# imatge-upc/rsis

Hardware: AMD Instinct MI355X
Metric: training images/sec at 256x256, T=10, batch=32 per GPU (higher is better)
Workload: dtype f32

## Files before the change

include/rsis_hip.h:

```cpp
#ifndef RSIS_HIP_H
#define RSIS_HIP_H
#include <stddef.h>
#ifdef __cplusplus
extern "C" {
#endif

#define RSIS_ABI_VERSION 2

#define RSIS_DTYPE_F32 0
#define RSIS_DTYPE_BF16 1
#define RSIS_DTYPE_BF16_BLK 2
#define RSIS_DTYPE_F32_WINO 3

int rsis_version(void);
const char* rsis_error_string(int code);
int rsis_conv_uses_wino(int ks, int stride, int pad, int Cin, int Cout, int nseg, int lstm_hid);

int rsis_set_deterministic(int on);
int rsis_get_deterministic(void);

int rsis_conv_uses_bf16(int ks, int stride, int pad, int Cout);
long rsis_conv_packed_bytes_fwd(int dtype, int Cout, int ks, int stride, int pad, int nseg, const int* Cseg);
long rsis_conv_packed_bytes_dgrad(int dtype, int Cout, int ks, int stride, int pad, int c_count);
int rsis_conv_pack_fwd(const float* W, void* Wp, int Cout, int Ctot, int ks, int stride, int pad, int nseg, const int* Cseg,
                       const int* Coff, int lstm_hid, int dtype, void* stream);
int rsis_conv_pack_dgrad(const float* W, void* Wd, int Cout, int Ctot, int ks, int stride, int pad, int nseg, const int* Cseg,
                         const int* Coff, int lstm_hid, int dtype, void* stream);

int rsis_conv2d_fwd(const float* const* src, const int* Csrc, int nsrc, int B, int H, int W, const void* Wp, int Cout,
                    int ks, int stride, int pad, const float* bias, const float* addend, float* out, int Ho, int Wo,
                    int tile, int dtype, void* stream);
int rsis_conv2d_fwd_bn_eval(const float* const* src, const int* Csrc, int nsrc, int B, int H, int W, const void* Wp, int Cout,
                            int ks, int stride, int pad, const float* bias, const float* addend, const float* gamma, const float* beta,
                            const float* running_mean, const float* running_var, float eps, int relu, float* out, int Ho, int Wo,
                            int tile, int dtype, void* stream);

int rsis_conv2d_dgrad(const float* dy, int B, int Cout, int Hy, int Wy, const void* Wd, int Cin_packed, int ks, int stride,
                      int pad, float* const* dx, const int* Cdx, int ndst, int Hx, int Wx, const float* addend, int tile,
                      int dtype, void* stream);

int rsis_conv2d_wgrad(const float* dy, const float* x, float* dW, int B, int Cs, int H, int W, int Cout, int Ho, int Wo,
                      int ks, int stride, int pad, int Ctot, int c_off, int lstm_hid, int dtype, void* stream);

typedef struct rsis_wgrad_job {
  const float* dy;
  const float* x;
  float* dW;
  int B, Cs, H, W, Cout, Ho, Wo, ks, stride, pad, Ctot, c_off, lstm_hid, dtype;
} rsis_wgrad_job;
int rsis_conv2d_wgrad_batch(const rsis_wgrad_job* jobs, int njobs, void* stream);

int rsis_bias_grad(const float* dy, float* db, int B, int C, int HW, int lstm_hid, void* stream);

int rsis_convlstm_fwd(const float* const* src, const int* Csrc, int nsrc, int B, int H, int W, const void* Wp,
                      const float* bias_packed, const float* addend, const float* c_prev, float* h_out, float* c_out,
                      float* act_out, int hid, int ks, int pad, int tile, int dtype, void* stream);

typedef struct rsis_lstm_job {
  const float* src[3];
  int Csrc[3];
  int nsrc, B, H, W;
  const void* Wp;
  const float* bias_packed;
  const float* addend;
  const float* c_prev;
  float* h_out;
  float* c_out;
  float* act_out;
  int hid, ks, pad, tile, dtype;
  unsigned long long* side_key;
} rsis_lstm_job;
int rsis_convlstm_fwd_batch(const rsis_lstm_job* jobs, int njobs, void* stream);

int rsis_convlstm_bwd_gates(const float* dh, const float* dh2, const float* dc_next, const float* act, const float* c_prev,
                            const float* c, float* da, float* dc_prev, float* da_sum, int B, int hid, int HW, void* stream);

typedef struct rsis_lstm_bwd_job {
  const float* dh;
  const float* dh2;
  const float* dc_next;
  const float* act;
  const float* c_prev;
  const float* c;
  float* da;
  float* dc_prev;
  int B, hid, HW;
} rsis_lstm_bwd_job;
int rsis_convlstm_bwd_gates_batch(const rsis_lstm_bwd_job* jobs, int njobs, void* stream);
typedef struct rsis_dgrad_job {
  const float* dy;
  int B, Cout, Hy, Wy;
  const void* Wd;
  int Cin_packed, ks, stride, pad;
  float* dx[3];
  int Cdx[3];
  int ndst, Hx, Wx;
  const float* addend;
  int tile, dtype;
} rsis_dgrad_job;
int rsis_conv2d_dgrad_batch(const rsis_dgrad_job* jobs, int njobs, void* stream);

int rsis_upsample_bilinear_ac_fwd(const float* x, float* y, long BC, int Hi, int Wi, int Ho, int Wo, void* stream);
int rsis_upsample_bilinear_ac_bwd(const float* dy, float* dx, long BC, int Hi, int Wi, int Ho, int Wo, void* stream);
int rsis_upsample_maxpool_bwd(const float* dy, const float* dpool, const int* argmax, float* dx, long BC, int Hi, int Wi, int Ho,
                              int Wo, void* stream);

int rsis_global_maxpool_fwd(const float* x, float* y, int* argmax, long BC, int HW, void* stream);
int rsis_global_maxpool_bwd(const float* dy, const int* argmax, float* dx, long BC, int HW, void* stream);
int rsis_global_maxpool_bwd_add(const float* dy, const int* argmax, float* dx, long BC, int HW, void* stream);

int rsis_upsample_bilinear_ac_scaled_fwd(const float* x, const float* scale, float* y, long BC, int Hi, int Wi, int Ho, int Wo, void* stream);
int rsis_upsample_maxpool_scaled_bwd(const float* dy, const float* dpool, const int* argmax, const float* scale, float* dx, long BC, int Hi,
                                     int Wi, int Ho, int Wo, void* stream);
int rsis_global_maxpool_scaled_bwd_add(const float* dy, const int* argmax, const float* scale, float* dx, long BC, int HW, void* stream);
int rsis_scale_planes(const float* x, const float* scale, float* y, long BC, int HW, void* stream);

int rsis_dropout_scales(unsigned int* state, float* s2, float* mc, float* ms, long n, float p2, float pc, float ps, void* stream);
int rsis_dropout_heads_mask(float* side, const float* s2, const float* mc, const float* ms, float* side_c, float* side_s, long n, void* stream);
int rsis_dropout_heads_mask_bwd(const float* dside_c, const float* dside_s, const float* mc, const float* ms, float* dside, long n, void* stream);

int rsis_bn_fwd(const float* x, const float* res, float* y, double* stats, const float* gamma, const float* beta,
                float* running_mean, float* running_var, float* save_mean, float* save_rstd, int B, int C, int HW,
                float eps, float momentum, int relu, int train, void* stream);
int rsis_bn_bwd(const float* dy, const float* x, const float* y, const float* save_mean, const float* save_rstd,
                const float* gamma, double* stats, float* dx, float* dres, float* dgamma, float* dbeta, int B, int C,
                int HW, int relu, void* stream);

int rsis_bn_bwd_eval(const float* dy, const float* x, const float* y, const float* running_mean, const float* running_var,
                     const float* gamma, double* stats, float* dx, float* dres, float* dgamma, float* dbeta, int B, int C, int HW,
                     float eps, int relu, void* stream);

int rsis_bn_fwd_mask(const float* x, const float* res, float* y, unsigned char* mask, double* stats, const float* gamma, const float* beta,
                     float* running_mean, float* running_var, float* save_mean, float* save_rstd, int B, int C, int HW,
                     float eps, float momentum, int train, void* stream);
int rsis_bn_bwd_mask(const float* dy, const float* x, const unsigned char* mask, const float* save_mean, const float* save_rstd,
                     const float* gamma, double* stats, float* dx, float* dres, float* dgamma, float* dbeta, int B, int C,
                     int HW, int flags, void* stream);
int rsis_bn_bwd_eval_mask(const float* dy, const float* x, const unsigned char* mask, const float* running_mean, const float* running_var,
                          const float* gamma, double* stats, float* dx, float* dres, float* dgamma, float* dbeta, int B, int C, int HW,
                          float eps, int flags, void* stream);

int rsis_subsample2d(const float* x, float* y, long BC, int H, int W, int stride, void* stream);

int rsis_maxpool3x3s2_fwd(const float* x, float* y, unsigned char* argmax, long BC, int H, int W, int Ho, int Wo,
                          void* stream);
int rsis_maxpool3x3s2_bwd(const float* dy, const unsigned char* argmax, float* dx, long BC, int H, int W, int Ho, int Wo,
                          int accumulate, void* stream);

int rsis_adam_step(float* p, const float* g, float* m, float* v, long n, float lr, float beta1, float beta2, float eps,
                   float weight_decay, int step, float gscale, const int* step_dev, void* stream);

int rsis_sgd_step(float* p, const float* g, float* buf, long n, float lr, float momentum, float weight_decay, float gscale,
                  void* stream);
int rsis_rmsprop_step(float* p, const float* g, float* sq, long n, float lr, float alpha, float eps, float weight_decay, float gscale,
                      void* stream);

int rsis_assign_min_cost(const float* scores, long long* perm, int B, int G, int T, void* stream);

typedef struct rsis_pack_job {
  const float* W;
  void* out;
  int dgrad;
  int dtype;
  int Cout, Ctot, ks, stride, pad, nseg, Cseg[3], Coff[3], lstm_hid;
  int imode, ldw, krows;
  int block_begin;
} rsis_pack_job;
int rsis_conv_pack_job_fill(rsis_pack_job* job);
int rsis_conv_pack_batch(const rsis_pack_job* jobs_dev, int njobs, int total_blocks, void* stream);

int rsis_conv_out_wgrad(const float* dy, const float* x, float* dW, float* db, int B, int Cin, int H, int W, void* stream);

int rsis_conv_out_seq_fwd(const float* x, const void* Wp, const float* bias, float* y, int T, int B, int Cin, int H, int W, void* stream);
int rsis_conv_out_seq_dgrad(const float* dy, const void* Wd, float* dx, int T, int B, int Cin, int H, int W, void* stream);
int rsis_conv_out_seq_wgrad(const float* dy, const float* x, float* dW, float* db, int T, int B, int Cin, int H, int W, void* stream);

int rsis_sum_leading(const float* x, float* y, int T, long n, void* stream);

int rsis_affine_nearest(const float* x, float* y, const float* mat, int mat_rows, int N, int C, int H, int W, void* stream);

long rsis_targets_work_ints(int B);
int rsis_targets_from_maps(const int* ins, const int* seg, int B, int H, int W, int T, float* y_mask, long long* y_class, float* sw_mask,
                           float* sw_class, int* work, void* stream);

long rsis_instance_maps_work_ints(int B);
int rsis_instance_maps(const int* raw, const int* class_of_label, int n_labels, int B, int H, int W, int* ins, int* seg, int* work,
                       void* stream);

int rsis_palette_to_ids(const unsigned char* rgb, long npix, const unsigned char* table, int ntab, unsigned char* ids, void* stream);
int rsis_idmap_rle_encode(const unsigned char* idmap, int h, int w, const int* ids, int k, unsigned int* counts, int cap, int* nruns,
                          void* stream);

int rsis_softiou_sums(const float* logits, const float* y, float* S, int B, int T, int G, long N, void* stream);
int rsis_softiou_bwd(const float* logits, const float* y, const long long* perm, int perm_ld, const float* ca, const float* cb,
                     float* dlogits, int B, int T, int G, long N, void* stream);

int rsis_heads_fwd(const float* const* side, const int* Cside, int nside, int B, const float* Wc, const float* bc, int ncls,
                   const float* Ws, const float* bs, float* class_probs, float* stop, void* stream);
int rsis_heads_fwd_keys(const unsigned long long* const* keys, float* const* side_out, int* const* arg_out, const int* Cside, int nside,
                        int B, const float* Wc, const float* bc, int ncls, const float* Ws, const float* bs, float* class_probs, float* stop,
                        void* stream);
int rsis_heads_bwd(const float* const* side, const int* Cside, int nside, int B, const float* Wc, int ncls, const float* Ws,
                   const float* class_probs, const float* dprobs, const float* dstop, float* const* dside, float* dWc, float* dbc,
                   float* dWs, float* dbs, void* stream);
int rsis_heads_wide_fwd(const unsigned long long* const* keys, float* const* side_out, int* const* arg_out, const float* const* side,
                        const int* Cside, int nside, int rows, const float* Wc, const float* bc, int ncls, const float* Ws, const float* bs,
                        float* class_probs, float* stop, void* stream);
int rsis_heads_wide_bwd(const float* const* side, const int* Cside, int nside, int rows, const float* Wc, int ncls, const float* Ws,
                        const float* class_probs, const float* dprobs, const float* dstop, float* const* dside, float* dWc, float* dbc,
                        float* dWs, float* dbs, float* scratch, long scratch_floats, void* stream);

int rsis_loss_tail(const float* probs, const long long* y_class, const float* stop, const float* siou, const float* sw_mask,
                   const float* sw_class, const float* cls_w, int n, int C, float bw, float w_iou, float w_cls, float w_stop,
                   float* out, float* dprobs, float* dstop, float* dsiou, const float* gout, void* stream);

int rsis_mask_resize_threshold(const float* prob, int n, int Hm, int Wm, const unsigned char* ignore, float th, unsigned char* seg,
                               unsigned char* raw, unsigned int* area, int h, int w, void* stream);
int rsis_rle_encode(const unsigned char* masks, int n, long len, unsigned int* counts, int cap, int* nruns, void* stream);
int rsis_rle_to_string(const unsigned int* counts, int m, char* out, int cap);
int rsis_largest_component(const unsigned char* mask, unsigned char* out, int* labels, int* counts, int* best, int n, int h, int w,
                           void* stream);

int rsis_overlay_moments(const unsigned char* masks, int n, const int* order, int k, int h, int w, unsigned long long* moments,
                         void* stream);
int rsis_overlay_masks(const unsigned char* image, const unsigned char* masks, int n, const int* order, const unsigned char* colors,
                       int k, float alpha, unsigned char* out, int h, int w, void* stream);

int rsis_mask_pack_bits(const unsigned char* masks, int n, long len, unsigned long long* bits, long stride, unsigned int* area, void* stream);
int rsis_rle_to_bits(const unsigned int* counts, long counts_len, const long long* desc, int n, unsigned int* ends, unsigned long long* bits,
                     long bits_len, unsigned int* area, void* stream);
int rsis_poly_to_bits(const double* xy, long nverts, const long long* parts, long nparts, const long long* recs, int n,
                      unsigned long long* scratch, unsigned long long* bits, long bits_len, unsigned int* area, void* stream);
int rsis_paint_instance_maps(const unsigned long long* bits, long bits_len, const unsigned int* area, long nrec, const long long* recs,
                             const long long* imgs, int B, int max_recs, const int* src_y, const int* src_x, int Ho, int Wo, int* ins, int* seg,
                             void* stream);
long rsis_mask_intersect_blocks(long D, long G, long stride);
int rsis_mask_intersect_batch(const unsigned long long* bits, long bits_len, const long long* jobs, int njobs, int total_blocks,
                              unsigned int* inter, long inter_len, void* stream);
int rsis_coco_iou_batch(const long long* cells, int ncells, const unsigned int* inter, long inter_len, const int* dt_row,
                        const unsigned int* dt_marea, long ndt, const int* gt_col, const unsigned int* gt_marea, const int* gt_crowd, long ngt,
                        double* ious, long ious_len, void* stream);
int rsis_coco_match_batch(const long long* cells, int ncells, const double* ious, long ious_len, const int* gperm, const int* gflag, long ngt,
                          const double* dt_area, long ndt, const double* arng, int nrng, const double* thrs, int T, int* dtm, int* dti,
                          long dt_out_len, int* gtm, long gt_out_len, void* stream);
int rsis_rle_from_string(const char* s, unsigned int* counts, int cap);

long rsis_label_contingency_blocks(long npix);
int rsis_label_contingency_batch(const unsigned char* pool, long pool_len, const long long* jobs, int njobs, int total_blocks,
                                 unsigned int* counts, long counts_len, void* stream);
int rsis_label_scores_batch(const unsigned int* counts, long counts_len, const long long* jobs, int njobs, double* scores, void* stream);

long rsis_inst_overlap_blocks(long npix, long P);
int rsis_inst_presence_batch(const void* pool, long pool_len, const long long* jobs, int njobs, int total_blocks, unsigned char* flags,
                             long flags_len, void* stream);
int rsis_inst_overlap_batch(const void* pool, long pool_len, const long long* jobs, int njobs, int total_blocks, const unsigned short* lut,
                            long lut_len, const unsigned long long* bits, long bits_len, unsigned int* counts, long counts_len, void* stream);


int rsis_blk_from_nchw(const float* x, void* y_blk, int B, int C, int H, int W, void* stream);
int rsis_blk_to_nchw(const void* x_blk, float* y, int B, int C, int H, int W, void* stream);
// ... 99 lines not shown
```

rsis_amd/_lib.py:

```python
import ctypes
import os

import torch

_HERE = os.path.dirname(os.path.abspath(__file__))
LIB_PATH = os.environ.get("RSIS_HIP_LIB") or os.path.join(_HERE, "lib", "librsis_hip.so")

_vp, _i, _l, _f = ctypes.c_void_p, ctypes.c_int, ctypes.c_long, ctypes.c_float
_ip = ctypes.POINTER(ctypes.c_int)
_vpp = ctypes.POINTER(ctypes.c_void_p)

class PackJob(ctypes.Structure):
    _fields_ = [("W", ctypes.c_void_p), ("out", ctypes.c_void_p), ("dgrad", ctypes.c_int), ("dtype", ctypes.c_int), ("Cout", ctypes.c_int),
                ("Ctot", ctypes.c_int), ("ks", ctypes.c_int), ("stride", ctypes.c_int), ("pad", ctypes.c_int),
                ("nseg", ctypes.c_int), ("Cseg", ctypes.c_int * 3), ("Coff", ctypes.c_int * 3), ("lstm_hid", ctypes.c_int),
                ("imode", ctypes.c_int), ("ldw", ctypes.c_int), ("krows", ctypes.c_int), ("block_begin", ctypes.c_int)]


class WgradJob(ctypes.Structure):
    _fields_ = [("dy", ctypes.c_void_p), ("x", ctypes.c_void_p), ("dW", ctypes.c_void_p)] + \
               [(k, ctypes.c_int) for k in ("B", "Cs", "H", "W", "Cout", "Ho", "Wo", "ks", "stride", "pad", "Ctot", "c_off", "lstm_hid", "dtype")]


class LstmJob(ctypes.Structure):
    _fields_ = [("src", ctypes.c_void_p * 3), ("Csrc", ctypes.c_int * 3), ("nsrc", ctypes.c_int), ("B", ctypes.c_int), ("H", ctypes.c_int),
                ("W", ctypes.c_int), ("Wp", ctypes.c_void_p), ("bias_packed", ctypes.c_void_p), ("addend", ctypes.c_void_p),
                ("c_prev", ctypes.c_void_p), ("h_out", ctypes.c_void_p), ("c_out", ctypes.c_void_p), ("act_out", ctypes.c_void_p),
                ("hid", ctypes.c_int), ("ks", ctypes.c_int), ("pad", ctypes.c_int), ("tile", ctypes.c_int), ("dtype", ctypes.c_int),
                ("side_key", ctypes.c_void_p)]


class LstmBwdJob(ctypes.Structure):
    _fields_ = [(k, ctypes.c_void_p) for k in ("dh", "dh2", "dc_next", "act", "c_prev", "c", "da", "dc_prev")] + \
               [(k, ctypes.c_int) for k in ("B", "hid", "HW")]


class DgradJob(ctypes.Structure):
    _fields_ = [("dy", ctypes.c_void_p), ("B", ctypes.c_int), ("Cout", ctypes.c_int), ("Hy", ctypes.c_int), ("Wy", ctypes.c_int),
                ("Wd", ctypes.c_void_p), ("Cin_packed", ctypes.c_int), ("ks", ctypes.c_int), ("stride", ctypes.c_int), ("pad", ctypes.c_int),
                ("dx", ctypes.c_void_p * 3), ("Cdx", ctypes.c_int * 3), ("ndst", ctypes.c_int), ("Hx", ctypes.c_int), ("Wx", ctypes.c_int),
                ("addend", ctypes.c_void_p), ("tile", ctypes.c_int), ("dtype", ctypes.c_int)]


class BlkConvJob(ctypes.Structure):
    _fields_ = [("src", ctypes.c_void_p * 3), ("Csrc", ctypes.c_int * 3), ("nsrc", ctypes.c_int), ("B", ctypes.c_int), ("H", ctypes.c_int),
                ("W", ctypes.c_int), ("Wp", ctypes.c_void_p), ("Cout", ctypes.c_int), ("Cpack", ctypes.c_int), ("bias", ctypes.c_void_p),
                ("addend", ctypes.c_void_p), ("dst", ctypes.c_void_p * 2), ("Cdst", ctypes.c_int * 2), ("ndst", ctypes.c_int),
                ("hid", ctypes.c_int), ("c_prev", ctypes.c_void_p), ("c_out", ctypes.c_void_p), ("h_out", ctypes.c_void_p),
                ("act_out", ctypes.c_void_p), ("side_key", ctypes.c_void_p), ("tile", ctypes.c_int)]


class BlkResizeJob(ctypes.Structure):
    _fields_ = [("src", ctypes.c_void_p), ("dst", ctypes.c_void_p), ("dpool", ctypes.c_void_p), ("arg", ctypes.c_void_p)] + \
               [(k, ctypes.c_int) for k in ("B", "C", "Hi", "Wi", "Ho", "Wo")]


class BlkResizeScaledJob(ctypes.Structure):
    _fields_ = BlkResizeJob._fields_ + [("scale", ctypes.c_void_p)]


class BlkLstmBwdJob(ctypes.Structure):
    _fields_ = [(k, ctypes.c_void_p) for k in ("dh", "dh2", "dc_next", "act", "c_prev", "c", "da", "dc_prev")] + \
               [(k, ctypes.c_int) for k in ("B", "hid", "HW")]


SIGNATURES = {
    "rsis_version": (_i, []),
    "rsis_error_string": (ctypes.c_char_p, [_i]),
    "rsis_set_deterministic": (_i, [_i]),
    "rsis_get_deterministic": (_i, []),
    "rsis_conv_uses_bf16": (_i, [_i, _i, _i, _i]),
    "rsis_conv_uses_wino": (_i, [_i, _i, _i, _i, _i, _i, _i]),
    "rsis_conv_packed_bytes_fwd": (_l, [_i, _i, _i, _i, _i, _i, _ip]),
    "rsis_conv_packed_bytes_dgrad": (_l, [_i, _i, _i, _i, _i, _i]),
    "rsis_conv_pack_fwd": (_i, [_vp, _vp, _i, _i, _i, _i, _i, _i, _ip, _ip, _i, _i, _vp]),
    "rsis_conv_pack_dgrad": (_i, [_vp, _vp, _i, _i, _i, _i, _i, _i, _ip, _ip, _i, _i, _vp]),
    "rsis_conv_pack_job_fill": (_i, [ctypes.POINTER(PackJob)]),
    "rsis_conv_pack_batch": (_i, [_vp, _i, _i, _vp]),
    "rsis_conv2d_fwd": (_i, [_vpp, _ip, _i, _i, _i, _i, _vp, _i, _i, _i, _i, _vp, _vp, _vp, _i, _i, _i, _i, _vp]),
    "rsis_conv2d_fwd_bn_eval": (_i, [_vpp, _ip, _i, _i, _i, _i, _vp, _i, _i, _i, _i, _vp, _vp, _vp, _vp, _vp, _vp, _f, _i, _vp, _i, _i, _i, _i, _vp]),
    "rsis_conv2d_dgrad": (_i, [_vp, _i, _i, _i, _i, _vp, _i, _i, _i, _i, _vpp, _ip, _i, _i, _i, _vp, _i, _i, _vp]),
    "rsis_conv2d_wgrad": (_i, [_vp, _vp, _vp, _i, _i, _i, _i, _i, _i, _i, _i, _i, _i, _i, _i, _i, _i, _vp]),
    "rsis_conv2d_wgrad_batch": (_i, [ctypes.POINTER(WgradJob), _i, _vp]),
    "rsis_affine_nearest": (_i, [_vp, _vp, _vp, _i, _i, _i, _i, _i, _vp]),
    "rsis_targets_work_ints": (_l, [_i]),
    "rsis_targets_from_maps": (_i, [_vp, _vp, _i, _i, _i, _i, _vp, _vp, _vp, _vp, _vp, _vp]),
    "rsis_instance_maps_work_ints": (_l, [_i]),
    "rsis_instance_maps": (_i, [_vp, _vp, _i, _i, _i, _i, _vp, _vp, _vp, _vp]),
    "rsis_palette_to_ids": (_i, [_vp, _l, _vp, _i, _vp, _vp]),
    "rsis_idmap_rle_encode": (_i, [_vp, _i, _i, _vp, _i, _vp, _i, _vp, _vp]),
    "rsis_conv_out_wgrad": (_i, [_vp, _vp, _vp, _vp, _i, _i, _i, _i, _vp]),
    "rsis_conv_out_seq_fwd": (_i, [_vp, _vp, _vp, _vp, _i, _i, _i, _i, _i, _vp]),
    "rsis_conv_out_seq_dgrad": (_i, [_vp, _vp, _vp, _i, _i, _i, _i, _i, _vp]),
    "rsis_conv_out_seq_wgrad": (_i, [_vp, _vp, _vp, _vp, _i, _i, _i, _i, _i, _vp]),
    "rsis_sum_leading": (_i, [_vp, _vp, _i, _l, _vp]),
    "rsis_bias_grad": (_i, [_vp, _vp, _i, _i, _i, _i, _vp]),
    "rsis_convlstm_fwd": (_i, [_vpp, _ip, _i, _i, _i, _i, _vp, _vp, _vp, _vp, _vp, _vp, _vp, _i, _i, _i, _i, _i, _vp]),
    "rsis_convlstm_fwd_batch": (_i, [ctypes.POINTER(LstmJob), _i, _vp]),
    "rsis_convlstm_bwd_gates": (_i, [_vp, _vp, _vp, _vp, _vp, _vp, _vp, _vp, _vp, _i, _i, _i, _vp]),
    "rsis_upsample_bilinear_ac_fwd": (_i, [_vp, _vp, _l, _i, _i, _i, _i, _vp]),
    "rsis_upsample_bilinear_ac_bwd": (_i, [_vp, _vp, _l, _i, _i, _i, _i, _vp]),
    "rsis_upsample_maxpool_bwd": (_i, [_vp, _vp, _vp, _vp, _l, _i, _i, _i, _i, _vp]),
    "rsis_global_maxpool_fwd": (_i, [_vp, _vp, _vp, _l, _i, _vp]),
    "rsis_global_maxpool_bwd": (_i, [_vp, _vp, _vp, _l, _i, _vp]),
    "rsis_global_maxpool_bwd_add": (_i, [_vp, _vp, _vp, _l, _i, _vp]),
    "rsis_bn_fwd": (_i, [_vp, _vp, _vp, _vp, _vp, _vp, _vp, _vp, _vp, _vp, _i, _i, _i, _f, _f, _i, _i, _vp]),
    "rsis_bn_bwd": (_i, [_vp, _vp, _vp, _vp, _vp, _vp, _vp, _vp, _vp, _vp, _vp, _i, _i, _i, _i, _vp]),
    "rsis_bn_bwd_eval": (_i, [_vp, _vp, _vp, _vp, _vp, _vp, _vp, _vp, _vp, _vp, _vp, _i, _i, _i, _f, _i, _vp]),
    "rsis_bn_fwd_mask": (_i, [_vp, _vp, _vp, _vp, _vp, _vp, _vp, _vp, _vp, _vp, _vp, _i, _i, _i, _f, _f, _i, _vp]),
    "rsis_bn_bwd_mask": (_i, [_vp, _vp, _vp, _vp, _vp, _vp, _vp, _vp, _vp, _vp, _vp, _i, _i, _i, _i, _vp]),
    "rsis_bn_bwd_eval_mask": (_i, [_vp, _vp, _vp, _vp, _vp, _vp, _vp, _vp, _vp, _vp, _vp, _i, _i, _i, _f, _i, _vp]),
    "rsis_subsample2d": (_i, [_vp, _vp, _l, _i, _i, _i, _vp]),
    "rsis_maxpool3x3s2_fwd": (_i, [_vp, _vp, _vp, _l, _i, _i, _i, _i, _vp]),
    "rsis_maxpool3x3s2_bwd": (_i, [_vp, _vp, _vp, _l, _i, _i, _i, _i, _i, _vp]),
    "rsis_assign_min_cost": (_i, [_vp, _vp, _i, _i, _i, _vp]),
    "rsis_heads_fwd": (_i, [_vpp, _ip, _i, _i, _vp, _vp, _i, _vp, _vp, _vp, _vp, _vp]),
    "rsis_heads_fwd_keys": (_i, [_vpp, _vpp, _vpp, _ip, _i, _i, _vp, _vp, _i, _vp, _vp, _vp, _vp, _vp]),
    "rsis_blk_from_nchw": (_i, [_vp, _vp, _i, _i, _i, _i, _vp]),
    "rsis_blk_to_nchw": (_i, [_vp, _vp, _i, _i, _i, _i, _vp]),
    "rsis_blk_bn_scratch_doubles": (ctypes.c_long, [_i]),
    "rsis_blk_bn_fwd": (_i, [_vp, _vp, _vp, _vp, _vp, _vp, _vp, _vp, _vp, _vp, _i, _i, _i, _i, _f, _f, _i, _i, _vp]),
    "rsis_blk_bn_bwd": (_i, [_vp, _vp, _vp, _vp, _vp, _vp, _vp, _vp, _vp, _vp, _vp, _vp, _i, _i, _i, _i, _i, _i, _vp]),
    "rsis_blk_subsample2d": (_i, [_vp, _vp, _i, _i, _i, _i, _i, _vp]),
    "rsis_blk_upscatter2d": (_i, [_vp, _vp, _i, _i, _i, _i, _i, _vp]),
    "rsis_blk_conv2d": (_i, [_vp, _i, _i, _i, _i, _vp, _i, _i, _vp, _vp, _i, _vp]),
    "rsis_blk_conv2d_bn_eval": (_i, [_vp, _i, _i, _i, _i, _vp, _i, _i, _vp, _vp, _vp, _vp, _vp, ctypes.c_float, _i, _i, _vp, _i, _vp]),
    "rsis_convlstm_bwd_gates_batch": (_i, [ctypes.POINTER(LstmBwdJob), _i, _vp]),
    "rsis_conv2d_dgrad_batch": (_i, [ctypes.POINTER(DgradJob), _i, _vp]),
    "rsis_blk_conv3x3_batch": (_i, [ctypes.POINTER(BlkConvJob), _i, _vp]),
    "rsis_blk_upsample_fwd_batch": (_i, [ctypes.POINTER(BlkResizeJob), _i, _vp]),
    "rsis_blk_upsample_bwd_batch": (_i, [ctypes.POINTER(BlkResizeJob), _i, _vp]),
    "rsis_blk_lstm_bwd_batch": (_i, [ctypes.POINTER(BlkLstmBwdJob), _i, _vp]),
    "rsis_blk_sum_leading": (_i, [_vp, _vp, _i, _l, _vp]),
    "rsis_blk_bias_grad": (_i, [_vp, _vp, _i, _i, _i, _i, _vp]),
    "rsis_blk_conv_out_seq_fwd": (_i, [_vp, _vp, _vp, _vp, _i, _i, _i, _i, _vp]),
    "rsis_blk_conv_out_seq_dgrad": (_i, [_vp, _vp, _vp, _i, _i, _i, _i, _vp]),
    "rsis_blk_conv_out_seq_wgrad": (_i, [_vp, _vp, _vp, _vp, _i, _i, _i, _i, _vp]),
    "rsis_upconv_out_supported": (_i, [_i, _i, _i, _i, _i]),
    "rsis_upconv_out_bwd_blocks": (_i, [_i, _i, _i, _i]),
    "rsis_upconv_out_fwd": (_i, [_vp, _i, _vp, _vp, _vp, _i, _i, _i, _i, _i, _i, _i, _vp]),
    "rsis_upconv_out_bwd": (_i, [_vp, _vp, _i, _vp, _vp, _vp, _vp, _vp, _vp, _vp, _i, _i, _i, _i, _i, _i, _i, _vp]),
    "rsis_comm_available": (_i, []),
    "rsis_comm_unique_id": (_i, [_vp]),
    "rsis_comm_init": (_i, [_vpp, _i, _i, _vp]),
    "rsis_comm_size": (_i, [_vp]),
    "rsis_comm_allreduce_sum_f32": (_i, [_vp, _vp, _l, _vp]),
    "rsis_comm_destroy": (_i, [_vp]),
    "rsis_comm_last_error": (ctypes.c_char_p, []),
    "rsis_heads_bwd": (_i, [_vpp, _ip, _i, _i, _vp, _i, _vp, _vp, _vp, _vp, _vpp, _vp, _vp, _vp, _vp, _vp]),
    "rsis_heads_wide_fwd": (_i, [_vpp, _vpp, _vpp, _vpp, _ip, _i, _i, _vp, _vp, _i, _vp, _vp, _vp, _vp, _vp]),
    "rsis_heads_wide_bwd": (_i, [_vpp, _ip, _i, _i, _vp, _i, _vp, _vp, _vp, _vp, _vpp, _vp, _vp, _vp, _vp, _vp, _l, _vp]),
    "rsis_loss_tail": (_i, [_vp, _vp, _vp, _vp, _vp, _vp, _vp, _i, _i, _f, _f, _f, _f, _vp, _vp, _vp, _vp, _vp, _vp]),
    "rsis_softiou_sums": (_i, [_vp, _vp, _vp, _i, _i, _i, _l, _vp]),
    "rsis_softiou_bwd": (_i, [_vp, _vp, _vp, _i, _vp, _vp, _vp, _i, _i, _i, _l, _vp]),
    "rsis_mask_resize_threshold": (_i, [_vp, _i, _i, _i, _vp, _f, _vp, _vp, _vp, _i, _i, _vp]),
    "rsis_rle_encode": (_i, [_vp, _i, _l, _vp, _i, _vp, _vp]),
    "rsis_largest_component": (_i, [_vp, _vp, _vp, _vp, _vp, _i, _i, _i, _vp]),
    "rsis_overlay_moments": (_i, [_vp, _i, _vp, _i, _i, _i, _vp, _vp]),
    "rsis_overlay_masks": (_i, [_vp, _vp, _i, _vp, _vp, _i, _f, _vp, _i, _i, _vp]),
    "rsis_rle_to_string": (_i, [_vp, _i, ctypes.c_char_p, _i]),
    "rsis_mask_pack_bits": (_i, [_vp, _i, _l, _vp, _l, _vp, _vp]),
    "rsis_rle_to_bits": (_i, [_vp, _l, _vp, _i, _vp, _vp, _l, _vp, _vp]),
    "rsis_mask_intersect_blocks": (_l, [_l, _l, _l]),
    "rsis_mask_intersect_batch": (_i, [_vp, _l, _vp, _i, _i, _vp, _l, _vp]),
    "rsis_coco_iou_batch": (_i, [_vp, _i, _vp, _l, _vp, _vp, _l, _vp, _vp, _vp, _l, _vp, _l, _vp]),
    "rsis_poly_to_bits": (_i, [_vp, _l, _vp, _l, _vp, _i, _vp, _vp, _l, _vp, _vp]),
    "rsis_paint_instance_maps": (_i, [_vp, _l, _vp, _l, _vp, _vp, _i, _i, _vp, _vp, _i, _i, _vp, _vp, _vp]),
    "rsis_coco_match_batch": (_i, [_vp, _i, _vp, _l, _vp, _vp, _l, _vp, _l, _vp, _i, _vp, _i, _vp, _vp, _l, _vp, _l, _vp]),
    "rsis_rle_from_string": (_i, [ctypes.c_char_p, _vp, _i]),
    "rsis_label_contingency_blocks": (_l, [_l]),
    "rsis_label_contingency_batch": (_i, [_vp, _l, _vp, _i, _i, _vp, _l, _vp]),
    "rsis_label_scores_batch": (_i, [_vp, _l, _vp, _i, _vp, _vp]),
    "rsis_inst_overlap_blocks": (_l, [_l, _l]),
    "rsis_inst_presence_batch": (_i, [_vp, _l, _vp, _i, _i, _vp, _l, _vp]),
    "rsis_inst_overlap_batch": (_i, [_vp, _l, _vp, _i, _i, _vp, _l, _vp, _l, _vp, _l, _vp]),
    "rsis_adam_step": (_i, [_vp, _vp, _vp, _vp, _l, _f, _f, _f, _f, _f, _i, _f, _vp, _vp]),
    "rsis_sgd_step": (_i, [_vp, _vp, _vp, _l, _f, _f, _f, _f, _vp]),
    "rsis_rmsprop_step": (_i, [_vp, _vp, _vp, _l, _f, _f, _f, _f, _f, _vp]),
    "rsis_upsample_bilinear_ac_scaled_fwd": (_i, [_vp, _vp, _vp, _l, _i, _i, _i, _i, _vp]),
# ... 67 lines not shown
```

rsis_amd/csrc/api.hip:

```cpp
#include "common.h"
#include "../../include/rsis_hip.h"
#include "launchers.h"
#include <stdlib.h>

static inline int krows_of(int C, int ks) { return rsis_roundup(C * ks * ks, RSIS_KPAD); }
static inline int log2i(int s) { int l = 0; while ((1 << l) < s) ++l; return l; }
static inline bool use_direct(int ks, int stride, int pad) { return ks == 3 && stride == 1 && pad == 1; }
static inline bool use_direct_s2(int ks, int stride, int pad) { return ks == 3 && stride == 2 && pad == 1; }
static inline bool use_direct_f2(int ks, int stride, int pad) {
  static const bool on = !(getenv("RSIS_CONV_F2") && getenv("RSIS_CONV_F2")[0] == '0');
  return on && use_direct_s2(ks, stride, pad);
}
static inline bool use_direct_fwd(int ks, int stride, int pad) { return use_direct(ks, stride, pad) || use_direct_f2(ks, stride, pad); }
static inline int seg_chunks(int nseg, const int* Cseg, int ck) {
  int q = 0;
  for (int s = 0; s < nseg; ++s) q += (Cseg[s] + ck - 1) / ck;
  return q;
}
static inline int direct_rows(int nseg, const int* Cseg) { return seg_chunks(nseg, Cseg, RSIS_CK) * RSIS_CK * 9; }
static inline bool bf16_geom(int ks, int stride, int pad, int Cout) {
  return Cout > 1 && ((ks == 3 && stride == 1 && pad == 1) || (ks == 1 && pad == 0));
}
static inline bool use_bf16(int dtype, int ks, int stride, int pad, int Cout) {
  return dtype == RSIS_DTYPE_BF16 && bf16_geom(ks, stride, pad, Cout);
// ... 52 lines not shown
    default: return "unknown error";
  }
}

int rsis_conv_uses_bf16(int ks, int stride, int pad, int Cout) { return bf16_geom(ks, stride, pad, Cout) ? 1 : 0; }
int rsis_conv_uses_wino(int ks, int stride, int pad, int Cin, int Cout, int nseg, int lstm_hid) {
  return wino_geom(ks, stride, pad, Cin, Cout, nseg, lstm_hid) ? 1 : 0;
}

struct PackPlan { int status; PackMode mode; int krows; int ldw; long bytes; };
static PackPlan pack_plan(bool dgrad, int dtype, int Cout, int Ctot, int ks, int stride, int pad, int nseg, const int* Cseg, const int* Coff,
                          int lstm_hid) {
  PackPlan p = {RSIS_OK, PACK_IGEMM_FWD, 0, 0, 0};
  int csum = 0;
  for (int s = 0; s < nseg; ++s) csum += Cseg[s];
  p.ldw = rsis_roundup(dgrad ? csum : Cout, RSIS_LDW_ALIGN);
  if (lstm_hid > 0 && dtype == RSIS_DTYPE_BF16 && ks != 3) { p.status = RSIS_ERR_UNSUPPORTED; return p; }
  if (dtype == RSIS_DTYPE_F32_WINO && (dgrad ? wino_geom_dgrad(ks, stride, pad, csum, Cout) : wino_geom(ks, stride, pad, csum, Cout, nseg, lstm_hid))) {
    if (!dgrad && (csum != Ctot || (Coff && Coff[0] != 0))) { p.status = RSIS_ERR_UNSUPPORTED; return p; }
    p.mode = dgrad ? PACK_WINO_DGRAD : PACK_WINO_FWD;
    p.krows = dgrad ? (csum / 32) * (Cout / 8) : (Cout / 32) * (csum / 8);
    p.bytes = (long)p.krows * 32 * 8 * 16 * 4;
    return p;
  }
  long cell = 4;
  if (use_bf16(dtype, ks, stride, pad, Cout)) {
    p.mode = dgrad ? PACK_BF16_DGRAD : PACK_BF16_FWD;
    p.krows = dgrad ? bf16_rows(ks, 1, &Cout) : bf16_rows(ks, nseg, Cseg);
    cell = 16;
  } else if (dgrad ? use_direct(ks, stride, pad) : use_direct_fwd(ks, stride, pad)) {
    p.mode = dgrad ? PACK_DIRECT_DGRAD : PACK_DIRECT_FWD;
    p.krows = dgrad ? direct_rows(1, &Cout) : direct_rows(nseg, Cseg);
  } else if (dgrad && use_direct_s2(ks, stride, pad) && nseg == 1) {
    p.mode = PACK_DIRECT_DGRAD_S2;
    p.krows = direct_rows(1, &Cout);
  } else {
    p.mode = dgrad ? PACK_IGEMM_DGRAD : PACK_IGEMM_FWD;
    p.krows = krows_of(dgrad ? Cout : csum, ks);
  }
  p.bytes = (long)p.krows * p.ldw * cell;
  return p;
}

long rsis_conv_packed_bytes_fwd(int dtype, int Cout, int ks, int stride, int pad, int nseg, const int* Cseg) {
  if (nseg < 1 || nseg > RSIS_MAX_SRC || !Cseg) return -1;
  int csum = 0;
  for (int s = 0; s < nseg; ++s) csum += Cseg[s];
  return pack_plan(false, dtype, Cout, csum, ks, stride, pad, nseg, Cseg, nullptr, 0).bytes;
}

long rsis_conv_packed_bytes_dgrad(int dtype, int Cout, int ks, int stride, int pad, int c_count) {
  const int one[1] = {c_count}, two[2] = {c_count, 0};
  const long a = pack_plan(true, dtype, Cout, c_count, ks, stride, pad, 1, one, nullptr, 0).bytes;
  const long b = pack_plan(true, dtype, Cout, c_count, ks, stride, pad, 2, two, nullptr, 0).bytes;
  return a > b ? a : b;
}

static int pack_args_check(int Cout, int Ctot, int ks, int nseg, const int* Cseg, const int* Coff, int lstm_hid) {
  if (nseg < 1 || nseg > RSIS_MAX_SRC || !Cseg) return RSIS_ERR_ARG;
  int base = 0;
  for (int s = 0; s < nseg; ++s) {
    const int off = Coff ? Coff[s] : base;
    if (Cseg[s] < 1 || off < 0 || off + Cseg[s] > Ctot) return RSIS_ERR_ARG;
    base += Cseg[s];
  }
  if (Cout < 1 || ks < 1 || (long)Cout * Ctot * ks * ks >= (1L << 31)) return RSIS_ERR_ARG;
  return (lstm_hid > 0 && Cout != 4 * lstm_hid) ? RSIS_ERR_ARG : RSIS_OK;
}

static int pack_one(bool dgrad, const float* W, void* out, int Cout, int Ctot, int ks, int stride, int pad, int nseg, const int* Cseg,
                    const int* Coff, int lstm_hid, int dtype, void* stream) {
  if (!W || !out || pack_args_check(Cout, Ctot, ks, nseg, Cseg, Coff, lstm_hid)) return RSIS_ERR_ARG;
  const PackPlan p = pack_plan(dgrad, dtype, Cout, Ctot, ks, stride, pad, nseg, Cseg, Coff, lstm_hid);
  if (p.status) return p.status;
  return rsis_l_pack(p.mode, W, out, Cout, Ctot, ks, nseg, Cseg, Coff, p.ldw, p.krows, lstm_hid, (hipStream_t)stream);
}
int rsis_conv_pack_fwd(const float* W, void* Wp, int Cout, int Ctot, int ks, int stride, int pad, int nseg, const int* Cseg,
                       const int* Coff, int lstm_hid, int dtype, void* stream) {
  return pack_one(false, W, Wp, Cout, Ctot, ks, stride, pad, nseg, Cseg, Coff, lstm_hid, dtype, stream);
}
int rsis_conv_pack_dgrad(const float* W, void* Wd, int Cout, int Ctot, int ks, int stride, int pad, int nseg, const int* Cseg,
                         const int* Coff, int lstm_hid, int dtype, void* stream) {
  return pack_one(true, W, Wd, Cout, Ctot, ks, stride, pad, nseg, Cseg, Coff, lstm_hid, dtype, stream);
}

int rsis_conv_pack_job_fill(rsis_pack_job* j) {
  if (!j || pack_args_check(j->Cout, j->Ctot, j->ks, j->nseg, j->Cseg, j->Coff, j->lstm_hid)) return -1;
  const PackPlan p = pack_plan(j->dgrad != 0, j->dtype, j->Cout, j->Ctot, j->ks, j->stride, j->pad, j->nseg, j->Cseg, j->Coff, j->lstm_hid);
  if (p.status) return -1;
  j->imode = p.mode; j->krows = p.krows; j->ldw = p.ldw;
  return rsis_l_pack_blocks(p.mode, p.krows, p.ldw, j->ks);
}

int rsis_conv_pack_batch(const rsis_pack_job* jobs_dev, int njobs, int total_blocks, void* stream) {
  if (!jobs_dev || njobs < 1 || total_blocks < 1) return RSIS_ERR_ARG;
  return rsis_l_pack_batch(jobs_dev, njobs, total_blocks, (hipStream_t)stream);
}


int rsis_conv_out_wgrad(const float* dy, const float* x, float* dW, float* db, int B, int Cin, int H, int W, void* stream) {
  if (!dy || !x || !dW || B < 1) return RSIS_ERR_ARG;
  if (!rsis_c1_supported(Cin) || W % 4 != 0) return RSIS_ERR_UNSUPPORTED;
  return rsis_l_c1_wgrad(dy, x, dW, db, B, Cin, H, W, 1, (hipStream_t)stream);
}

static inline bool c1_seq_ok(int T, int B, int Cin, int H, int W) {
  return T >= 1 && B >= 1 && rsis_c1_supported(Cin) && W % 4 == 0 && (long)T * B * Cin * H * W < (1L << 40);
}
int rsis_conv_out_seq_fwd(const float* x, const void* Wp, const float* bias, float* y, int T, int B, int Cin, int H, int W, void* stream) {
  if (!x || !Wp || !y) return RSIS_ERR_ARG;
  if (!c1_seq_ok(T, B, Cin, H, W)) return RSIS_ERR_UNSUPPORTED;
  return rsis_l_c1_fwd(x, (const float*)Wp, rsis_roundup(1, RSIS_LDW_ALIGN), bias, y, T * B, Cin, H, W, T, (hipStream_t)stream);
}
int rsis_conv_out_seq_dgrad(const float* dy, const void* Wd, float* dx, int T, int B, int Cin, int H, int W, void* stream) {
  if (!dy || !Wd || !dx) return RSIS_ERR_ARG;
  if (!c1_seq_ok(T, B, Cin, H, W)) return RSIS_ERR_UNSUPPORTED;
  return rsis_l_c1_dgrad(dy, (const float*)Wd, rsis_roundup(Cin, RSIS_LDW_ALIGN), dx, T * B, Cin, H, W, T, (hipStream_t)stream);
}
int rsis_conv_out_seq_wgrad(const float* dy, const float* x, float* dW, float* db, int T, int B, int Cin, int H, int W, void* stream) {
  if (!dy || !x || !dW) return RSIS_ERR_ARG;
  if (!c1_seq_ok(T, B, Cin, H, W)) return RSIS_ERR_UNSUPPORTED;
  return rsis_l_c1_wgrad(dy, x, dW, db, T * B, Cin, H, W, T, (hipStream_t)stream);
}
int rsis_sum_leading(const float* x, float* y, int T, long n, void* stream) {
  if (!x || !y || T < 1 || n < 1) return RSIS_ERR_ARG;
  return rsis_l_sum_leading(x, y, T, n, (hipStream_t)stream);
}

int rsis_affine_nearest(const float* x, float* y, const float* mat, int mat_rows, int N, int C, int H, int W, void* stream) {
  if (!x || !y || !mat || x == y || N < 1 || C < 1 || H < 1 || W < 1 || (mat_rows != 2 && mat_rows != 3)) return RSIS_ERR_ARG;
  if ((long)H * W >= (1L << 31) || N > 65535) return RSIS_ERR_UNSUPPORTED;
  return rsis_l_affine_nearest(x, y, mat, N, C, H, W, mat_rows * 3, (hipStream_t)stream);
}

long rsis_targets_work_ints(int B) { return B < 1 ? 0 : rsis_l_targets_work_ints(B); }

int rsis_targets_from_maps(const int* ins, const int* seg, int B, int H, int W, int T, float* y_mask, long long* y_class, float* sw_mask,
                           float* sw_class, int* work, void* stream) {
  if (!ins || !seg || !y_mask || !y_class || !sw_mask || !sw_class || !work || B < 1 || H < 1 || W < 1 || T < 1) return RSIS_ERR_ARG;
  if ((long)H * W >= (1L << 31) || B > 65535) return RSIS_ERR_UNSUPPORTED;
  return rsis_l_targets_from_maps(ins, seg, B, H, W, T, y_mask, y_class, sw_mask, sw_class, work, (hipStream_t)stream);
}

long rsis_instance_maps_work_ints(int B) { return B < 1 ? 0 : rsis_l_instance_maps_work_ints(B); }

int rsis_instance_maps(const int* raw, const int* class_of_label, int n_labels, int B, int H, int W, int* ins, int* seg, int* work,
                       void* stream) {
  if (!raw || !class_of_label || !ins || !seg || !work || raw == ins || raw == seg || ins == seg || n_labels < 1 || n_labels > 66 ||
      B < 1 || H < 1 || W < 1)
    return RSIS_ERR_ARG;
  if ((long)H * W >= (1L << 31) || B > 65535) return RSIS_ERR_UNSUPPORTED;
  return rsis_l_instance_maps(raw, class_of_label, n_labels, B, H, W, ins, seg, work, (hipStream_t)stream);
}

int rsis_palette_to_ids(const unsigned char* rgb, long npix, const unsigned char* table, int ntab, unsigned char* ids, void* stream) {
  if (!rgb || !table || !ids || npix < 1 || ntab < 1 || ntab > 256) return RSIS_ERR_ARG;
  return rsis_l_palette_to_ids(rgb, npix, table, ntab, ids, (hipStream_t)stream);
}

int rsis_idmap_rle_encode(const unsigned char* idmap, int h, int w, const int* ids, int k, unsigned int* counts, int cap, int* nruns,
                          void* stream) {
  if (!idmap || !ids || !counts || !nruns || h < 1 || w < 1 || k < 1 || cap < 1 || (long)h * w >= (1L << 32)) return RSIS_ERR_ARG;
  return rsis_l_idmap_rle_encode(idmap, h, w, ids, k, counts, cap, nruns, (hipStream_t)stream);
}

static int fill_sources(ConvArgs& a, const float* const* src, const int* Csrc, int nsrc, int ks, bool allow_empty = false) {
// ... 131 lines not shown
    return rsis_launch_conv3x3_direct(a, 2, direct_variant(tile), (hipStream_t)stream);
  }
  if (ks == 1 && pad == 0 && stride > 1) {
    if (!inplace && zero_dsts(a, (hipStream_t)stream)) return RSIS_ERR_LAUNCH;
    a.Ho = Hy; a.Wo = Wy; a.stride = 1; a.sshift = 0; a.ostride = stride;
    return rsis_launch_conv_igemm(a, ks, false, 0, tile, (hipStream_t)stream);
  }
  return rsis_launch_conv_igemm(a, ks, true, 0, tile, (hipStream_t)stream);
}

static int wgrad_route(WgradArgs& a, int ks, int lstm_hid, int dtype) {
  if (dtype == RSIS_DTYPE_BF16_BLK) {
    a.blk = 1;
    return rsis_wgrad_bf16_supported(a, ks) ? 1 : -1;
  }
  if (dtype != RSIS_DTYPE_BF16) {
    const int staged = rsis_wgrad_staged_limbs(a, ks);
    if (staged < 0) return -1;
    if (staged > 0) { a.limbs = 1; return 1; }
  }
  if (use_direct(ks, a.stride, a.pad) && a.Cout == 1 && lstm_hid == 0 && rsis_c1_supported(a.Cs) && a.H == a.Ho && a.W == a.Wo && a.W % 4 == 0)
    return 0;
  if (dtype == RSIS_DTYPE_BF16 && rsis_wgrad_bf16_supported(a, ks)) return 1;
  static const bool tiled_ok = !(getenv("RSIS_WGRAD_TILED") && getenv("RSIS_WGRAD_TILED")[0] == '0');
  if (tiled_ok && rsis_wgrad_tiled_supported(a, ks)) return 2;
  return 3;
}
static int wgrad_fill(WgradArgs& a, const float* dy, const float* x, float* dW, int B, int Cs, int H, int W, int Cout, int Ho, int Wo,
                      int ks, int stride, int pad, int Ctot, int c_off, int lstm_hid) {
  if (!dy || !x || !dW || c_off < 0 || c_off + Cs > Ctot) return RSIS_ERR_ARG;
  a = WgradArgs{};
  a.dy = dy; a.x = x; a.dw = dW; a.B = B; a.Cs = Cs; a.H = H; a.W = W; a.Ho = Ho; a.Wo = Wo; a.Cout = Cout;
  a.stride = stride; a.pad = pad; a.ldo = Ctot * ks * ks; a.n_off = c_off * ks * ks; a.interleave_hid = lstm_hid;
  return RSIS_OK;
}
static int wgrad_launch_one(WgradArgs& a, int route, int ks, hipStream_t st) {
  switch (route) {
    case 0: return rsis_l_c1_wgrad(a.dy, a.x, a.dw + a.n_off, nullptr, a.B, a.Cs, a.H, a.W, 1, st);
    case 1: return rsis_launch_conv_wgrad_bf16(a, ks, st);
    case 2: return rsis_launch_conv_wgrad_tiled(a, ks, st);
    default: return rsis_launch_conv_wgrad(a, ks, st);
  }
}

int rsis_conv2d_wgrad(const float* dy, const float* x, float* dW, int B, int Cs, int H, int W, int Cout, int Ho, int Wo,
                      int ks, int stride, int pad, int Ctot, int c_off, int lstm_hid, int dtype, void* stream) {
  WgradArgs a;
  const int rc = wgrad_fill(a, dy, x, dW, B, Cs, H, W, Cout, Ho, Wo, ks, stride, pad, Ctot, c_off, lstm_hid);
  if (rc) return rc;
  const int route = wgrad_route(a, ks, lstm_hid, dtype);
  if (route < 0) return RSIS_ERR_UNSUPPORTED;
  return wgrad_launch_one(a, route, ks, (hipStream_t)stream);
}

int rsis_conv2d_wgrad_batch(const rsis_wgrad_job* jobs, int njobs, void* stream) {
  if (!jobs || njobs < 1) return RSIS_ERR_ARG;
  WgradArgs* tiled[4] = {(WgradArgs*)malloc(sizeof(WgradArgs) * njobs), (WgradArgs*)malloc(sizeof(WgradArgs) * njobs),
                         (WgradArgs*)malloc(sizeof(WgradArgs) * njobs), (WgradArgs*)malloc(sizeof(WgradArgs) * njobs)};
  int nt[4] = {0, 0, 0, 0};
  int rc = (tiled[0] && tiled[1] && tiled[2] && tiled[3]) ? RSIS_OK : RSIS_ERR_LAUNCH;
  for (int j = 0; j < njobs && rc == RSIS_OK; ++j) {
    const rsis_wgrad_job& q = jobs[j];
    WgradArgs a;
    rc = wgrad_fill(a, q.dy, q.x, q.dW, q.B, q.Cs, q.H, q.W, q.Cout, q.Ho, q.Wo, q.ks, q.stride, q.pad, q.Ctot, q.c_off, q.lstm_hid);
    if (rc) break;
    const int route = wgrad_route(a, q.ks, q.lstm_hid, q.dtype);
    if (route < 0) { rc = RSIS_ERR_UNSUPPORTED; break; }
    if ((route == 1 || route == 2) && (q.ks == 1 || q.ks == 3) && !rsis_deterministic()) {
      const int li = (route == 1 ? 2 : 0) + (q.ks == 3);
      tiled[li][nt[li]++] = a;
    } else rc = wgrad_launch_one(a, route, q.ks, (hipStream_t)stream);
  }
  if (rc == RSIS_OK) rc = rsis_launch_conv_wgrad_tiled_group(tiled[0], nt[0], 1, (hipStream_t)stream);
  if (rc == RSIS_OK) rc = rsis_launch_conv_wgrad_tiled_group(tiled[1], nt[1], 3, (hipStream_t)stream);
  if (rc == RSIS_OK) rc = rsis_launch_conv_wgrad_bf16_group(tiled[2], nt[2], 1, (hipStream_t)stream);
  if (rc == RSIS_OK) rc = rsis_launch_conv_wgrad_bf16_group(tiled[3], nt[3], 3, (hipStream_t)stream);
  for (int i = 0; i < 4; ++i) free(tiled[i]);
  return rc;
}

int rsis_bias_grad(const float* dy, float* db, int B, int C, int HW, int lstm_hid, void* stream) {
  if (!dy || !db) return RSIS_ERR_ARG;
  return rsis_l_channel_sum(dy, db, B, C, HW, lstm_hid, (hipStream_t)stream);
}

static int lstm_fill(ConvArgs& a, int& route, const float* const* src, const int* Csrc, int nsrc, int B, int H, int W, const void* Wp,
                     const float* bias_packed, const float* addend, const float* c_prev, float* h_out, float* c_out, float* act_out, int hid,
                     int ks, int pad, int dtype, unsigned long long* side_key = nullptr) {
  a = ConvArgs{};
  int rc = fill_sources(a, src, Csrc, nsrc, ks, addend != nullptr);
  if (rc) return rc;
  if (!Wp || !h_out || !c_out || hid < 1 || B < 1) return RSIS_ERR_ARG;
  if (2 * pad != ks - 1) return RSIS_ERR_UNSUPPORTED;
  if (dtype == RSIS_DTYPE_BF16 && ks != 3) return RSIS_ERR_UNSUPPORTED;
  a.B = B; a.H = H; a.W = W; a.Ho = H; a.Wo = W; a.stride = 1; a.pad = pad; a.sshift = 0;
  a.wp = (const float*)Wp; a.ldw = rsis_roundup(4 * hid, RSIS_LDW_ALIGN); a.Cout = 4 * hid; a.bias = bias_packed; a.addend = addend;
  a.ndst = 1; a.dst[0] = nullptr; a.Cd[0] = 4 * hid;
  a.hid = hid; a.c_prev = c_prev; a.h_out = h_out; a.c_out = c_out; a.act_out = act_out;
  a.ostride = 1; a.oH = H; a.oW = W; a.ksplit = 1;
  route = use_bf16(dtype, ks, 1, pad, 4 * hid) ? 0 : (use_direct(ks, 1, pad) ? 1 : 2);
  a.side_key = side_key;
  a.precise = act_out ? 0 : 1;
  if (side_key && (route == 2 || (long)H * W >= 0x7FFFFFFFL)) return RSIS_ERR_UNSUPPORTED;
  return RSIS_OK;
}
static int lstm_launch_one(ConvArgs& a, int route, int ks, int tile, hipStream_t st) {
  if (route == 0) return rsis_launch_conv_bf16(a, 3, 1, direct_variant(tile), st);
  if (route == 1) return rsis_launch_conv3x3_direct(a, 1, direct_variant(tile), st);
  return rsis_launch_conv_igemm(a, ks, false, 1, tile, st);
}

int rsis_convlstm_fwd(const float* const* src, const int* Csrc, int nsrc, int B, int H, int W, const void* Wp,
                      const float* bias_packed, const float* addend, const float* c_prev, float* h_out, float* c_out,
                      float* act_out, int hid, int ks, int pad, int tile, int dtype, void* stream) {
  ConvArgs a;
  int route = 0;
  const int rc = lstm_fill(a, route, src, Csrc, nsrc, B, H, W, Wp, bias_packed, addend, c_prev, h_out, c_out, act_out, hid, ks, pad, dtype);
  if (rc) return rc;
  return lstm_launch_one(a, route, ks, tile, (hipStream_t)stream);
}

int rsis_convlstm_fwd_batch(const rsis_lstm_job* jobs, int njobs, void* stream) {
  if (!jobs || njobs < 1) return RSIS_ERR_ARG;
  ConvArgs* grp = (ConvArgs*)malloc(sizeof(ConvArgs) * njobs);
  int* force = (int*)malloc(sizeof(int) * njobs);
  if (!grp || !force) { free(grp); free(force); return RSIS_ERR_LAUNCH; }
  int ng = 0, rc = RSIS_OK;
  for (int j = 0; j < njobs && rc == RSIS_OK; ++j) {
    const rsis_lstm_job& q = jobs[j];
    if (q.nsrc < 0 || q.nsrc > RSIS_MAX_SRC) { rc = RSIS_ERR_ARG; break; }
    ConvArgs a;
    int route = 0;
    rc = lstm_fill(a, route, q.src, q.Csrc, q.nsrc, q.B, q.H, q.W, q.Wp, q.bias_packed, q.addend, q.c_prev, q.h_out, q.c_out, q.act_out,
                   q.hid, q.ks, q.pad, q.dtype, q.side_key);
    if (rc) break;
    const bool groupable = route == 1 && (size_t)q.B * 4 * q.hid * q.H * q.W * 4 < (1ull << 31) && !rsis_deterministic();
    if (groupable) { force[ng] = direct_variant(q.tile % 100); grp[ng++] = a; }
    else rc = lstm_launch_one(a, route, q.ks, q.tile, (hipStream_t)stream);
  }
  if (rc == RSIS_OK && ng == 1) rc = rsis_launch_conv3x3_direct(grp[0], 1, force[0], (hipStream_t)stream);
  else if (rc == RSIS_OK && ng > 1) rc = rsis_launch_convlstm_direct_group(grp, ng, force, (hipStream_t)stream);
  free(grp); free(force);
  return rc;
}

int rsis_convlstm_bwd_gates(const float* dh, const float* dh2, const float* dc_next, const float* act, const float* c_prev,
                            const float* c, float* da, float* dc_prev, float* da_sum, int B, int hid, int HW, void* stream) {
  if (!act || !c || !da) return RSIS_ERR_ARG;
  return rsis_l_lstm_bwd(dh, dh2, dc_next, act, c_prev, c, da, dc_prev, da_sum, B, hid, HW, (hipStream_t)stream);
}

int rsis_upsample_bilinear_ac_fwd(const float* x, float* y, long BC, int Hi, int Wi, int Ho, int Wo, void* stream) {
  if (!x || !y) return RSIS_ERR_ARG;
  return rsis_l_upsample_fwd(x, y, BC, Hi, Wi, Ho, Wo, nullptr, (hipStream_t)stream);
}
int rsis_upsample_bilinear_ac_scaled_fwd(const float* x, const float* scale, float* y, long BC, int Hi, int Wi, int Ho, int Wo, void* stream) {
  if (!x || !y || BC < 1 || Hi < 1 || Wi < 1 || Ho < 1 || Wo < 1) return RSIS_ERR_ARG;
  if (scale && Hi == Ho && Wi == Wo) return rsis_l_scale_planes(x, scale, y, BC, Hi * Wi, (hipStream_t)stream);
  return rsis_l_upsample_fwd(x, y, BC, Hi, Wi, Ho, Wo, scale, (hipStream_t)stream);
}
int rsis_upsample_maxpool_scaled_bwd(const float* dy, const float* dpool, const int* argmax, const float* scale, float* dx, long BC, int Hi, int Wi,
                                     int Ho, int Wo, void* stream) {
  if (!dy || !dx || !dpool || !argmax || BC < 1 || Hi < 1 || Wi < 1 || Ho < 1 || Wo < 1) return RSIS_ERR_ARG;
  return rsis_l_upsample_bwd(dy, dx, BC, Hi, Wi, Ho, Wo, dpool, argmax, scale, (hipStream_t)stream);
}
int rsis_global_maxpool_scaled_bwd_add(const float* dy, const int* argmax, const float* scale, float* dx, long BC, int HW, void* stream) {
// ... 589 lines not shown
```

rsis_amd/csrc/launchers.h:

```cpp
#pragma once
#include "common.h"
#include "../../include/rsis_hip.h"

int rsis_launch_conv_igemm(ConvArgs& a, int ks, bool dgrad, int epi, int force_tile, hipStream_t st);
int rsis_launch_conv3x3_direct(ConvArgs& a, int epi, int force_variant, hipStream_t st);
int rsis_launch_convlstm_direct_group(ConvArgs* jobs, int n, const int* force_variant, hipStream_t st);
int rsis_launch_conv3x3_direct_group_plain(ConvArgs* jobs, int n, const int* force_variant, hipStream_t st);
int rsis_launch_conv_wino(const float* x, const void* U, const float* bias, const float* addend, float* y, int B, int C, int Cout, int H, int W, hipStream_t st,
                          int precise);
int rsis_launch_conv_wino_group(int n, const float* const* x, const void* const* U, float* const* y, float* const* y1, const int* B, const int* C, const int* Cout,
                                const int* C0, const int* H, const int* W, hipStream_t st);
int rsis_launch_conv_bf16(ConvArgs& a, int ks, int epi, int force_variant, hipStream_t st);
int rsis_launch_conv_blk(ConvArgs& a, int ks, int variant, hipStream_t st);
int rsis_l_blk_from_nchw(const float* x, void* y, int B, int C, int HW, hipStream_t st);
int rsis_l_blk_to_nchw(const void* x, float* y, int B, int C, int HW, hipStream_t st);
int rsis_launch_conv_blk_dec(BlkConvJob* jobs, int n, int epi, const int* force_variant, hipStream_t st);
int rsis_launch_conv_wgrad(WgradArgs& a, int ks, hipStream_t st);
bool rsis_wgrad_bf16_supported(const WgradArgs& w, int ks);
int rsis_wgrad_staged_limbs(const WgradArgs& w, int ks);
int rsis_launch_conv_wgrad_bf16_group(const WgradArgs* w, int n, int ks, hipStream_t st);
int rsis_launch_conv_wgrad_bf16(const WgradArgs& w, int ks, hipStream_t st);
int rsis_launch_conv_wgrad_tiled_group(const WgradArgs* w, int n, int ks, hipStream_t st);
int rsis_launch_conv_wgrad_tiled(const WgradArgs& w, int ks, hipStream_t st);
bool rsis_wgrad_tiled_supported(const WgradArgs& w, int ks);
bool rsis_c1_supported(int Cin);
int rsis_l_c1_fwd(const float* x, const float* wp, int ldw, const float* bias, float* y, int B, int Cin, int H, int W, int seqT, hipStream_t st);
int rsis_l_c1_dgrad(const float* dy, const float* wd, int ldw, float* dx, int B, int Cin, int H, int W, int seqT, hipStream_t st);
int rsis_l_c1_wgrad(const float* dy, const float* x, float* dw, float* db, int B, int Cin, int H, int W, int seqT, hipStream_t st);
bool rsis_upconv_supported(int C, int Hs, int Ws, int Ho, int Wo);
int rsis_upconv_bwd_blocks(int T, int B, int Hs, int Ws);
int rsis_l_upconv_fwd(const void* h, int h_blk, const float* w, const float* bias, float* out, int T, int B, int Hs, int Ws, int Ho, int Wo, hipStream_t st);
int rsis_l_upconv_bwd(const float* dout, const void* h, int h_blk, const float* w, void* dh, float* dW, float* db, const float* dside, const int* arg,
                      float* partial, int T, int B, int Hs, int Ws, int Ho, int Wo, hipStream_t st);
int rsis_l_pack_batch(const rsis_pack_job* jobs, int njobs, int total_blocks, hipStream_t st);
int rsis_l_pack_blocks(PackMode mode, int krows, int ldw, int ks);
int rsis_l_pack(PackMode mode, const float* W, void* out, int Cout, int Ctot, int ks, int nseg, const int* Cseg, const int* Coff, int ldw, int krows, int hid,
                hipStream_t st);
int rsis_l_lstm_bwd(const float* dh, const float* dh2, const float* dc_next, const float* act, const float* c_prev, const float* c, float* da, float* dc_prev,
                    float* da_sum, int B, int hid, int HW, hipStream_t st);
int rsis_l_lstm_bwd_group(const void* const* ptrs, const int* dims, int n, hipStream_t st);
int rsis_l_upsample_fwd(const float* x, float* y, long BC, int Hi, int Wi, int Ho, int Wo, const float* scale, hipStream_t st);
int rsis_l_upsample_bwd(const float* dy, float* dx, long BC, int Hi, int Wi, int Ho, int Wo, const float* pool_g, const int* pool_arg, const float* scale,
                        hipStream_t st);
int rsis_l_scale_planes(const float* x, const float* scale, float* y, long BC, int HW, hipStream_t st);
int rsis_l_gmax_fwd(const float* x, float* y, int* arg, long BC, int HW, hipStream_t st);
int rsis_l_gmax_bwd(const float* dy, const int* arg, float* dx, long BC, int HW, hipStream_t st);
int rsis_l_bn_fwd(const float* x, const float* res, float* y, unsigned char* mask, double* stats, const float* gamma, const float* beta, float* run_mean,
                  float* run_var, float* save_mean, float* save_rstd, int B, int C, int HW, float eps, float momentum, int relu, int train_flags, hipStream_t st);
int rsis_l_bn_bwd(const float* dy, const float* x, const float* y, const unsigned char* mask, const float* mean, const float* rstd, const float* gamma,
                  double* stats, float* dx, float* dres, float* dgamma, float* dbeta, int B, int C, int HW, int relu_flags, float eval_eps, hipStream_t st);
int rsis_l_gmax_bwd_add(const float* dy, const int* arg, float* dx, long BC, int HW, const float* scale, hipStream_t st);
int rsis_l_subsample(const float* x, float* y, long BC, int H, int W, int Ho, int Wo, int s, hipStream_t st);
int rsis_l_maxpool_fwd(const float* x, float* y, unsigned char* arg, long BC, int H, int W, int Ho, int Wo, hipStream_t st);
int rsis_l_maxpool_bwd(const float* dy, const unsigned char* arg, float* dx, long BC, int H, int W, int Ho, int Wo, int accumulate, hipStream_t st);
int rsis_l_sum_leading(const float* x, float* y, int T, long n, hipStream_t st);
int rsis_l_channel_sum(const float* dy, float* db, int B, int C, int HW, int hid, hipStream_t st);
int rsis_l_adam(float* p, const float* g, float* m, float* v, long n, float lr, float b1, float b2, float eps, float wd, int step, float gscale, const int* step_dev,
                hipStream_t st);
int rsis_l_assign(const float* scores, long long* perm, int B, int G, int T, hipStream_t st);
int rsis_l_flat_rule(int rule, float* p, const float* g, float* s, long n, float lr, float c0, float c1, float wd, float gscale, hipStream_t st);
long rsis_l_blk_bn_scratch(int C);
int rsis_l_blk_bn_fwd(const void* x, const void* res, void* y, double* scratch, const float* gamma, const float* beta, float* run_mean, float* run_var,
                      float* save_mean, float* save_rstd, int B, int C, int HW, float eps, float momentum, int relu, int train, hipStream_t st);
int rsis_l_blk_bn_bwd(const void* dy, const void* x, const void* y, double* scratch, const float* gamma, const float* beta, const float* save_mean,
                      const float* save_rstd, void* dx, void* dres, float* dgamma, float* dbeta, int accumulate, int B, int C, int HW, int relu, hipStream_t st);
int rsis_l_blk_subsample(const void* x, void* y, long BCb, int H, int W, int Ho, int Wo, int stride, hipStream_t st);
int rsis_l_blk_upscatter(const void* dy, void* dx, long BCb, int H, int W, int Ho, int Wo, int stride, hipStream_t st);
int rsis_l_blk_upsample_fwd(const BlkResizeJob* jobs, int n, hipStream_t st);
int rsis_l_blk_upsample_bwd(const BlkResizeJob* jobs, int n, hipStream_t st);
int rsis_l_blk_upsample_fwd_scaled(const BlkResizeScaledJob* jobs, int n, hipStream_t st);
int rsis_l_blk_upsample_bwd_scaled(const BlkResizeScaledJob* jobs, int n, hipStream_t st);
int rsis_l_blk_lstm_bwd(const BlkLstmBwdJob* jobs, int n, hipStream_t st);
int rsis_l_blk_sum_leading(const void* x, void* y, int T, long n, hipStream_t st);
int rsis_l_blk_channel_sum(const void* dy, float* db, int B, int C, int HW, int hid, hipStream_t st);
int rsis_l_blk_c1_fwd(const void* x, const float* w, const float* bias, float* y, int T, int B, int H, int W, hipStream_t st);
int rsis_l_blk_c1_dgrad(const float* dy, const float* w, void* dx, int T, int B, int H, int W, hipStream_t st);
int rsis_l_blk_c1_wgrad(const float* dy, const void* x, float* dw, float* db, int T, int B, int H, int W, hipStream_t st);
int rsis_l_dropout_scales(unsigned* state, float* s2, float* mc, float* ms, long n, float p2, float pc, float ps, hipStream_t st);
int rsis_l_dropout_heads_mask(float* side, const float* s2, const float* mc, const float* ms, float* side_c, float* side_s, long n, hipStream_t st);
int rsis_l_dropout_heads_mask_bwd(const float* dc, const float* ds, const float* mc, const float* ms, float* dside, long n, hipStream_t st);
int rsis_l_softiou_sums(const float* logits, const float* y, float* S, int B, int T, int G, long N, hipStream_t st);
int rsis_l_softiou_bwd(const float* logits, const float* y, const long long* perm, int perm_ld, const float* ca, const float* cb, float* dlogits, int B, int T,
                       int G, long N, hipStream_t st);
int rsis_l_heads_fwd(const float* const* side, const int* C, int n, int B, const float* Wc, const float* bc, int ncls, const float* Ws, const float* bs,
                     float* probs, float* stop, hipStream_t st, const unsigned long long* const* keys = nullptr, float* const* side_out = nullptr,
                     int* const* arg_out = nullptr);
int rsis_l_heads_bwd(const float* const* side, const int* C, int n, int B, const float* Wc, int ncls, const float* Ws, const float* probs, const float* dprobs,
                     const float* dstop, float* const* dside, float* dWc, float* dbc, float* dWs, float* dbs, hipStream_t st);
int rsis_l_heads_wide_fwd(const float* const* side, const int* C, int n, int rows, const float* Wc, const float* bc, int ncls, const float* Ws,
                          const float* bs, float* probs, float* stop, hipStream_t st, const unsigned long long* const* keys = nullptr,
                          float* const* side_out = nullptr, int* const* arg_out = nullptr);
int rsis_l_heads_wide_bwd(const float* const* side, const int* C, int n, int rows, const float* Wc, int ncls, const float* Ws, const float* probs,
                          const float* dprobs, const float* dstop, float* const* dside, float* dWc, float* dbc, float* dWs, float* dbs, float* scratch,
                          long scratch_floats, hipStream_t st);
int rsis_l_loss_tail(const float* probs, const long long* y_class, const float* stop, const float* siou, const float* sw_mask, const float* sw_class,
                     const float* cls_w, int n, int C, float bw, float w_iou, float w_cls, float w_stop, float* out, float* dprobs, float* dstop, float* dsiou,
                     const float* gout, hipStream_t st);
int rsis_l_affine_nearest(const float* x, float* y, const float* mat, int N, int C, int H, int W, int mat_stride, hipStream_t st);
long rsis_l_targets_work_ints(int B);
int rsis_l_targets_from_maps(const int* ins, const int* seg, int B, int H, int W, int T, float* y_mask, long long* y_class, float* sw_mask, float* sw_class,
                             int* work, hipStream_t st);
long rsis_l_instance_maps_work_ints(int B);
int rsis_l_instance_maps(const int* raw, const int* class_of_label, int n_labels, int B, int H, int W, int* ins, int* seg, int* work, hipStream_t st);
int rsis_l_palette_to_ids(const unsigned char* rgb, long npix, const unsigned char* table, int ntab, unsigned char* ids, hipStream_t st);
int rsis_l_idmap_rle_encode(const unsigned char* idmap, int h, int w, const int* ids, int k, unsigned int* counts, int cap, int* nruns, hipStream_t st);
int rsis_l_mask_resize_threshold(const float* prob, int n, int Hm, int Wm, const unsigned char* ignore, float th, unsigned char* seg, unsigned char* raw,
                                 unsigned int* area, int h, int w, hipStream_t st);
int rsis_l_rle_encode(const unsigned char* masks, int n, long len, unsigned int* counts, int cap, int* nruns, hipStream_t st);
int rsis_l_rle_to_string(const unsigned int* counts, int m, char* out, int cap);
int rsis_l_largest_component(const unsigned char* mask, unsigned char* out, int* labels, int* counts, int* best, int n, int h, int w, hipStream_t st);
int rsis_l_overlay_moments(const unsigned char* masks, int n, const int* order, int k, int h, int w, unsigned long long* moments, hipStream_t st);
int rsis_l_overlay_masks(const unsigned char* image, const unsigned char* masks, int n, const int* order, const unsigned char* colors, int k, float alpha,
                         unsigned char* out, int h, int w, hipStream_t st);
int rsis_l_mask_pack_bits(const unsigned char* masks, int n, long len, unsigned long long* bits, long stride, unsigned int* area, hipStream_t st);
int rsis_l_rle_to_bits(const unsigned int* counts, long counts_len, const long long* desc, int n, unsigned int* ends, unsigned long long* bits, long bits_len,
                       unsigned int* area, hipStream_t st);
int rsis_l_poly_to_bits(const double* xy, long nverts, const long long* parts, long nparts, const long long* recs, int n, unsigned long long* scratch,
                        unsigned long long* bits, long bits_len, unsigned int* area, hipStream_t st);
int rsis_l_paint_instance_maps(const unsigned long long* bits, long bits_len, const unsigned int* area, long nrec, const long long* recs,
                               const long long* imgs, int B, int max_recs, const int* src_y, const int* src_x, int Ho, int Wo, int* ins, int* seg,
                               hipStream_t st);
long rsis_l_mask_intersect_blocks(long D, long G, long stride);
int rsis_l_mask_intersect_batch(const unsigned long long* bits, long bits_len, const long long* jobs, int njobs, int total_blocks, unsigned int* inter,
                                long inter_len, hipStream_t st);
int rsis_l_coco_iou_batch(const long long* cells, int ncells, const unsigned int* inter, long inter_len, const int* dt_row, const unsigned int* dt_marea, long ndt,
                          const int* gt_col, const unsigned int* gt_marea, const int* gt_crowd, long ngt, double* ious, long ious_len, hipStream_t st);
int rsis_l_coco_match_batch(const long long* cells, int ncells, const double* ious, long ious_len, const int* gperm, const int* gflag, long ngt,
                            const double* dt_area, long ndt, const double* arng, int nrng, const double* thrs, int T, int* dtm, int* dti, long dt_out_len, int* gtm,
                            long gt_out_len, hipStream_t st);
int rsis_l_rle_from_string(const char* s, unsigned int* counts, int cap);
long rsis_l_label_contingency_blocks(long npix);
int rsis_l_label_contingency_batch(const unsigned char* pool, long pool_len, const long long* jobs, int njobs, int total_blocks, unsigned int* counts,
                                   long counts_len, hipStream_t st);
int rsis_l_label_scores_batch(const unsigned int* counts, long counts_len, const long long* jobs, int njobs, double* scores, hipStream_t st);
long rsis_l_inst_overlap_blocks(long npix, long P);
int rsis_l_inst_presence_batch(const unsigned char* pool, long pool_len, const long long* jobs, int njobs, int total_blocks, unsigned char* flags, long flags_len,
                               hipStream_t st);
int rsis_l_inst_overlap_batch(const unsigned char* pool, long pool_len, const long long* jobs, int njobs, int total_blocks, const unsigned short* lut, long lut_len,
                              const unsigned long long* bits, long bits_len, unsigned int* counts, long counts_len, hipStream_t st);
// ... 1 lines not shown
```

rsis_amd/csrc/pointwise.hip:

```cpp
#include "common.h"
#include "launchers.h"
#include <cstdlib>
#include <type_traits>

__global__ void lstm_bwd_kernel(const float* __restrict__ dh, const float* __restrict__ dh2, const float* __restrict__ dc_next,
                                const float* __restrict__ act, const float* __restrict__ c_prev,
                                const float* __restrict__ c, float* __restrict__ da, float* __restrict__ dc_prev,
                                float* __restrict__ da_sum, int hid, int HW, long total) {
  for (long e = blockIdx.x * (long)blockDim.x + threadIdx.x; e < total; e += (long)gridDim.x * blockDim.x) {
    const long bj = e / HW;
    const int sp = (int)(e - bj * HW);
    const long g0 = bj * 4 * HW + sp;
    const float gi = act[g0], gf = act[g0 + HW], go = act[g0 + 2L * HW], gg = act[g0 + 3L * HW];
    const float tc = tanhf(c[e]);
    const float dhv = (dh ? dh[e] : 0.f) + (dh2 ? dh2[e] : 0.f);
    float dcv = dhv * go * (1.f - tc * tc);
    if (dc_next) dcv += dc_next[e];
    const float cp = c_prev ? c_prev[e] : 0.f;
    const float dai = dcv * gg * gi * (1.f - gi);
    const float daf = dcv * cp * gf * (1.f - gf);
    const float dao = dhv * tc * go * (1.f - go);
    const float dag = dcv * gi * (1.f - gg * gg);
    da[g0] = dai; da[g0 + HW] = daf; da[g0 + 2L * HW] = dao; da[g0 + 3L * HW] = dag;
    if (da_sum) { da_sum[g0] += dai; da_sum[g0 + HW] += daf; da_sum[g0 + 2L * HW] += dao; da_sum[g0 + 3L * HW] += dag; }
// ... 482 lines not shown
  double s1 = 0.0, s2 = 0.0;
  if ((HW & 3) == 0) {
    BN_FOREACH(4, {
      f32x4 g = *reinterpret_cast<const f32x4*>(dy + idx);
      const f32x4 xv = *reinterpret_cast<const f32x4*>(x + idx);
      if constexpr (MASK) {
        bn_mask_grad(g, mask[idx >> 2]);
      } else if (relu) {
        const f32x4 yv = *reinterpret_cast<const f32x4*>(y + idx);
        for (int k = 0; k < 4; ++k) if (!(yv[k] > 0.f)) g[k] = 0.f;
      }
      float p1 = 0.f, p2 = 0.f;
      for (int k = 0; k < 4; ++k) { p1 += g[k]; p2 += g[k] * ((xv[k] - m) * r); }
      s1 += p1; s2 += p2;
    })
  } else {
    BN_FOREACH(1, {
      float g = dy[idx];
      if (relu && !(y[idx] > 0.f)) g = 0.f;
      s1 += g; s2 += (double)g * ((x[idx] - m) * r);
    })
  }
  block_reduce2_atomic(s1, s2, stats + 2 * c);
}

template <bool MASK>
__global__ __launch_bounds__(256) void bn_bwd_apply_kernel(const float* __restrict__ dy, const float* __restrict__ x,
                                                           const float* __restrict__ y, const unsigned char* __restrict__ mask,
                                                           const float* __restrict__ mean,
                                                           const float* __restrict__ rstd, const float* __restrict__ gamma,
                                                           const double* __restrict__ stats, float* __restrict__ dx,
                                                           float* __restrict__ dres, float* __restrict__ dgamma,
                                                           float* __restrict__ dbeta, int C, int HW, long N, int relu,
                                                           int accum, float eval_eps) {
  const int c = blockIdx.x;
  const bool ev = eval_eps >= 0.f;
  const float m = mean[c], r = ev ? 1.f / sqrtf(rstd[c] + eval_eps) : rstd[c];
  const float mg = ev ? 0.f : (float)(stats[2 * c] / (double)N), mgx = ev ? 0.f : (float)(stats[2 * c + 1] / (double)N);
  const float kk = gamma[c] * r;
  if (blockIdx.y == 0 && threadIdx.x == 0) {
    const float dg = (float)stats[2 * c + 1], db = (float)stats[2 * c];
    dgamma[c] = accum ? dgamma[c] + dg : dg;
    dbeta[c] = accum ? dbeta[c] + db : db;
  }
  if ((HW & 3) == 0) {
    BN_FOREACH(4, {
      f32x4 g = *reinterpret_cast<const f32x4*>(dy + idx);
      const f32x4 xv = *reinterpret_cast<const f32x4*>(x + idx);
      if constexpr (MASK) {
        bn_mask_grad(g, mask[idx >> 2]);
      } else if (relu) {
        const f32x4 yv = *reinterpret_cast<const f32x4*>(y + idx);
        for (int k = 0; k < 4; ++k) if (!(yv[k] > 0.f)) g[k] = 0.f;
      }
      f32x4 o;
      for (int k = 0; k < 4; ++k) o[k] = kk * (g[k] - mg - ((xv[k] - m) * r) * mgx);
      *reinterpret_cast<f32x4*>(dx + idx) = o;
      if (dres) *reinterpret_cast<f32x4*>(dres + idx) = g;
    })
  } else {
    BN_FOREACH(1, {
      float g = dy[idx];
      if (relu && !(y[idx] > 0.f)) g = 0.f;
      const float xh = (x[idx] - m) * r;
      dx[idx] = kk * (g - mg - xh * mgx);
      if (dres) dres[idx] = g;
    })
  }
}
#undef BN_FOREACH

template <int NT>
__device__ __forceinline__ void block_allreduce2(double& a, double& b) {
  for (int o = 32; o > 0; o >>= 1) { a += __shfl_down(a, o, 64); b += __shfl_down(b, o, 64); }
  __shared__ double sa[NT / 64], sb[NT / 64];
  const int w = threadIdx.x >> 6;
  if ((threadIdx.x & 63) == 0) { sa[w] = a; sb[w] = b; }
  __syncthreads();
  a = 0.0; b = 0.0;
#pragma unroll
  for (int i = 0; i < NT / 64; ++i) { a += sa[i]; b += sb[i]; }
}

template <int NT, int VPT>
__global__ __launch_bounds__(NT) void bn_fwd_fused_kernel(const float* __restrict__ x, const float* __restrict__ res,
                                                          float* __restrict__ y, unsigned char* __restrict__ mask,
                                                          const float* __restrict__ gamma,
                                                          const float* __restrict__ beta, float* __restrict__ run_mean,
                                                          float* __restrict__ run_var, float* __restrict__ save_mean,
                                                          float* __restrict__ save_rstd, int C, int HW, long N, float eps,
                                                          float momentum, int relu) {
  const int c = blockIdx.x;
  const int ng = (int)(N / 4), hwg = HW / 4;
  f32x4 v[VPT];
  double s = 0.0, ss = 0.0;
#pragma unroll
  for (int i = 0; i < VPT; ++i) {
    const int g = threadIdx.x + i * NT;
    if (g < ng) {
      const int b = g / hwg, sp = (g - b * hwg) * 4;
      v[i] = *reinterpret_cast<const f32x4*>(x + ((size_t)b * C + c) * HW + sp);
      s += (v[i][0] + v[i][1]) + (v[i][2] + v[i][3]);
      ss += (v[i][0] * v[i][0] + v[i][1] * v[i][1]) + (v[i][2] * v[i][2] + v[i][3] * v[i][3]);
    }
  }
  block_allreduce2<NT>(s, ss);
  const double m = s / (double)N;
  double var = ss / (double)N - m * m;
  if (var < 0) var = 0;
  const float mean = (float)m, rstd = (float)(1.0 / sqrt(var + (double)eps));
  if (threadIdx.x == 0) {
    save_mean[c] = mean; save_rstd[c] = rstd;
    const double unb = N > 1 ? var * (double)N / (double)(N - 1) : var;
    run_mean[c] = (1.f - momentum) * run_mean[c] + momentum * mean;
    run_var[c] = (1.f - momentum) * run_var[c] + momentum * (float)unb;
  }
  const float sc = rstd * gamma[c], sh = beta[c] - mean * sc;
#pragma unroll
  for (int i = 0; i < VPT; ++i) {
    const int g = threadIdx.x + i * NT;
    if (g < ng) {
      const int b = g / hwg, sp = (g - b * hwg) * 4;
      const size_t idx = ((size_t)b * C + c) * HW + sp;
      f32x4 r = {0.f, 0.f, 0.f, 0.f};
      if (res) r = *reinterpret_cast<const f32x4*>(res + idx);
      f32x4 o;
#pragma unroll
      for (int k = 0; k < 4; ++k) { const float t = v[i][k] * sc + sh + r[k]; o[k] = relu ? fmaxf(t, 0.f) : t; }
      *reinterpret_cast<f32x4*>(y + idx) = o;
      if (mask) mask[idx >> 2] = bn_relu_bits(o);
    }
  }
}

template <int NT, int VPT, bool MASK>
__global__ __launch_bounds__(NT) void bn_bwd_fused_kernel(const float* __restrict__ dy, const float* __restrict__ x,
                                                          const float* __restrict__ y, const unsigned char* __restrict__ mask,
                                                          const float* __restrict__ mean,
                                                          const float* __restrict__ rstd, const float* __restrict__ gamma,
                                                          float* __restrict__ dx, float* __restrict__ dres,
                                                          float* __restrict__ dgamma, float* __restrict__ dbeta, int C, int HW,
                                                          long N, int relu, int accum) {
  const int c = blockIdx.x;
  const int ng = (int)(N / 4), hwg = HW / 4;
  const float m = mean[c], r = rstd[c];
  f32x4 g[VPT], xh[VPT];
  double s1 = 0.0, s2 = 0.0;
  if constexpr (MASK) {
    unsigned mb[VPT];
#pragma unroll
    for (int i = 0; i < VPT; ++i) {
      const int gi = min((int)threadIdx.x + i * NT, ng - 1);
      const int b = gi / hwg, sp = (gi - b * hwg) * 4;
      const size_t idx = ((size_t)b * C + c) * HW + sp;
      g[i] = *reinterpret_cast<const f32x4*>(dy + idx);
      xh[i] = *reinterpret_cast<const f32x4*>(x + idx);
      mb[i] = mask[idx >> 2];
    }
#pragma unroll
    for (int i = 0; i < VPT; ++i) {
      if ((int)threadIdx.x + i * NT < ng) {
        bn_mask_grad(g[i], mb[i]);
        float p1 = 0.f, p2 = 0.f;
#pragma unroll
        for (int k = 0; k < 4; ++k) { xh[i][k] = (xh[i][k] - m) * r; p1 += g[i][k]; p2 += g[i][k] * xh[i][k]; }
        s1 += p1; s2 += p2;
      }
    }
  } else {
#pragma unroll
    for (int i = 0; i < VPT; ++i) {
      const int gi = threadIdx.x + i * NT;
      if (gi < ng) {
        const int b = gi / hwg, sp = (gi - b * hwg) * 4;
        const size_t idx = ((size_t)b * C + c) * HW + sp;
        g[i] = *reinterpret_cast<const f32x4*>(dy + idx);
        const f32x4 xv = *reinterpret_cast<const f32x4*>(x + idx);
        if (relu) {
          const f32x4 yv = *reinterpret_cast<const f32x4*>(y + idx);
#pragma unroll
          for (int k = 0; k < 4; ++k) if (!(yv[k] > 0.f)) g[i][k] = 0.f;
        }
        float p1 = 0.f, p2 = 0.f;
#pragma unroll
        for (int k = 0; k < 4; ++k) { xh[i][k] = (xv[k] - m) * r; p1 += g[i][k]; p2 += g[i][k] * xh[i][k]; }
        s1 += p1; s2 += p2;
      }
    }
  }
  block_allreduce2<NT>(s1, s2);
  const float mg = (float)(s1 / (double)N), mgx = (float)(s2 / (double)N);
  const float kk = gamma[c] * r;
  if (threadIdx.x == 0) {
    const float dg = (float)s2, db = (float)s1;
    dgamma[c] = accum ? dgamma[c] + dg : dg;
    dbeta[c] = accum ? dbeta[c] + db : db;
  }
#pragma unroll
  for (int i = 0; i < VPT; ++i) {
    const int gi = threadIdx.x + i * NT;
    if (gi < ng) {
      const int b = gi / hwg, sp = (gi - b * hwg) * 4;
      const size_t idx = ((size_t)b * C + c) * HW + sp;
      f32x4 o;
#pragma unroll
      for (int k = 0; k < 4; ++k) o[k] = kk * (g[i][k] - mg - xh[i][k] * mgx);
      *reinterpret_cast<f32x4*>(dx + idx) = o;
      if (dres) *reinterpret_cast<f32x4*>(dres + idx) = g[i];
    }
  }
}

__global__ void subsample_kernel(const float* __restrict__ x, float* __restrict__ y, int H, int W, int Ho, int Wo, int s, long total4) {
  const int wq = (Wo + 3) / 4;
  for (long e = blockIdx.x * (long)blockDim.x + threadIdx.x; e < total4; e += (long)gridDim.x * blockDim.x) {
    const int q = (int)(e % wq);
    const long t = e / wq;
    const int ho = (int)(t % Ho);
    const long bc = t / Ho;
    const float* xr = x + (bc * H + (long)ho * s) * W;
    float* yr = y + (bc * Ho + ho) * (long)Wo + 4 * q;
    if (s == 2 && (W & 3) == 0 && 4 * q + 3 < Wo && 8 * q + 7 < W) {
      const f32x4 a = *reinterpret_cast<const f32x4*>(xr + 8 * q), b = *reinterpret_cast<const f32x4*>(xr + 8 * q + 4);
      const f32x4 o = {a[0], a[2], b[0], b[2]};
      if ((Wo & 3) == 0) *reinterpret_cast<f32x4*>(yr) = o;
      else { yr[0] = o[0]; yr[1] = o[1]; yr[2] = o[2]; yr[3] = o[3]; }
    } else {
      for (int k = 0; k < 4 && 4 * q + k < Wo; ++k) yr[k] = xr[(long)(4 * q + k) * s];
    }
  }
}

__global__ void maxpool3x3s2_fwd_kernel(const float* __restrict__ x, float* __restrict__ y, unsigned char* __restrict__ arg,
                                        int H, int W, int Ho, int Wo, long total) {
  for (long e = blockIdx.x * (long)blockDim.x + threadIdx.x; e < total; e += (long)gridDim.x * blockDim.x) {
    const int wo = (int)(e % Wo);
    const long t = e / Wo;
    const int ho = (int)(t % Ho);
    const long bc = t / Ho;
    const float* xb = x + bc * H * W;
    float v[9];
    bool ok[9];
#pragma unroll
    for (int r = 0; r < 3; ++r)
#pragma unroll
      for (int s = 0; s < 3; ++s) {
        const int h = ho * 2 - 1 + r, w = wo * 2 - 1 + s;
        ok[r * 3 + s] = (unsigned)h < (unsigned)H && (unsigned)w < (unsigned)W;
        v[r * 3 + s] = xb[min(max(h, 0), H - 1) * W + min(max(w, 0), W - 1)];
      }
    float best = -INFINITY; int bi = 0;
#pragma unroll
    for (int k = 0; k < 9; ++k)
      if (ok[k] && (v[k] > best || v[k] != v[k])) { best = v[k]; bi = k; }
    y[e] = best; arg[e] = (unsigned char)bi;
  }
}

__global__ void maxpool3x3s2_bwd_kernel(const float* __restrict__ dy, const unsigned char* __restrict__ arg,
                                        float* __restrict__ dx, int H, int W, int Ho, int Wo, long total, int accumulate) {
  for (long e = blockIdx.x * (long)blockDim.x + threadIdx.x; e < total; e += (long)gridDim.x * blockDim.x) {
    const int w = (int)(e % W);
    const long t = e / W;
    const int h = (int)(t % H);
    const long bc = t / H;
    float g = 0.f;
    const int ho_lo = h >> 1, wo_lo = w >> 1;
#pragma unroll
    for (int a = 0; a < 2; ++a) {
#pragma unroll
      for (int b = 0; b < 2; ++b) {
        const int ho = ho_lo + a, wo = wo_lo + b;
        const int r = h - (ho * 2 - 1), s = w - (wo * 2 - 1);
        const bool ok = ho < Ho && r >= 0 && r <= 2 && wo < Wo && s >= 0 && s <= 2;
        const long o = (bc * Ho + min(ho, Ho - 1)) * Wo + min(wo, Wo - 1);
        const int ar = arg[o];
        const float d = dy[o];
        g += (ok && ar == r * 3 + s) ? d : 0.f;
      }
    }
    if (accumulate) g += dx[e];
    dx[e] = g;
  }
}

__global__ __launch_bounds__(256) void maxpool3x3s2_bwd_v8_kernel(const float* __restrict__ dy, const unsigned char* __restrict__ arg,
                                                                  float* __restrict__ dx, int H, int W, int Ho, int Wo, long items,
                                                                  int accumulate) {
  const int Wq = W >> 2, Hp = H >> 1;
  for (long e = blockIdx.x * (long)blockDim.x + threadIdx.x; e < items; e += (long)gridDim.x * blockDim.x) {
    const int wq = (int)(e % Wq);
    const long t = e / Wq;
    const int hp = (int)(t % Hp);
    const long bc = t / Hp;
    const int h0 = hp * 2, w0 = wq * 4;
    float d[6];
    int th[6], tw[6];
#pragma unroll
    for (int a = 0; a < 2; ++a)
#pragma unroll
      for (int b = 0; b < 3; ++b) {
        const int ho = hp + a, wo = wq * 2 + b;
        const bool ok = ho < Ho && wo < Wo;
        const long o = (bc * Ho + min(ho, Ho - 1)) * Wo + min(wo, Wo - 1);
        const int ar = arg[o];
        d[a * 3 + b] = dy[o];
        th[a * 3 + b] = ok ? ho * 2 - 1 + ar / 3 - h0 : -1;
        tw[a * 3 + b] = wo * 2 - 1 + ar % 3 - w0;
      }
    f32x4 o0 = {0.f, 0.f, 0.f, 0.f}, o1 = {0.f, 0.f, 0.f, 0.f};
#pragma unroll
    for (int k = 0; k < 6; ++k)
#pragma unroll
      for (int j = 0; j < 4; ++j) {
        o0[j] += (th[k] == 0 && tw[k] == j) ? d[k] : 0.f;
        o1[j] += (th[k] == 1 && tw[k] == j) ? d[k] : 0.f;
      }
    float* p = dx + (bc * H + h0) * W + w0;
    if (accumulate) {
      o0 += *reinterpret_cast<const f32x4*>(p);
      o1 += *reinterpret_cast<const f32x4*>(p + W);
    }
    *reinterpret_cast<f32x4*>(p) = o0;
    *reinterpret_cast<f32x4*>(p + W) = o1;
  }
}

__global__ __launch_bounds__(256) void channel_sum_kernel(const float* __restrict__ dy, float* __restrict__ db, int C, int HW,
                                                          long N, int hid) {
  const int c = blockIdx.x;
  double s = 0.0;
  if ((HW & 3) == 0) {
    const long ng = N / 4;
    const int hwg = HW / 4;
    for (long g = blockIdx.y * 256L + threadIdx.x; g < ng; g += gridDim.y * 256L) {
      const long b = g / hwg; const int sp = (int)(g - b * hwg) * 4;
      const f32x4 v = *reinterpret_cast<const f32x4*>(dy + (b * C + c) * HW + sp);
      s += ((double)v[0] + (double)v[1]) + ((double)v[2] + (double)v[3]);
    }
  } else {
    for (long e = blockIdx.y * 256L + threadIdx.x; e < N; e += gridDim.y * 256L) {
      const long b = e / HW; const int sp = (int)(e - b * HW);
      s += dy[(b * C + c) * HW + sp];
    }
  }
  for (int o = 32; o > 0; o >>= 1) s += __shfl_down(s, o, 64);
  __shared__ double sa[4];
  if ((threadIdx.x & 63) == 0) sa[threadIdx.x >> 6] = s;
  __syncthreads();
  if (threadIdx.x == 0) {
    const int row = hid > 0 ? (c & 3) * hid + (c >> 2) : c;
    atomicAdd(db + row, (float)(sa[0] + sa[1] + sa[2] + sa[3]));
  }
}

__global__ void adam_kernel(float* __restrict__ p, const float* __restrict__ g, float* __restrict__ m, float* __restrict__ v,
                            long n, float lr, float b1, float b2, float eps, float wd, int step, float gscale,
                            const int* __restrict__ step_dev) {
  const float st = (float)(step_dev ? *step_dev : step);
  const float bc1 = 1.f - powf(b1, st);
  const float bc2_sqrt = sqrtf(1.f - powf(b2, st));
  for (long e = blockIdx.x * (long)blockDim.x + threadIdx.x; e < n; e += (long)gridDim.x * blockDim.x) {
    float gv = g[e] * gscale + wd * p[e];
    const float mv = b1 * m[e] + (1.f - b1) * gv;
    const float vv = b2 * v[e] + (1.f - b2) * gv * gv;
    m[e] = mv; v[e] = vv;
    const float denom = sqrtf(vv) / bc2_sqrt + eps;
    p[e] -= (lr / bc1) * (mv / denom);
  }
}

#define RSIS_ASSIGN_MAX 64
__global__ __launch_bounds__(64) void assign_kernel(const float* __restrict__ scores, long long* __restrict__ perm, int B, int G,
                                                    int T) {
  const int b = blockIdx.x;
  const int lane = threadIdx.x;
  const float* a = scores + (size_t)b * G * T;
  const int n = T, m = G;
  const bool col = lane < m;
  double u = 0.0, v = 0.0;
  int p = 0;
  for (int i = 1; i <= n; ++i) {
    const int p0 = i;
    int j0 = 0;
    double minv = 1e300;
    bool used = false, in_tree = false;
    int way = 0;
    for (int it = 0; it <= m; ++it) {
      if (j0 > 0 && lane == j0 - 1) used = true;
      const int i0 = j0 == 0 ? p0 : __shfl(p, j0 - 1, 64);
      if (lane == i0 - 1) in_tree = true;
      const double ui0 = __shfl(u, i0 - 1, 64);
      double cand = 1e300;
      if (col && !used) {
        const float sc = a[(size_t)lane * T + (i0 - 1)];
        const double cur = (sc == sc && fabsf(sc) < 1e30f ? (double)sc : 1e30) - ui0 - v;
        if (cur < minv) { minv = cur; way = j0; }
        cand = minv;
      }
      double best = cand;
      int bj = lane;
      for (int o = 32; o > 0; o >>= 1) {
        const double ob = __shfl_xor(best, o, 64);
        const int oj = __shfl_xor(bj, o, 64);
        if (ob < best || (ob == best && oj < bj)) { best = ob; bj = oj; }
      }
      const double delta = best;
      if (in_tree) u += delta;
      if (col) { if (used) v -= delta; else minv -= delta; }
      j0 = bj + 1;
      if (__shfl(p, j0 - 1, 64) == 0) break;
    }
    while (j0 != 0) {
      const int j1 = __shfl(way, j0 - 1, 64);
      const int pj1 = j1 == 0 ? p0 : __shfl(p, j1 - 1, 64);
      if (lane == j0 - 1) p = pj1;
      j0 = j1;
    }
  }
  __shared__ long long outp[RSIS_ASSIGN_MAX];
  if (lane < G) outp[lane] = 0;
  __syncthreads();
  if (col && p != 0) outp[p - 1] = lane;
  __syncthreads();
  if (lane < G) perm[(size_t)b * G + lane] = outp[lane];
}

#define RSIS_ASSIGN_MAX2 128
__device__ __forceinline__ int assign2_lane(int x, int l) { return __builtin_amdgcn_readlane(x, l); }
__device__ __forceinline__ double assign2_lane(double x, int l) {
  return __hiloint2double(__builtin_amdgcn_readlane(__double2hiint(x), l), __builtin_amdgcn_readlane(__double2loint(x), l));
}
template <int CTRL, int ROW_MASK>
__device__ __forceinline__ double assign2_min_dpp(double x) {
  const int lo = __double2loint(x), hi = __double2hiint(x);
  return fmin(x, __hiloint2double(__builtin_amdgcn_update_dpp(hi, hi, CTRL, ROW_MASK, 0xf, false),
// ... 173 lines not shown
      const int tiles_x = (Wo + 63) / 64, tiles_y = (Ho + 31) / 32;
      if (!scale)
        hipLaunchKernelGGL((upsample_fwd_lds_kernel<32, 64, 20, 12>), dim3((unsigned)(BC * tiles_x * tiles_y)), dim3(256), 0, st, x, y, Hi,
                           Wi, Ho, Wo, fh, fw, tiles_x, tiles_y, scale);
      else
        hipLaunchKernelGGL((upsample_fwd_lds_kernel<32, 64, 20, 12, true>), dim3((unsigned)(BC * tiles_x * tiles_y)), dim3(256), 0, st, x, y,
                           Hi, Wi, Ho, Wo, fh, fw, tiles_x, tiles_y, scale);
      return rsis_check_launch();
    }
  }
  if (Wo % 4 == 0 && BC * Ho < (1L << 31)) {
    const int Wq = Wo / 4;
    const long rows = BC * Ho;
    int shift = -1;
    if (Wq <= 256 && (Wq & (Wq - 1)) == 0) { shift = 0; while ((1 << shift) < Wq) ++shift; }
    if (shift < 0 && Wq <= 256) shift = -2;
    const dim3 grid = shift >= 0 ? dim3((unsigned)((rows + (256 >> shift) - 1) / (256 >> shift)))
                                 : (shift == -2 ? dim3((unsigned)((rows * Wq + 255) / 256)) : dim3((unsigned)rows, (Wq + 255) / 256));
    sc_pick(scale, [&](auto sc) {
      hipLaunchKernelGGL((upsample_fwd_v4_kernel<decltype(sc)::value>), grid, dim3(256), 0, st, x, y, Hi, Wi, Ho, Wo, ac_scale(Hi, Ho),
                         ac_scale(Wi, Wo), rows, Wq, shift, scale);
    });
  } else {
    sc_pick(scale, [&](auto sc) {
      hipLaunchKernelGGL((upsample_fwd_kernel<decltype(sc)::value>), dim3(ew_grid(total)), dim3(256), 0, st, x, y, Hi, Wi, Ho, Wo,
                         ac_scale(Hi, Ho), ac_scale(Wi, Wo), total, scale);
    });
  }
  return rsis_check_launch();
}
int rsis_l_upsample_bwd(const float* dy, float* dx, long BC, int Hi, int Wi, int Ho, int Wo, const float* pool_g, const int* pool_arg,
                        const float* scale, hipStream_t st) {
  const float sh = ac_scale(Hi, Ho), sw = ac_scale(Wi, Wo);
  const float smin = sh < sw ? sh : sw;
  const bool tiled = smin > 0.f && (2.f / smin + 1.f <= UK);
  const int ut = (Hi > 16 || Wi > 16) ? 32 : 16;
  const bool fits = tiled && ((ut - 1) / smin + UK + 3 <= (ut == 32 ? 80 : 44));
  if (fits) {
    const int tiles_x = (Wi + ut - 1) / ut, tiles_y = (Hi + ut - 1) / ut;
    long ppb = BC * tiles_x * tiles_y / 2048;
    if (ppb < 1) ppb = 1;
    if (ppb > 16) ppb = 16;
    const long blocks = (BC + ppb - 1) / ppb * tiles_x * tiles_y;
    const int vec = Wo % 4 == 0;
    if (ut == 32 && !scale)
      hipLaunchKernelGGL((upsample_bwd_kernel<32, 80>), dim3((unsigned)blocks), dim3(256), 0, st, dy, dx, Hi, Wi, Ho, Wo, sh, sw, tiles_x,
                         tiles_y, BC, (int)ppb, vec, pool_g, pool_arg, scale);
    else if (ut == 32)
      hipLaunchKernelGGL((upsample_bwd_kernel<32, 80, true>), dim3((unsigned)blocks), dim3(256), 0, st, dy, dx, Hi, Wi, Ho, Wo, sh, sw, tiles_x,
                         tiles_y, BC, (int)ppb, vec, pool_g, pool_arg, scale);
    else if (!scale)
      hipLaunchKernelGGL((upsample_bwd_kernel<16, 44>), dim3((unsigned)blocks), dim3(256), 0, st, dy, dx, Hi, Wi, Ho, Wo, sh, sw, tiles_x,
                         tiles_y, BC, (int)ppb, vec, pool_g, pool_arg, scale);
    else
      hipLaunchKernelGGL((upsample_bwd_kernel<16, 44, true>), dim3((unsigned)blocks), dim3(256), 0, st, dy, dx, Hi, Wi, Ho, Wo, sh, sw, tiles_x,
                         tiles_y, BC, (int)ppb, vec, pool_g, pool_arg, scale);
  } else {
    const long total = BC * Hi * Wi;
    sc_pick(scale, [&](auto sc) {
      hipLaunchKernelGGL((upsample_bwd_generic_kernel<decltype(sc)::value>), dim3(ew_grid(total)), dim3(256), 0, st, dy, dx, Hi, Wi, Ho, Wo, sh, sw,
                         total, pool_g, pool_arg, scale);
    });
  }
  return rsis_check_launch();
}
int rsis_l_gmax_fwd(const float* x, float* y, int* arg, long BC, int HW, hipStream_t st) {
  hipLaunchKernelGGL(global_maxpool_fwd_kernel, dim3((unsigned)BC), dim3(256), 0, st, x, y, arg, HW);
  return rsis_check_launch();
}
int rsis_l_gmax_bwd(const float* dy, const int* arg, float* dx, long BC, int HW, hipStream_t st) {
  const long total = BC * HW;
  hipLaunchKernelGGL(global_maxpool_bwd_kernel, dim3(ew_grid(total)), dim3(256), 0, st, dy, arg, dx, HW, total);
  return rsis_check_launch();
}
int rsis_l_bn_fwd(const float* x, const float* res, float* y, unsigned char* mask, double* stats, const float* gamma, const float* beta,
                  float* run_mean, float* run_var, float* save_mean, float* save_rstd, int B, int C, int HW, float eps,
                  float momentum, int relu, int train_flags, hipStream_t st) {
  const long N = (long)B * HW;
  const int S = chan_splits(C, N);
  const int train = train_flags & 1;
  if (mask && (!relu || (HW & 3))) return RSIS_ERR_UNSUPPORTED;
  if (train && bn_fused_ok(C, HW, N)) {
    if (N / 4 <= 256 * 8 && C <= 512)
      hipLaunchKernelGGL((bn_fwd_fused_kernel<512, 4>), dim3(C), dim3(512), 0, st, x, res, y, mask, gamma, beta, run_mean, run_var,
                         save_mean, save_rstd, C, HW, N, eps, momentum, relu);
    else if (N / 4 <= 256 * 8)
      hipLaunchKernelGGL((bn_fwd_fused_kernel<256, 8>), dim3(C), dim3(256), 0, st, x, res, y, mask, gamma, beta, run_mean, run_var,
                         save_mean, save_rstd, C, HW, N, eps, momentum, relu);
    else
      hipLaunchKernelGGL((bn_fwd_fused_kernel<1024, 8>), dim3(C), dim3(1024), 0, st, x, res, y, mask, gamma, beta, run_mean, run_var,
                         save_mean, save_rstd, C, HW, N, eps, momentum, relu);
    return rsis_check_launch();
  }
  if (train) {
    if (!(train_flags & 2) && rsis_zero_async(stats, sizeof(double) * 2 * C, st) != RSIS_OK) return RSIS_ERR_LAUNCH;
    hipLaunchKernelGGL(bn_stats_kernel, dim3(C, S), dim3(256), 0, st, x, stats, C, HW, N);
  }
  hipLaunchKernelGGL(bn_apply_kernel, dim3(C, S), dim3(256), 0, st, x, res, y, mask, stats, gamma, beta, run_mean, run_var, save_mean,
                     save_rstd, C, HW, N, eps, momentum, relu, train ? 0 : 1);
  return rsis_check_launch();
}
template <int NT, int VPT>
static void bn_bwd_fused_launch(const float* dy, const float* x, const float* y, const unsigned char* mask, const float* mean,
                                const float* rstd, const float* gamma, float* dx, float* dres, float* dgamma, float* dbeta, int C,
                                int HW, long N, int relu, int accum, hipStream_t st) {
  if (mask)
    hipLaunchKernelGGL((bn_bwd_fused_kernel<NT, VPT, true>), dim3(C), dim3(NT), 0, st, dy, x, y, mask, mean, rstd, gamma, dx, dres,
                       dgamma, dbeta, C, HW, N, relu, accum);
  else
    hipLaunchKernelGGL((bn_bwd_fused_kernel<NT, VPT, false>), dim3(C), dim3(NT), 0, st, dy, x, y, mask, mean, rstd, gamma, dx, dres,
                       dgamma, dbeta, C, HW, N, relu, accum);
}
int rsis_l_bn_bwd(const float* dy, const float* x, const float* y, const unsigned char* mask, const float* mean, const float* rstd,
                  const float* gamma, double* stats, float* dx, float* dres, float* dgamma, float* dbeta, int B, int C, int HW,
                  int relu_flags, float eval_eps, hipStream_t st) {
  const long N = (long)B * HW;
  const int S = chan_splits(C, N);
  const int relu = relu_flags & 1, accum = (relu_flags >> 2) & 1;
  if (mask && (!relu || (HW & 3))) return RSIS_ERR_UNSUPPORTED;
  if (eval_eps < 0.f && bn_fused_ok(C, HW, N)) {
    if (N / 4 <= 256 * 8 && C <= 512)
      bn_bwd_fused_launch<512, 4>(dy, x, y, mask, mean, rstd, gamma, dx, dres, dgamma, dbeta, C, HW, N, relu, accum, st);
    else if (N / 4 <= 256 * 8)
      bn_bwd_fused_launch<256, 8>(dy, x, y, mask, mean, rstd, gamma, dx, dres, dgamma, dbeta, C, HW, N, relu, accum, st);
    else
      bn_bwd_fused_launch<1024, 8>(dy, x, y, mask, mean, rstd, gamma, dx, dres, dgamma, dbeta, C, HW, N, relu, accum, st);
    return rsis_check_launch();
  }
  if (!(relu_flags & 2) && rsis_zero_async(stats, sizeof(double) * 2 * C, st) != RSIS_OK) return RSIS_ERR_LAUNCH;
  if (mask) {
    hipLaunchKernelGGL(bn_bwd_reduce_kernel<true>, dim3(C, S), dim3(256), 0, st, dy, x, y, mask, mean, rstd, stats, C, HW, N, relu,
                       eval_eps);
    hipLaunchKernelGGL(bn_bwd_apply_kernel<true>, dim3(C, S), dim3(256), 0, st, dy, x, y, mask, mean, rstd, gamma, stats, dx, dres,
                       dgamma, dbeta, C, HW, N, relu, accum, eval_eps);
  } else {
    hipLaunchKernelGGL(bn_bwd_reduce_kernel<false>, dim3(C, S), dim3(256), 0, st, dy, x, y, mask, mean, rstd, stats, C, HW, N, relu,
                       eval_eps);
    hipLaunchKernelGGL(bn_bwd_apply_kernel<false>, dim3(C, S), dim3(256), 0, st, dy, x, y, mask, mean, rstd, gamma, stats, dx, dres,
                       dgamma, dbeta, C, HW, N, relu, accum, eval_eps);
  }
  return rsis_check_launch();
}
int rsis_l_scale_planes(const float* x, const float* scale, float* y, long BC, int HW, hipStream_t st) {
  const long total = BC * HW;
  hipLaunchKernelGGL(scale_planes_kernel, dim3(ew_grid(total)), dim3(256), 0, st, x, scale, y, HW, total);
  return rsis_check_launch();
}
int rsis_l_gmax_bwd_add(const float* dy, const int* arg, float* dx, long BC, int HW, const float* scale, hipStream_t st) {
  sc_pick(scale, [&](auto sc) {
    hipLaunchKernelGGL((global_maxpool_bwd_add_kernel<decltype(sc)::value>), dim3((unsigned)((BC + 255) / 256)), dim3(256), 0, st, dy, arg, dx, HW, BC,
                       scale);
  });
  return rsis_check_launch();
}
int rsis_l_subsample(const float* x, float* y, long BC, int H, int W, int Ho, int Wo, int s, hipStream_t st) {
  const long total4 = BC * Ho * ((Wo + 3) / 4);
  hipLaunchKernelGGL(subsample_kernel, dim3(ew_grid(total4)), dim3(256), 0, st, x, y, H, W, Ho, Wo, s, total4);
  return rsis_check_launch();
}
int rsis_l_maxpool_fwd(const float* x, float* y, unsigned char* arg, long BC, int H, int W, int Ho, int Wo, hipStream_t st) {
  const long total = BC * Ho * Wo;
  hipLaunchKernelGGL(maxpool3x3s2_fwd_kernel, dim3(ew_grid(total)), dim3(256), 0, st, x, y, arg, H, W, Ho, Wo, total);
  return rsis_check_launch();
}
int rsis_l_maxpool_bwd(const float* dy, const unsigned char* arg, float* dx, long BC, int H, int W, int Ho, int Wo, int accumulate,
                       hipStream_t st) {
  const long total = BC * H * W;
  if ((H & 1) == 0 && (W & 3) == 0) {
    hipLaunchKernelGGL(maxpool3x3s2_bwd_v8_kernel, dim3(ew_grid(total / 8)), dim3(256), 0, st, dy, arg, dx, H, W, Ho, Wo, total / 8,
                       accumulate);
    return rsis_check_launch();
  }
  hipLaunchKernelGGL(maxpool3x3s2_bwd_kernel, dim3(ew_grid(total)), dim3(256), 0, st, dy, arg, dx, H, W, Ho, Wo, total, accumulate);
  return rsis_check_launch();
}
__global__ __launch_bounds__(256) void sum_leading_kernel(const float* __restrict__ x, float* __restrict__ y, int T, long n, long n4) {
  const long e = (long)blockIdx.x * 256 + threadIdx.x;
  if (e < n4) {
    const f32x4* p = reinterpret_cast<const f32x4*>(x) + e;
    f32x4 acc = p[0];
    for (int t = 1; t < T; ++t) { const f32x4 v = p[(size_t)t * (n / 4)]; acc[0] += v[0]; acc[1] += v[1]; acc[2] += v[2]; acc[3] += v[3]; }
    reinterpret_cast<f32x4*>(y)[e] = acc;
  } else {
    const long i = 4 * n4 + (e - n4);
    if (i < n) { float acc = x[i]; for (int t = 1; t < T; ++t) acc += x[(size_t)t * n + i]; y[i] = acc; }
  }
}
int rsis_l_sum_leading(const float* x, float* y, int T, long n, hipStream_t st) {
  const bool v4 = (n % 4 == 0) && ((((size_t)x | (size_t)y) & 15) == 0);
  const long n4 = v4 ? n / 4 : 0, threads = n4 + (n - 4 * n4);
  hipLaunchKernelGGL(sum_leading_kernel, dim3((unsigned)((threads + 255) / 256)), dim3(256), 0, st, x, y, T, n, n4);
  return rsis_check_launch();
}

int rsis_l_channel_sum(const float* dy, float* db, int B, int C, int HW, int hid, hipStream_t st) {
  const long N = (long)B * HW;
  int S = chan_splits(C, N);
  if (S > 512) S = 512;
  hipLaunchKernelGGL(channel_sum_kernel, dim3(C, S), dim3(256), 0, st, dy, db, C, HW, N, hid);
  return rsis_check_launch();
}
int rsis_l_adam(float* p, const float* g, float* m, float* v, long n, float lr, float b1, float b2, float eps, float wd,
                int step, float gscale, const int* step_dev, hipStream_t st) {
  hipLaunchKernelGGL(adam_kernel, dim3(ew_grid(n)), dim3(256), 0, st, p, g, m, v, n, lr, b1, b2, eps, wd, step, gscale, step_dev);
  return rsis_check_launch();
}

int rsis_l_assign(const float* scores, long long* perm, int B, int G, int T, hipStream_t st) {
  if (G > RSIS_ASSIGN_MAX2) return RSIS_ERR_ARG;
  if (G <= RSIS_ASSIGN_MAX) hipLaunchKernelGGL(assign_kernel, dim3(B), dim3(64), 0, st, scores, perm, B, G, T);
  else hipLaunchKernelGGL(assign2_kernel, dim3(B), dim3(64), sizeof(float) * (size_t)G * (T < 2 ? 2 : T), st, scores, perm, B, G, T);
  return rsis_check_launch();
}
```

rsis_amd/decoder_seq.py:

```python
import os

import torch

from . import _lib, decoder_fused, dropout, ops
from ._lib import check, int_array, lib, ptr, ptr_array, stream

ENABLED = [os.environ.get("RSIS_DECODER_SEQ", "1") != "0"]
RECORD, LAST = [False], {}


def _is_blk(t):
    return t.dtype == torch.bfloat16 and t.dim() == 5 and t.shape[-1] == 8


def _chan(t):
    return t.shape[1] * 8 if _is_blk(t) else t.shape[1]


def supported(decoder, skip_feats, T):
    n = len(decoder.clstm_list)
    if not (ENABLED[0] and decoder_fused.WAVEFRONT[0] and decoder_fused.FUSED_POOL[0] and decoder.fused and decoder.skip_mode == "concat" and
            len(skip_feats) == n and T >= 1 and "forward" not in decoder.__dict__):
        return False
    if not all(0 <= p < 1 for p in dropout.rates(decoder)):
# ... 189 lines not shown
                  "rsis_conv_out_seq_fwd")
        else:
            tmp = torch.empty((B, 1, H5, W5), dtype=torch.float32, device=self.dev)
            for t in range(T):
                check(L.rsis_conv2d_fwd(ptr_array([UP5[t]]), int_array([last.hid]), 1, B, H5, W5, ptr(co_wp), 1, 3, 1, 1, ptr(co_b.detach()), None,
                                        ptr(tmp), H5, W5, ops.FORCE_TILE[0], co_pack.dtype, stream()), "rsis_conv2d_fwd(conv_out)")
                out_masks[:, t].copy_(tmp.view(B, -1))

    def tail_bwd(self, d_masks, last, UP5, dUP5, conv_out, co_w, dW, db):
        L, T, B = self.L, self.T, self.B
        H5, W5 = 2 * last.H, 2 * last.W
        co_pack = conv_out._pack
        co_wd = co_pack.dgrad(co_w)
        dW = dW() if dW else None
        db = db() if db else None
        if self.seq_ok:
            check(L.rsis_conv_out_seq_dgrad(ptr(d_masks), ptr(co_wd), ptr(dUP5), T, B, last.hid, H5, W5, stream()), "rsis_conv_out_seq_dgrad")
            if dW is not None:
                check(L.rsis_conv_out_seq_wgrad(ptr(d_masks), ptr(UP5), ptr(dW), ptr(db), T, B, last.hid, H5, W5, stream()), "rsis_conv_out_seq_wgrad")
            elif db is not None:
                db += d_masks.sum()
            return
        for t in range(T):
            dy = d_masks[:, t].contiguous().view(B, 1, H5, W5)
            check(L.rsis_conv2d_dgrad(ptr(dy), B, 1, H5, W5, ptr(co_wd), co_pack.cin, 3, 1, 1, ptr_array([dUP5[t]]), int_array([last.hid]), 1,
                                      H5, W5, None, ops.FORCE_TILE[0], co_pack.dtype, stream()), "rsis_conv2d_dgrad(conv_out)")
            if dW is not None:
                check(L.rsis_conv2d_wgrad(ptr(dy), ptr(UP5[t]), ptr(dW), B, last.hid, H5, W5, 1, H5, W5, 3, 1, 1, last.hid, 0, 0, co_pack.dtype,
                                          stream()), "rsis_conv2d_wgrad(conv_out)")
            if db is not None:
                check(L.rsis_bias_grad(ptr(dy), ptr(db), B, 1, H5 * W5, 0, stream()), "rsis_bias_grad(conv_out)")

    def up5_bwd(self, dUP5, dside, last, DH_last, sc=None):
        if sc is not None:
            check(self.L.rsis_upsample_maxpool_scaled_bwd(ptr(dUP5), ptr(dside), ptr(last.ARG), ptr(sc), ptr(DH_last), self.T * self.B * last.hid,
                                                          last.H, last.W, 2 * last.H, 2 * last.W, stream()), "rsis_upsample_maxpool_scaled_bwd(all steps)")
            return
        check(self.L.rsis_upsample_maxpool_bwd(ptr(dUP5), ptr(dside), ptr(last.ARG), ptr(DH_last), self.T * self.B * last.hid, last.H, last.W,
                                               2 * last.H, 2 * last.W, stream()), "rsis_upsample_maxpool_bwd(all steps)")

    def up_bwd(self, levels, cells, DUP, DH, dsides, s2=None):
        B = self.B
        for i, t in cells:
            if i + 1 < len(levels):
                lv, nx = levels[i], levels[i + 1]
                if s2 is not None and (nx.H, nx.W) == (lv.H, lv.W):
                    check(self.L.rsis_scale_planes(ptr(DUP[i + 1]), ptr(s2[i][t]), ptr(DH[i]), B * lv.hid, lv.H * lv.W, stream()), "rsis_scale_planes")
                    check(self.L.rsis_global_maxpool_scaled_bwd_add(ptr(dsides[i][t]), ptr(lv.ARG[t]), ptr(s2[i][t]), ptr(DH[i]), B * lv.hid,
                                                                    lv.H * lv.W, stream()), "rsis_global_maxpool_scaled_bwd_add")
                elif s2 is not None:
                    check(self.L.rsis_upsample_maxpool_scaled_bwd(ptr(DUP[i + 1]), ptr(dsides[i][t]), ptr(lv.ARG[t]), ptr(s2[i][t]), ptr(DH[i]),
                                                                  B * lv.hid, lv.H, lv.W, nx.H, nx.W, stream()), "rsis_upsample_maxpool_scaled_bwd")
                elif (nx.H, nx.W) == (lv.H, lv.W):
                    DH[i].copy_(DUP[i + 1])
                    check(self.L.rsis_global_maxpool_bwd_add(ptr(dsides[i][t]), ptr(lv.ARG[t]), ptr(DH[i]), B * lv.hid, lv.H * lv.W, stream()),
                          "rsis_global_maxpool_bwd_add")
                else:
                    check(self.L.rsis_upsample_maxpool_bwd(ptr(DUP[i + 1]), ptr(dsides[i][t]), ptr(lv.ARG[t]), ptr(DH[i]), B * lv.hid, lv.H, lv.W,
                                                           nx.H, nx.W, stream()), "rsis_upsample_maxpool_bwd")

    def lstm_bwd(self, jobs):
        lb = (_lib.LstmBwdJob * len(jobs))()
        for j, job in zip(lb, jobs):
            j.dh, j.dh2, j.dc_next, j.act, j.c_prev, j.c, j.da, j.dc_prev = [ptr(x) for x in job]
            dh = job[0]
            j.B, j.hid, j.HW = dh.shape[0], dh.shape[1], dh.shape[2] * dh.shape[3]
        check(self.L.rsis_convlstm_bwd_gates_batch(lb, len(jobs), stream()), "rsis_convlstm_bwd_gates_batch")

    def dgrad(self, jobs):
        if not jobs:
            return
        dg = (_lib.DgradJob * len(jobs))()
        for j, (dy, wd, cin, dtype, dxs) in zip(dg, jobs):
            B, Cout, H, W = dy.shape
            (j.dy, j.B, j.Cout, j.Hy, j.Wy, j.Wd, j.Cin_packed, j.ks, j.stride, j.pad, j.ndst, j.Hx, j.Wx, j.addend, j.tile, j.dtype) = (
                ptr(dy), B, Cout, H, W, ptr(wd), cin, 3, 1, 1, len(dxs), H, W, None, ops.FORCE_TILE[0], dtype)
            for k, x in enumerate(dxs):
                j.dx[k], j.Cdx[k] = x.data_ptr(), x.shape[1]
        check(self.L.rsis_conv2d_dgrad_batch(dg, len(jobs), stream()), "rsis_conv2d_dgrad_batch")

    def sum_t(self, DA, dG):
        check(self.L.rsis_sum_leading(ptr(DA), ptr(dG), self.T, dG.numel(), stream()), "rsis_sum_leading")

    def skip_dgrad(self, jobs):
        for dy, wd, cin, dtype, (dx,) in jobs:
            B, Cout, H, W = dy.shape
            check(self.L.rsis_conv2d_dgrad(ptr(dy), B, Cout, H, W, ptr(wd), cin, 3, 1, 1, ptr_array([dx]), int_array([dx.shape[1]]), 1, H, W, None,
                                           ops.FORCE_TILE[0], dtype, stream()), "rsis_conv2d_dgrad(hoist)")

    def bias_grad(self, dG, db, lv):
        check(self.L.rsis_bias_grad(ptr(dG), ptr(db), self.B, 4 * lv.hid, lv.H * lv.W, lv.hid, stream()), "rsis_bias_grad(hoist)")

    def wgrad_formats(self, lv):
        if lv.dyn.dtype == ops.DTYPE_BF16 and decoder_fused._BLK_WGRAD[0] and lv.W % 4 != 0 and lv.hid % 8 == 0 and lv.c_up % 8 == 0:
            return lv.hoist.dtype, ops.DTYPE_BF16_BLK, lambda x: ops.blk_from_nchw(x.flatten(0, 1))
        return lv.hoist.dtype, lv.dyn.dtype, lambda x: x.flatten(0, 1)


class _Blk(_Layout):
    blk = 1
    by_level = False

    def empty(self, lead, C, H, W):
        return torch.empty(lead + (C // 8, H, W, 8), dtype=torch.bfloat16, device=self.dev)

    def to_nchw(self, x):
        return ops.blk_to_nchw(x)

    def from_nchw(self, x):
        return ops.blk_from_nchw(x)

    def hoist(self, levels, feats, gates_w, gates_b, need_grad):
        jobs = []
        for lv, f, w, b in zip(levels, feats, gates_w, gates_b):
            lv.skip = f if _is_blk(f) else ops.blk_from_nchw(f)
            jobs.append(ops.blk_conv_job([lv.skip], lv.hoist.fwd(w, b), 4 * lv.hid, bias=lv.hoist.bias_p, dsts=[lv.G]))
        ops.blk_conv3x3_batch(jobs)

    def gates(self, levels, cells, wps):
        jobs = []
        for i, t in cells:
            lv = levels[i]
            jobs.append(ops.blk_conv_job(_gate_srcs(lv, t), wps[i], 4 * lv.hid, addend=lv.G, hid=lv.hid, c_prev=lv.Cs[t - 1] if t > 0 else None,
                                         c_out=lv.Cs[t], h_out=lv.Hs[t], act_out=lv.ACT[t] if lv.ACT is not None else None, side_key=lv.KEY[t],
                                         shape=(self.B, lv.H, lv.W)))
        ops.blk_conv3x3_batch(jobs)

    def up(self, levels, cells, s2=None):
        ups = [ops.blk_resize_job(levels[i].Hs[t], levels[i + 1].UP[t], scale=s2[i][t] if s2 is not None else None)
               for i, t in cells if i + 1 < len(levels)]
        if ups:
            ops.blk_upsample_fwd_batch(ups)

    def tail(self, last, UP5, conv_out, co_w, co_b, out_masks, heads, sc=None):
        heads()
        ops.blk_upsample_fwd_batch([ops.blk_resize_job(last.Hs.flatten(0, 1), UP5.flatten(0, 1), scale=sc)])
        check(self.L.rsis_blk_conv_out_seq_fwd(ptr(UP5), ptr(co_w.detach()), ptr(co_b.detach()), ptr(out_masks), self.T, self.B, 2 * last.H,
                                               2 * last.W, stream()), "rsis_blk_conv_out_seq_fwd")

    def tail_bwd(self, d_masks, last, UP5, dUP5, conv_out, co_w, dW, db):
        L, T, B = self.L, self.T, self.B
        H5, W5 = 2 * last.H, 2 * last.W
        check(L.rsis_blk_conv_out_seq_dgrad(ptr(d_masks), ptr(co_w.detach()), ptr(dUP5), T, B, H5, W5, stream()), "rsis_blk_conv_out_seq_dgrad")
        if dW or db:
            dW = dW() if dW else torch.zeros_like(co_w)
            db = db() if db else None
            check(L.rsis_blk_conv_out_seq_wgrad(ptr(d_masks), ptr(UP5), ptr(dW), ptr(db), T, B, H5, W5, stream()), "rsis_blk_conv_out_seq_wgrad")

    def up5_bwd(self, dUP5, dside, last, DH_last, sc=None):
        ops.blk_upsample_bwd_batch([ops.blk_resize_job(dUP5.flatten(0, 1), DH_last.flatten(0, 1), dside, last.ARG, backward=True, scale=sc)])

    def up_bwd(self, levels, cells, DUP, DH, dsides, s2=None):
        ups = [ops.blk_resize_job(DUP[i + 1], DH[i], dsides[i][t], levels[i].ARG[t], backward=True, scale=s2[i][t] if s2 is not None else None)
               for i, t in cells if i + 1 < len(levels)]
        if ups:
            ops.blk_upsample_bwd_batch(ups)

    def lstm_bwd(self, jobs):
        ops.blk_lstm_bwd_batch([ops.blk_lstm_bwd_job(*job) for job in jobs])

    def dgrad(self, jobs):
        if jobs:
            ops.blk_conv3x3_batch([ops.blk_conv_job([dy], wd, sum(x.shape[1] for x in dxs) * 8, cpack=cin, dsts=dxs) for dy, wd, cin, _dt, dxs in jobs])

    def sum_t(self, DA, dG):
        check(self.L.rsis_blk_sum_leading(ptr(DA), ptr(dG), self.T, dG.numel() // 8, stream()), "rsis_blk_sum_leading")

    skip_dgrad = dgrad

    def bias_grad(self, dG, db, lv):
        check(self.L.rsis_blk_bias_grad(ptr(dG), ptr(db), self.B, 4 * lv.hid, lv.H * lv.W, lv.hid, stream()), "rsis_blk_bias_grad")

    def wgrad_formats(self, lv):
        return ops.DTYPE_BF16_BLK, ops.DTYPE_BF16_BLK, lambda x: x.flatten(0, 1)


class _DecoderSeqFn(torch.autograd.Function):

    @staticmethod
    def forward(ctx, layout, decoder, T, keep, want_hidden, *tensors):
        L = lib()
        n = len(decoder.clstm_list)
        feats = [t.contiguous() for t in tensors[:n]]
        params = tensors[n:]
        gates_w, gates_b = params[0:2 * n:2], params[1:2 * n:2]
        co_w, co_b, Wc, bc, Ws, bs = params[2 * n:2 * n + 6]
        _lib.require_cuda_f32(*params)
        need_grad = bool(keep) and any(ctx.needs_input_grad)
        dev = feats[0].device
        B = feats[0].shape[0]
        lay = layout(L, T, B, dev)
        hs = [c.hidden_size for c in decoder.clstm_list]
        tot = sum(hs)
        f32 = dict(dtype=torch.float32, device=dev)
        KEY = torch.zeros(T * B * tot, dtype=torch.int64, device=dev)
        SIDE = torch.empty(T * B * tot, **f32)
        ARG = torch.empty(T * B * tot, dtype=torch.int32, device=dev)
        levels = []
        for i, cell in enumerate(decoder.clstm_list):
            lv = _Level()
            lv.cell, lv.hid, lv.c_up, lv.c_skip = cell, hs[i], (0 if i == 0 else hs[i - 1]), _chan(feats[i])
            lv.H, lv.W = feats[i].shape[2], feats[i].shape[3]
            lv.hoist, lv.dyn = decoder_fused._packs(cell, lv.c_up, lv.c_skip)
            lv.G = lay.empty((B,), 4 * lv.hid, lv.H, lv.W)
            lv.Hs = lay.empty((T, B), lv.hid, lv.H, lv.W)
            lv.Cs = torch.empty((T, B, lv.hid, lv.H, lv.W), **f32)
            lv.ACT = lay.empty((T, B), 4 * lv.hid, lv.H, lv.W) if need_grad else None
            lv.UP = lay.empty((T, B), lv.c_up, lv.H, lv.W) if lv.c_up > 0 else None
            levels.append(lv)
        for lv, key, side, arg in zip(levels, _per_level(KEY, hs, T, B), _per_level(SIDE, hs, T, B), _per_level(ARG, hs, T, B)):
            lv.KEY, lv.SIDE, lv.ARG = key, side, arg
        drop = None
        p2, pc, ps = dropout.rates(decoder)
        if p2 > 0 or pc > 0 or ps > 0:
            drop = _Drop()
            drop.S2, drop.MC, drop.MS = dropout.draw(dropout.decoder_state(decoder, dev), T * B * tot, p2, pc, ps)
            drop.s2 = _per_level(drop.S2, hs, T, B) if p2 > 0 else None
            drop.SIDEC, drop.SIDES = torch.empty(T * B * tot, **f32), torch.empty(T * B * tot, **f32)
        s2 = drop.s2 if drop is not None else None
        lay.hoist(levels, feats, gates_w, gates_b, need_grad)
        last = levels[-1]
        H5, W5 = 2 * last.H, 2 * last.W
        upc = UPCONV[0] and s2 is None and L.rsis_upconv_out_supported(last.hid, last.H, last.W, H5, W5) == 1
        UP5 = None if upc else lay.empty((T, B), last.hid, H5, W5)
        probs_tb = torch.empty((T, B, Wc.shape[0]), **f32)
        stop_tb = torch.empty((T, B, 1), **f32)
        wps = [lv.dyn.fwd(w) for lv, w in zip(levels, gates_w)]
        for d in range(T + n - 1):
            cells = _diagonal(d, n, T)
            lay.gates(levels, cells, wps)
            if s2 is not None:
                lay.up(levels, cells, s2)
            else:
                lay.up(levels, cells)

        def heads():
            ops.heads_fwd_launch(L, [v.SIDE for v in levels], hs, T * B, Wc, bc, Ws, bs, probs_tb, stop_tb,
                                 ([v.KEY for v in levels], [v.ARG for v in levels]))
            if drop is not None:
                _heads_fwd_masked(L, SIDE, drop, hs, T, B, Wc, bc, Ws, bs, probs_tb, stop_tb)
        out_masks = torch.empty((B, T, H5 * W5), **f32)
        if upc:
            heads()
            check(L.rsis_upconv_out_fwd(ptr(last.Hs), lay.blk, ptr(co_w.detach()), ptr(co_b.detach()), ptr(out_masks), T, B, last.hid, last.H, last.W,
                                        H5, W5, stream()), "rsis_upconv_out_fwd")
        else:
# ... 35 lines not shown
        need_par = [need[5 + n + k] for k in range(len(params))]
        dev = feats[0].device
        B = feats[0].shape[0]
        hs = [lv.hid for lv in levels]
        f32 = dict(dtype=torch.float32, device=dev)
        last = levels[-1]
        H5, W5 = 2 * last.H, 2 * last.W
        UP5 = ctx.UP5
        drop = ctx.drop
        s2 = drop.s2 if drop is not None else None
        grads_par = [None] * len(params)

        def target(k):
            p = params[k]
            t = ops._direct_target(p)
            if t is not None:
                return t, True
            g = torch.zeros_like(p)
            grads_par[k] = g
            return g, False

        upc = ctx.upc
        dUP5 = None if upc else torch.empty_like(UP5)
        kw, kb = 2 * n, 2 * n + 1
        have_masks = d_masks is not None
        if upc:
            d_masks = torch.zeros((B, T, H5 * W5), **f32) if d_masks is None else d_masks.contiguous()
        elif d_masks is None:
            dUP5.zero_()
        else:
            lay.tail_bwd(d_masks.contiguous(), last, UP5, dUP5, decoder.conv_out, co_w, (lambda: target(kw)[0]) if need_par[kw] else None,
                         (lambda: target(kb)[0]) if need_par[kb] else None)
        DSIDE = torch.empty(T * B * sum(hs), **f32)
        dsides = _per_level(DSIDE, hs, T, B)
        if d_probs is None and d_stops is None:
            DSIDE.zero_()
        else:
            dp_tb = d_probs.transpose(0, 1).contiguous() if d_probs is not None else None
            ds_tb = d_stops.transpose(0, 1).contiguous() if d_stops is not None else None
            hb = [target(2 * n + 2 + k)[0] if need_par[2 * n + 2 + k] else None for k in range(4)]
            if drop is None:
                _heads_bwd_all_steps(L, levels, hs, n, T, B, Wc, Ws, ctx.probs_tb, dp_tb, ds_tb, dsides, hb)
            else:
                _heads_bwd_masked(L, drop, hs, T, B, Wc, Ws, ctx.probs_tb, dp_tb, ds_tb, DSIDE, hb)
        DA = [torch.empty_like(lv.ACT) for lv in levels]
        DH = [lay.empty((B,), lv.hid, lv.H, lv.W) for lv in levels]
        DHP = [lay.empty((B,), lv.hid, lv.H, lv.W) for lv in levels]
        DC = [[torch.empty((B, lv.hid, lv.H, lv.W), **f32) for _ in range(2)] for lv in levels]
        DUP = [lay.empty((B,), lv.c_up, lv.H, lv.W) if lv.c_up > 0 else None for lv in levels]
        dpk = [decoder_fused.dyn_dgrad_pack(lv.cell, lv.c_up, lv.c_skip, lv.H, lv.W) for lv in levels]
        wds = [pk.dgrad(w) for pk, w in zip(dpk, gates_w)]
        d_hidden = d_hidden or (None,) * (2 * n)
        dhf = [lay.from_nchw(g.contiguous()) if g is not None else None for g in d_hidden[0::2]]
        dcf = [g.contiguous() if g is not None else None for g in d_hidden[1::2]]
        DH_last = lay.empty((T, B), last.hid, last.H, last.W)
        if upc:
            dW = target(kw)[0] if need_par[kw] and have_masks else None
            db = target(kb)[0] if need_par[kb] and have_masks else None
            partial = torch.empty(L.rsis_upconv_out_bwd_blocks(T, B, last.H, last.W) * 80, **f32)
            check(L.rsis_upconv_out_bwd(ptr(d_masks), ptr(last.Hs), lay.blk, ptr(co_w.detach()), ptr(DH_last), ptr(dW), ptr(db), ptr(dsides[n - 1]),
                                        ptr(last.ARG), ptr(partial), T, B, last.hid, last.H, last.W, H5, W5, stream()), "rsis_upconv_out_bwd")
        else:
            if s2 is not None:
                lay.up5_bwd(dUP5, dsides[n - 1], last, DH_last, s2[n - 1])
            else:
                lay.up5_bwd(dUP5, dsides[n - 1], last, DH_last)
        for d in range(T + n - 2, -1, -1):
            cells = _diagonal(d, n, T)
            if s2 is not None:
                lay.up_bwd(levels, cells, DUP, DH, dsides, s2)
            else:
                lay.up_bwd(levels, cells, DUP, DH, dsides)
            lstm, dg = [], []
            for i, t in cells:
                lv = levels[i]
                dh2, dcn = (dhf[i], dcf[i]) if t == T - 1 else (DHP[i], DC[i][(t + 1) & 1])
                lstm.append((DH[i] if i + 1 < n else DH_last[t], dh2, dcn, lv.ACT[t], lv.Cs[t - 1] if t > 0 else None, lv.Cs[t], DA[i][t],
                             DC[i][t & 1] if t > 0 else None))
                dxs = ([DUP[i]] if lv.c_up > 0 else []) + ([DHP[i]] if t > 0 else [])
                if dxs:
                    dg.append((DA[i][t], wds[i], lv.dyn.cin, dpk[i].dtype, dxs))
            lay.lstm_bwd(lstm)
            lay.dgrad(dg)
        dG, dskip, dfeats = [None] * n, [None] * n, [None] * n
        for grp in ([[i] for i in range(n)] if lay.by_level else [range(n)]):
            for i in grp:
                if T == 1:
                    dG[i] = DA[i][0]
                else:
                    dG[i] = torch.empty_like(levels[i].G)
                    lay.sum_t(DA[i], dG[i])
                if need_feat[i]:
                    dskip[i] = torch.empty_like(levels[i].skip)
            lay.skip_dgrad([(dG[i], levels[i].hoist.dgrad(gates_w[i]), levels[i].hoist.cin, levels[i].hoist.dtype, [dskip[i]]) for i in grp
                            if need_feat[i]])
            for i in grp:
                lv = levels[i]
                kw, kb = 2 * i, 2 * i + 1
                hid, H, W = lv.hid, lv.H, lv.W
                if need_feat[i]:
                    dfeats[i] = dskip[i] if _is_blk(feats[i]) else lay.to_nchw(dskip[i])
                if need_par[kb]:
                    lay.bias_grad(dG[i], target(kb)[0], lv)
                if need_par[kw]:
                    dW, direct = target(kw)
                    Ctot = gates_w[i].shape[1]
                    dt_skip, dt, rows = lay.wgrad_formats(lv)
                    ops.wgrad_launch(L, dG[i], lv.skip, dW, B, lv.c_skip, H, W, 4 * hid, H, W, 3, 1, 1, Ctot, lv.c_up, hid, dt_skip,
                                     "rsis_conv2d_wgrad(hoist)", direct)
                    da = rows(DA[i])
                    if lv.c_up > 0:
                        ops.wgrad_launch(L, da, rows(lv.UP), dW, T * B, lv.c_up, H, W, 4 * hid, H, W, 3, 1, 1, Ctot, 0, hid, dt,
                                         "rsis_conv2d_wgrad(batched up)", direct)
                    if T > 1:
                        ops.wgrad_launch(L, da[B:], rows(lv.Hs[:T - 1]), dW, (T - 1) * B, hid, H, W, 4 * hid, H, W, 3, 1, 1, Ctot, lv.c_up + lv.c_skip,
                                         hid, dt, "rsis_conv2d_wgrad(batched h)", direct)
        for lv in levels:
            lv.G = lv.Hs = lv.Cs = lv.ACT = lv.UP = lv.skip = None
        ctx.lay = ctx.levels = ctx.UP5 = ctx.feats = ctx.params = ctx.decoder = ctx.drop = None
        return (None, None, None, None, None) + tuple(dfeats) + tuple(grads_par)


def decoder_sequence_stacked(decoder, skip_feats, T, want_hidden=True):
    n = len(decoder.clstm_list)
    params = []
    for c in decoder.clstm_list:
        params += [c.Gates.weight, c.Gates.bias]
    params += [decoder.conv_out.weight, decoder.conv_out.bias, decoder.fc_class.weight, decoder.fc_class.bias, decoder.fc_stop.weight,
               decoder.fc_stop.bias]
    keep = torch.is_grad_enabled() and (any(f.requires_grad for f in skip_feats) or any(p.requires_grad for p in params))
    layout = _Blk if blk_supported(decoder, skip_feats) else _Nchw
    res = _DecoderSeqFn.apply(layout, decoder, int(T), keep, bool(want_hidden), *skip_feats, *params)
    out_masks, out_probs, out_stops = res[:3]
    hidden = [[res[3 + 2 * i], res[4 + 2 * i]] for i in range(n)] if len(res) > 3 else None
    size = (2 * skip_feats[-1].shape[2], 2 * skip_feats[-1].shape[3])
    return out_masks, out_probs, out_stops, hidden, size
```

rsis_amd/ops.py:

```python
import ctypes
import os
import weakref

import torch

from . import _lib
from ._lib import check, int_array, lib, ptr, ptr_array, require_cuda_f32, stream

_WEIGHT_EPOCH = [0]


FORCE_TILE = [0]


DIRECT_GRAD = [False]


def _direct_target(param):
    g = param.grad if DIRECT_GRAD[0] and param is not None else None
    return g if (g is not None and g.is_contiguous() and g.dtype == torch.float32 and g.is_cuda) else None


DTYPE_F32, DTYPE_BF16 = 0, 1
DTYPE_F32_WINO = 3
# ... 21 lines not shown
        return d
    return DTYPE_F32_WINO if (rule == "all" or (cin == cout and cin in rule)) else d

DTYPES = {"fp32": DTYPE_F32, "f32": DTYPE_F32, "float32": DTYPE_F32, "bf16": DTYPE_BF16, "bfloat16": DTYPE_BF16}


def set_dtype(module, dtype):
    d = DTYPES[dtype] if isinstance(dtype, str) else int(dtype)
    for m in module.modules():
        if hasattr(m, "_set_rsis_dtype"):
            m._set_rsis_dtype(d)
    return module


def set_deterministic(on=True):
    return bool(lib().rsis_set_deterministic(1 if on else 0))


def is_deterministic():
    return bool(lib().rsis_get_deterministic())


SUBSAMPLE_1X1 = [os.environ.get("RSIS_SUBSAMPLE_1X1", "1") != "0"]
_PACKS = weakref.WeakSet()
_BATCH = {"sig": None, "jobs": None, "n": 0, "blocks": 0}


def repack_all():
    L = lib()
    todo = []
    for p in list(_PACKS):
        w = p._refs[0]() if p._refs is not None else None
        if w is None or not w.is_cuda:
            continue
        b = p._refs[1]() if p._refs[1] is not None else None
        if p.wp is not None and p._key_f is not None:
            todo.append((p, w, b, p.wp, 0))
        if p.wd is not None and p._key_d is not None:
            todo.append((p, w, b, p.wd, 1))
    if not todo:
        return
    sig = tuple((id(p), w.data_ptr(), out.data_ptr(), d) for p, w, _b, out, d in todo)
    if _BATCH["sig"] != sig:
        jobs = (_lib.PackJob * len(todo))()
        blocks = 0
        for i, (p, w, _b, out, d) in enumerate(todo):
            jobs[i] = p._job(w, out, d)
            nb = L.rsis_conv_pack_job_fill(ctypes.byref(jobs[i]))
            if nb < 0:
                raise _lib.RsisHipError("rsis_conv_pack_job_fill rejected a pack job")
            jobs[i].block_begin = blocks
            blocks += nb
        raw = torch.frombuffer(bytearray(bytes(jobs)), dtype=torch.uint8).to(todo[0][1].device)
        _BATCH.update(sig=sig, jobs=raw, n=len(todo), blocks=blocks)
    check(L.rsis_conv_pack_batch(ptr(_BATCH["jobs"]), _BATCH["n"], _BATCH["blocks"], stream()), "rsis_conv_pack_batch")
    for p, w, b, _out, d in todo:
        if d == 0:
            p._key_f = p._key(w) + ((b._version, b.data_ptr()) if b is not None else ())
            if b is not None and p.lstm_hid > 0:
                p._pack_bias(b)
        else:
            p._key_d = p._key(w)


def bump_weight_epoch():
    _WEIGHT_EPOCH[0] += 1


class PackedConv(object):

    def __init__(self, ks, segs, lstm_hid=0, stride=1, pad=None, offs=None, dtype=DTYPE_F32):
        self.dtype = int(dtype)
        if int(lstm_hid) > 0 and int(ks) != 3:
            self.dtype = DTYPE_F32
        self.ks = int(ks)
        self.stride = int(stride)
        self.pad = int(ks // 2 if pad is None else pad)
        self.segs = [int(s) for s in segs]
        self.offs = [int(o) for o in offs] if offs is not None else None
        self.cin = sum(self.segs)
        self.lstm_hid = int(lstm_hid)
        self._key_f = None
        self._key_d = None
        self.training_call = False
        self._twin = None
        self.wp = None
        self.wd = None
        self.bias_p = None
        self._refs = None

    def _key(self, w):
        return (_WEIGHT_EPOCH[0], w._version, w.data_ptr(), self.dtype)

    def direct_twin(self):
        if self._twin is None:
            self._twin = PackedConv(self.ks, self.segs, lstm_hid=self.lstm_hid, stride=self.stride, pad=self.pad, offs=self.offs, dtype=DTYPE_F32)
        return self._twin

    def _pack_bias(self, bias):
        n = 4 * self.lstm_hid
        if self.bias_p is None or self.bias_p.numel() != n or self.bias_p.device != bias.device:
            self.bias_p = torch.empty(n, dtype=torch.float32, device=bias.device)
        self.bias_p.view(self.lstm_hid, 4).copy_(bias.detach().view(4, self.lstm_hid).t())

    def _job(self, w, out, dgrad):
        j = _lib.PackJob()
        j.W, j.out, j.dgrad, j.dtype = w.data_ptr(), out.data_ptr(), int(dgrad), self.dtype
        j.Cout, j.Ctot, j.ks, j.stride, j.pad = w.shape[0], w.shape[1], self.ks, self.stride, self.pad
        j.nseg, j.lstm_hid = len(self.segs), self.lstm_hid
        off = 0
        for i, c in enumerate(self.segs):
            j.Cseg[i] = c
            j.Coff[i] = self.offs[i] if self.offs is not None else off
            off += c
        return j

    def _seg_args(self):
        return len(self.segs), int_array(self.segs), (int_array(self.offs) if self.offs is not None else None)

    def fwd(self, w, bias=None):
        key = self._key(w) + ((bias._version, bias.data_ptr()) if bias is not None else ())
        if self._key_f != key:
            L = lib()
            Cout, Ctot = w.shape[0], w.shape[1]
            nseg, segs, offs = self._seg_args()
            n = L.rsis_conv_packed_bytes_fwd(self.dtype, Cout, self.ks, self.stride, self.pad, nseg, segs) // 4
            if self.wp is None or self.wp.numel() != n:
                self.wp = torch.zeros(n, dtype=torch.float32, device=w.device)
            check(L.rsis_conv_pack_fwd(ptr(w.detach()), ptr(self.wp), Cout, Ctot, self.ks, self.stride, self.pad, nseg, segs, offs,
                                       self.lstm_hid, self.dtype, stream()), "rsis_conv_pack_fwd")
            if bias is not None and self.lstm_hid > 0:
                self._pack_bias(bias)
            self._key_f = key
            self._refs = (weakref.ref(w), weakref.ref(bias) if bias is not None else None)
            _PACKS.add(self)
        return self.wp

    def dgrad(self, w):
        key = self._key(w)
        if self._key_d != key:
            L = lib()
            Cout, Ctot = w.shape[0], w.shape[1]
            nseg, segs, offs = self._seg_args()
            n = L.rsis_conv_packed_bytes_dgrad(self.dtype, Cout, self.ks, self.stride, self.pad, self.cin) // 4
            if self.wd is None or self.wd.numel() != n:
                self.wd = torch.zeros(n, dtype=torch.float32, device=w.device)
            check(L.rsis_conv_pack_dgrad(ptr(w.detach()), ptr(self.wd), Cout, Ctot, self.ks, self.stride, self.pad, nseg, segs, offs,
                                         self.lstm_hid, self.dtype, stream()), "rsis_conv_pack_dgrad")
            self._key_d = key
            if self._refs is None:
                self._refs = (weakref.ref(w), None)
            _PACKS.add(self)
        return self.wd


def _contig(t):
    return t if t.is_contiguous() else t.contiguous()


def _conv_out_size(n, ks, stride, pad):
    return (n + 2 * pad - ks) // stride + 1


def _dgrad_all(L, dy, wd, cin_packed, ks, stride, pad, srcs, Hx, Wx, addend=None, inplace=False, dtype=DTYPE_F32):
    B, Cout, Hy, Wy = dy.shape
    shapes = [tuple(s.shape) if torch.is_tensor(s) else tuple(s) for s in srcs]
    dxs = [addend] if inplace else [torch.empty(sh, dtype=torch.float32, device=dy.device) for sh in shapes]
    check(L.rsis_conv2d_dgrad(ptr(dy), B, Cout, Hy, Wy, ptr(wd), cin_packed, ks, stride, pad, ptr_array(dxs),
                              int_array([sh[1] for sh in shapes]), len(shapes), Hx, Wx, ptr(addend), FORCE_TILE[0], dtype, stream()),
          "rsis_conv2d_dgrad")
    return dxs


class GradSlot(object):

    def __init__(self):
        self.grad = None
        self.done = False

    def reset(self):
        self.grad, self.done = None, False

    def take(self):
        g, self.grad = self.grad, None
        self.done = True
        return g

    def park(self, g):
        if self.done or self.grad is not None or g is None:
            return False
        self.grad = g
        return True


class _GradTapFn(torch.autograd.Function):
    @staticmethod
    def forward(ctx, x, slot):
        ctx.slot = slot
        return x.view_as(x)

    @staticmethod
    def backward(ctx, g):
        if g is not None and ctx.slot.park(g if g.is_contiguous() else g.contiguous()):
            return None, None
        return g, None


def grad_tap(x, slot):
    if slot is None or not (torch.is_grad_enabled() and x.requires_grad):
        return x
    return _GradTapFn.apply(x, slot)


WGRAD_DEFER = [False]
_WGRAD_QUEUE = []


def wgrad_launch(L, dy, x, dW, B, Cs, H, W, Cout, Ho, Wo, ks, stride, pad, Ctot, c_off, lstm_hid, dtype, what, direct):
    if direct and WGRAD_DEFER[0]:
        _WGRAD_QUEUE.append(((dy.data_ptr(), x.data_ptr(), dW.data_ptr(), B, Cs, H, W, Cout, Ho, Wo, ks, stride, pad, Ctot, c_off, lstm_hid,
                              dtype), (dy, x, dW)))
        return
    check(L.rsis_conv2d_wgrad(ptr(dy), ptr(x), ptr(dW), B, Cs, H, W, Cout, Ho, Wo, ks, stride, pad, Ctot, c_off, lstm_hid, dtype, stream()), what)


def flush_wgrads():
    n = len(_WGRAD_QUEUE)
    if n == 0:
        return
    jobs = (_lib.WgradJob * n)()
    for j, (f, _keep) in zip(jobs, _WGRAD_QUEUE):
        (j.dy, j.x, j.dW, j.B, j.Cs, j.H, j.W, j.Cout, j.Ho, j.Wo, j.ks, j.stride, j.pad, j.Ctot, j.c_off, j.lstm_hid, j.dtype) = f
    try:
        check(lib().rsis_conv2d_wgrad_batch(jobs, n, stream()), "rsis_conv2d_wgrad_batch")
    finally:
        del _WGRAD_QUEUE[:]


def _wgrad_all(L, dy, srcs, w_shape, ks, stride, pad, lstm_hid, out=None, dtype=DTYPE_F32):
    B, Cout, Ho, Wo = dy.shape
    Ctot = w_shape[1]
    dW = out if out is not None else torch.zeros(w_shape, dtype=torch.float32, device=dy.device)
    c_off = 0
    for s in srcs:
        _, Cs, H, W = s.shape
        wgrad_launch(L, dy, s, dW, B, Cs, H, W, Cout, Ho, Wo, ks, stride, pad, Ctot, c_off, lstm_hid, dtype, "rsis_conv2d_wgrad",
                     out is not None)
        c_off += Cs
    return dW


class _Conv2dFn(torch.autograd.Function):
    @staticmethod
    def forward(ctx, pack, stride, pad, nsrc, slot, *tensors):
        srcs = [_contig(t) for t in tensors[:nsrc]]
        weight, bias = tensors[nsrc], tensors[nsrc + 1]
        ctx.slot = slot
        require_cuda_f32(weight, bias, *srcs)
        L = lib()
        B, _, H, W = srcs[0].shape
        Cout, ks = weight.shape[0], weight.shape[2]
        Ho, Wo = _conv_out_size(H, ks, stride, pad), _conv_out_size(W, ks, stride, pad)
        if pack.stride != stride or pack.pad != pad:
            raise _lib.RsisHipError("PackedConv was built for stride %d pad %d, used with %d/%d" % (pack.stride, pack.pad, stride, pad))
        wp = pack.fwd(weight)
        out = torch.empty((B, Cout, Ho, Wo), dtype=torch.float32, device=weight.device)
        ctx.in_shape = None
        if ks == 1 and stride > 1 and pad == 0 and nsrc == 1 and (SUBSAMPLE_1X1[0] or pack.dtype == DTYPE_BF16):
            ctx.in_shape = tuple(srcs[0].shape)
            sub = torch.empty((B, srcs[0].shape[1], Ho, Wo), dtype=torch.float32, device=weight.device)
            check(L.rsis_subsample2d(ptr(srcs[0]), ptr(sub), B * srcs[0].shape[1], H, W, stride, stream()), "rsis_subsample2d")
            srcs = [sub]
            H, W, stride_k = Ho, Wo, 1
        else:
            stride_k = stride
        tile = FORCE_TILE[0] + (100 if pack.training_call else 0)
        check(L.rsis_conv2d_fwd(ptr_array(srcs), int_array([s.shape[1] for s in srcs]), nsrc, B, H, W, ptr(wp), Cout, ks, stride_k,
                                pad, ptr(bias.detach() if bias is not None else None), None, ptr(out), Ho, Wo, tile, pack.dtype, stream()),
              "rsis_conv2d_fwd")
        ctx.pack, ctx.stride, ctx.pad, ctx.nsrc = pack, stride, pad, nsrc
        ctx.has_bias = bias is not None
        ctx.wparam, ctx.bparam = weight, bias
        ctx.save_for_backward(weight, *srcs)
        return out

    @staticmethod
    def backward(ctx, dy):
        weight = ctx.saved_tensors[0]
        srcs = list(ctx.saved_tensors[1:])
        dy = _contig(dy)
        L = lib()
        ks = weight.shape[2]
        nsrc = ctx.nsrc
        grads = [None] * (nsrc + 2)
        take, park = ctx.slot if isinstance(ctx.slot, tuple) else (ctx.slot, None)
        addend = take.take() if take is not None else None
        sub = ctx.in_shape is not None
        in_shapes = [ctx.in_shape] if sub else [tuple(t.shape) for t in srcs]
        if any(ctx.needs_input_grad[5:5 + nsrc]):
            wd = ctx.pack.dgrad(weight)
            inplace, extra = False, None
            if addend is not None:
                if nsrc != 1 or tuple(addend.shape) != in_shapes[0]:
                    raise _lib.RsisHipError("GradSlot: the parked gradient does not belong to this conv's input")
                if ctx.stride != 1:
                    if ks == 1 and ctx.pad == 0 and addend.is_contiguous():
                        inplace = True
                    else:
                        extra, addend = addend, None
            dxs = _dgrad_all(L, dy, wd, ctx.pack.cin, ks, ctx.stride, ctx.pad, in_shapes, in_shapes[0][2], in_shapes[0][3], addend,
                             inplace, dtype=ctx.pack.dtype)
            if extra is not None:
                dxs[0].add_(extra)
            for i in range(nsrc):
                if ctx.needs_input_grad[5 + i]:
                    grads[i] = dxs[i]
            if park is not None and nsrc == 1 and grads[0] is not None and park.park(grads[0]):
                grads[0] = None
        want_w = ctx.needs_input_grad[5 + nsrc]
        want_b = ctx.has_bias and ctx.needs_input_grad[6 + nsrc]
        if (want_w and want_b and weight.shape[0] == 1 and ks == 3 and ctx.stride == 1 and ctx.pad == 1 and nsrc == 1 and
                weight.shape[1] in (4, 8, 16) and srcs[0].shape[3] % 4 == 0):
            tw, tb = _direct_target(ctx.wparam), _direct_target(ctx.bparam)
            dW = tw if tw is not None else torch.zeros_like(weight)
            db = tb if tb is not None else torch.zeros(1, dtype=torch.float32, device=dy.device)
            x0 = srcs[0]
            check(L.rsis_conv_out_wgrad(ptr(dy), ptr(x0), ptr(dW), ptr(db), x0.shape[0], x0.shape[1], x0.shape[2], x0.shape[3], stream()),
                  "rsis_conv_out_wgrad")
            grads[nsrc] = None if tw is not None else dW
            grads[nsrc + 1] = None if tb is not None else db
            return (None, None, None, None, None) + tuple(grads)
        if want_w:
            tgt = _direct_target(ctx.wparam)
            dW = _wgrad_all(L, dy, srcs, tuple(weight.shape), ks, 1 if sub else ctx.stride, ctx.pad, 0, out=tgt, dtype=ctx.pack.dtype)
            grads[nsrc] = None if tgt is not None else dW
        if want_b:
            tgt = _direct_target(ctx.bparam)
            db = tgt if tgt is not None else torch.zeros(weight.shape[0], dtype=torch.float32, device=dy.device)
            check(L.rsis_bias_grad(ptr(dy), ptr(db), dy.shape[0], dy.shape[1], dy.shape[2] * dy.shape[3], 0, stream()),
                  "rsis_bias_grad")
            grads[nsrc + 1] = None if tgt is not None else db
        return (None, None, None, None, None) + tuple(grads)


def conv2d(srcs, weight, bias, stride, pad, pack, grad_slot=None, park_slot=None):
    training = (torch.is_grad_enabled() and (weight.requires_grad or any(s.requires_grad for s in srcs))) or TRAINING_FORWARD[0]
    if pack.dtype == DTYPE_F32_WINO and not training and not WINOGRAD_INFER[0]:
        pack = pack.direct_twin()
    pack.training_call = training
    if grad_slot is not None:
        grad_slot.reset()
    slot = grad_slot if park_slot is None else (grad_slot, park_slot)
    return _Conv2dFn.apply(pack, int(stride), int(pad), len(srcs), slot, *srcs, weight, bias)


EVAL_FOLD = [os.environ.get("RSIS_EVAL_FOLD", "1") != "0"]
_ERR_UNSUPPORTED = 3


def conv2d_bn_eval(x, weight, bias, stride, pad, pack, gamma, beta, running_mean, running_var, eps, relu=False, res=None):
    if not EVAL_FOLD[0] or torch.is_grad_enabled() or pack.dtype not in (DTYPE_F32, DTYPE_F32_WINO, DTYPE_BF16):
        return None
    if pack.dtype == DTYPE_F32_WINO:
        if WINOGRAD_INFER[0]:
            return None
        pack = pack.direct_twin()
    x = _contig(x)
    res = _contig(res) if res is not None else None
    require_cuda_f32(x, weight, bias, res, gamma, beta, running_mean, running_var)
    L = lib()
    B, Cin, H, W = x.shape
    Cout, ks = weight.shape[0], weight.shape[2]
    Ho, Wo = _conv_out_size(H, ks, stride, pad), _conv_out_size(W, ks, stride, pad)
    if pack.stride != stride or pack.pad != pad:
        raise _lib.RsisHipError("PackedConv was built for stride %d pad %d, used with %d/%d" % (pack.stride, pack.pad, stride, pad))
    if Cout % 4 != 0:
        return None
    pack.training_call = False
    wp = pack.fwd(weight)
    stride_k = stride
    if ks == 1 and stride > 1 and pad == 0:
        sub = torch.empty((B, Cin, Ho, Wo), dtype=torch.float32, device=x.device)
        check(L.rsis_subsample2d(ptr(x), ptr(sub), B * Cin, H, W, stride, stream()), "rsis_subsample2d")
        x, H, W, stride_k = sub, Ho, Wo, 1
    out = torch.empty((B, Cout, Ho, Wo), dtype=torch.float32, device=x.device)
    assert res is None or tuple(res.shape) == tuple(out.shape)
    rc = L.rsis_conv2d_fwd_bn_eval(ptr_array([x]), int_array([Cin]), 1, B, H, W, ptr(wp), Cout, ks, stride_k, pad,
                                   ptr(bias.detach() if bias is not None else None), ptr(res), ptr(gamma.detach()), ptr(beta.detach()),
                                   ptr(running_mean), ptr(running_var), float(eps), 1 if relu else 0, ptr(out), Ho, Wo, FORCE_TILE[0], pack.dtype, stream())
    if rc == _ERR_UNSUPPORTED:
        return None
    check(rc, "rsis_conv2d_fwd_bn_eval")
    return out


class _ConvLSTMFn(torch.autograd.Function):

    @staticmethod
    def forward(ctx, pack, pad, nx, has_state, training, *tensors):
        xs = [_contig(t) for t in tensors[:nx]]
        h_prev, c_prev, weight, bias = tensors[nx], tensors[nx + 1], tensors[nx + 2], tensors[nx + 3]
        require_cuda_f32(weight, bias, h_prev, c_prev, *xs)
        L = lib()
        B, _, H, W = xs[0].shape
        hid, ks = weight.shape[0] // 4, weight.shape[2]
        srcs = list(xs)
        if has_state:
            h_prev, c_prev = _contig(h_prev), _contig(c_prev)
            srcs.append(h_prev)
        wp = pack.fwd(weight, bias)
        need_grad = training and any(ctx.needs_input_grad)
        h = torch.empty((B, hid, H, W), dtype=torch.float32, device=weight.device)
        c = torch.empty_like(h)
        act = torch.empty((B, 4 * hid, H, W), dtype=torch.float32, device=weight.device) if need_grad else None
        segs = [s.shape[1] for s in srcs]
        check(L.rsis_convlstm_fwd(ptr_array(srcs), int_array(segs), len(srcs), B, H, W, ptr(wp), ptr(pack.bias_p), None,
                                  ptr(c_prev) if has_state else None, ptr(h), ptr(c), ptr(act), hid, ks, pad, FORCE_TILE[0], pack.dtype,
                                  stream()), "rsis_convlstm_fwd")
        ctx.pack, ctx.pad, ctx.nx, ctx.has_state = pack, pad, nx, has_state
        if need_grad:
            ctx.save_for_backward(weight, act, c, c_prev if has_state else None, *srcs)
        return h, c

# ... 627 lines not shown
```

rsis_amd/train.py:

```python
import os
import pickle
import random
import sys
import time

import numpy as np
import torch
import torch.distributed as dist

from . import ops
from .args import get_parser
from .modules.model import RSIS, FeatureExtractor
from .optim import BucketedAllReduce, FlatAdam, FlatOptimizer, FlatRMSprop, FlatSGD
from .synthetic import SyntheticLoader
from .utils.hungarian import match_indices, softIoU_matrix
from .utils.objectives import MaskedBCELoss, MaskedNLLLoss, softIoULoss
from .utils.utils import (base_param_multiplicity, check_parallel, get_base_params, get_skip_params, load_checkpoint, make_dir,
                          save_checkpoint)


BLK_SKIPS = [os.environ.get("RSIS_BLK_SKIPS", "1") != "0"]


def _blk_skips_ok(encoder, decoder, x, T=1):
# ... 90 lines not shown
            for out_mask, out_class, out_stop in steps:
                out_mask = ops.upsample_bilinear_ac(out_mask, (x.size(-2), x.size(-1)))
                out_masks.append(out_mask.reshape(out_mask.size(0), -1))
                out_classes.append(out_class)
                out_stops.append(out_stop)
            t = len(out_masks)
            out_masks = torch.stack(out_masks, 1)
            out_classes = torch.stack(out_classes, 1)
            out_stops = torch.stack(out_stops, 1)

    fused_iou = ops.softiou_supported(out_masks, y_mask)
    with torch.no_grad():
        scores = torch.ones(y_mask.size(0), args.gt_maxseqlen, args.maxseqlen, device=x.device)
        if fused_iou:
            iou_sums = ops.softiou_sums(out_masks, y_mask)
            scores[:, :, :t] = args.iou_weight * ops.softiou_cost_matrix(iou_sums)
        else:
            log_once("softiou-bmm", "soft-IoU scores through torch.bmm (ops.softiou_supported is False for these shapes / dtypes)")
            scores[:, :, :t] = args.iou_weight * softIoU_matrix(y_mask, out_masks)
        valid = (sw_mask.unsqueeze(-1) * sw_mask[:, 0:args.maxseqlen].unsqueeze(1) > 0).float()
        scores = scores * valid + (1 - valid) * 10
        if scores.is_cuda and scores.size(1) <= 128 and scores.size(1) >= scores.size(2):
            perm = ops.assign_min_cost(scores)
        else:
            log_once("host-assignment", "assignment on the host (scipy, one D2H sync per step): %d GT slots x %d steps" % (scores.size(1), scores.size(2)))
            perm = torch.from_numpy(match_indices(scores)).to(x.device)
        idx = perm[:, 0:t]
        need_perm_masks = want_outs or not fused_iou
        y_mask_perm = torch.gather(y_mask, 1, idx.unsqueeze(-1).expand(-1, -1, y_mask.size(2))) if need_perm_masks else None
        y_class_perm = torch.gather(y_class, 1, idx)
    sw_mask_t = sw_mask[:, 0:t].contiguous()
    sw_class_t = sw_class[:, 0:t].contiguous()

    with torch.set_grad_enabled(train):
        N, C = out_masks.size(-1), out_classes.size(-1)
        if fused_iou:
            siou = ops.softiou_matched(out_masks, y_mask, perm, iou_sums)
        else:
            siou = softIoU(y_mask_perm.reshape(-1, N), out_masks.reshape(-1, N))
        cls_w, bw = getattr(class_crit, "balance_weight", None), getattr(stop_xentropy, "balance_weight", None)
        if out_classes.is_cuda and out_classes.dtype == torch.float32:
            cw = cls_w.to(out_classes.device, torch.float32) if cls_w is not None else None
            loss, parts = ops.loss_tail(out_classes, y_class_perm, out_stops.squeeze(-1), siou.reshape(y_class_perm.shape), sw_mask_t,
                                        sw_class_t, cw, bw, args.iou_weight, args.class_weight if args.use_class_loss else 0.0,
                                        args.stop_weight if args.use_stop_loss else 0.0)
            loss_mask_iou, loss_stop, loss_class = parts[0], parts[1], parts[2]
        else:
            nll = MaskedNLL(y_class_perm.reshape(-1, 1), out_classes.reshape(-1, C), cls_w)
            loss_class = _masked_mean(nll.reshape(-1, 1), sw_mask_t.reshape(-1, 1))
            loss_mask_iou = _masked_mean(siou.reshape(-1, 1), sw_mask_t.reshape(-1, 1))
            bce = StableBalancedMaskedBCE(sw_mask_t, out_stops.squeeze(-1), bw)
            loss_stop = _masked_mean(bce.reshape(-1, 1), sw_class_t.reshape(-1, 1))
            loss = args.iou_weight * loss_mask_iou
            if args.use_class_loss:
                loss = loss + args.class_weight * loss_class
            if args.use_stop_loss:
                loss = loss + args.stop_weight * loss_stop

    enc_opt.zero_grad()
    dec_opt.zero_grad()
    if train:
        if reducer is not None:
            reducer.reset()
        direct = isinstance(enc_opt, FlatOptimizer) and isinstance(dec_opt, FlatOptimizer)
        if isinstance(dec_opt, FlatOptimizer):
            if args.use_class_loss:
                dec_opt.mark_has_grad(decoder.fc_class.parameters())
            if args.use_stop_loss:
                dec_opt.mark_has_grad(decoder.fc_stop.parameters())
        prev, ops.DIRECT_GRAD[0] = ops.DIRECT_GRAD[0], direct
        prev_defer, ops.WGRAD_DEFER[0] = ops.WGRAD_DEFER[0], direct and WGRAD_DEFER_DEFAULT[0]
        try:
            loss.backward()
            ops.flush_wgrads()
            if getattr(encoder, "_cut", None) is not None:
                if between is not None:
                    between("dec")
                encoder.backward_trunk(between)
                ops.flush_wgrads()
        finally:
            ops.DIRECT_GRAD[0] = prev
            ops.WGRAD_DEFER[0] = prev_defer
            del ops._WGRAD_QUEUE[:]
            if staged:
                encoder.split_backward, reducer.hooks_enabled = restore
        if staged:
            exchange.finish()
            apply_update(args, optims, 1.0 / reducer.world)
        elif do_update:
            apply_update(args, optims, reducer.finish() if reducer is not None else 1.0)

    losses = [loss.detach(), loss_mask_iou.detach(), loss_stop.detach(), loss_class.detach()]
    if sync_losses:
        losses = [float(v) for v in torch.stack(losses).cpu()]
    outs = [torch.sigmoid(out_masks.detach()) if want_outs else out_masks.detach(), out_classes.detach()]
    perms = [y_mask_perm, y_class_perm, perm]
    return losses, outs, perms


WGRAD_DEFER_DEFAULT = [os.environ.get("RSIS_WGRAD_DEFER", "1") != "0"]


def init_distributed():
    os.environ.setdefault("HSA_ENABLE_IPC_MODE_LEGACY", "0")
    world = int(os.environ.get("WORLD_SIZE", "1"))
    rank = int(os.environ.get("RANK", "0"))
    local_rank = int(os.environ.get("LOCAL_RANK", "0"))
    if torch.cuda.is_available():
        if os.environ.get("RSIS_SHARE_GPU", "") == "1":
            local_rank = local_rank % torch.cuda.device_count()
        torch.cuda.set_device(local_rank)
    if world > 1 and os.environ.get("RSIS_PIN_THREADS", "1") != "0":
        try:
            cores = sorted(os.sched_getaffinity(0))
            per = max(1, len(cores) // int(os.environ.get("LOCAL_WORLD_SIZE", world)))
            mine = cores[local_rank * per:(local_rank + 1) * per]
            if mine:
                os.sched_setaffinity(0, mine)
                torch.set_num_threads(max(1, min(per, 8)))
        except (AttributeError, OSError):
            pass
    force = os.environ.get("RSIS_FORCE_DIST", "") == "1"
    if (world > 1 or force) and not dist.is_initialized():
        os.environ.setdefault("MASTER_ADDR", "127.0.0.1")
        os.environ.setdefault("MASTER_PORT", "29500")
        backend = os.environ.get("RSIS_DIST_BACKEND", "nccl" if torch.cuda.is_available() else "gloo")
        dist.init_process_group(backend=backend, rank=rank, world_size=world)
    return rank, local_rank, world


def _flat_optimizer(rule, params, lr, weight_decay, momentum, name, lazy=(), lr_mult=None):
    if rule == "adam":
        return FlatAdam(params, lr=lr, weight_decay=weight_decay, name=name, lazy=lazy, lr_mult=lr_mult)
    if rule == "sgd":
        return FlatSGD(params, lr=lr, weight_decay=weight_decay, momentum=momentum, name=name, lazy=lazy, lr_mult=lr_mult)
    if rule == "rmsprop":
        return FlatRMSprop(params, lr=lr, weight_decay=weight_decay, name=name, lazy=lazy, lr_mult=lr_mult)
    raise Exception("optimizer %r: adam, sgd or rmsprop" % (rule,))


def build_optimizers(args, encoder, decoder):
    quirk = getattr(args, "enc_lr_quirk", False)
    if quirk and args.optim_cnn != "adam":
        raise Exception("--enc_lr_quirk reproduces repeated Adam updates only: it cannot be combined with -optim_cnn %s"
                        % args.optim_cnn)
    momentum = getattr(args, "momentum", 0.9)
    decoder_params = list(decoder.parameters()) + list(get_skip_params(encoder))
    lazy = [] if args.use_class_loss else list(decoder.fc_class.parameters())
    lazy += [] if args.use_stop_loss else list(decoder.fc_stop.parameters())
    dec_opt = _flat_optimizer(args.optim, decoder_params, args.lr, args.weight_decay, momentum, "dec", lazy=lazy)
    mult = base_param_multiplicity(encoder) if quirk else None
    enc_opt = _flat_optimizer(args.optim_cnn, list(get_base_params(args, encoder)), args.lr_cnn, args.weight_decay_cnn, momentum, "enc",
                              lr_mult=mult)
    return enc_opt, dec_opt


EXCHANGE_CUTS = int(os.environ.get("RSIS_EXCHANGE_CUTS", "2"))


class StagedExchange(object):

    def __init__(self, plan, reduce):
        self.plan, self.reduce, self.fired, self.pending = plan, reduce, [], []

    def __call__(self, stage):
        self.fired.append(stage)
# ... 444 lines not shown
```

Measured before the change: 972.5.

## Batch bias grads, fuse time-sum with bias grad, skip identity dgrad packing, tune BN loads

Deferred conv bias-gradient reductions are now queued and launched together through a grouped channel-sum kernel, so many small launches become few. The ConvLSTM backward time-sum is fused with its bias reduction. 1x1 dgrad packing is skipped when the packed layout equals the raw weight. The BN forward and backward kernels clamp their indices so loads happen without branches and the residual and ReLU-mask loads are issued early. These aim to cut launch overhead, extra memory passes and load latency, at the cost of more registers in the BN kernels and a different floating-point summation order.

```diff
diff --git a/include/rsis_hip.h b/include/rsis_hip.h
--- a/include/rsis_hip.h
+++ b/include/rsis_hip.h
@@ -26,6 +26,8 @@
                        const int* Coff, int lstm_hid, int dtype, void* stream);
 int rsis_conv_pack_dgrad(const float* W, void* Wd, int Cout, int Ctot, int ks, int stride, int pad, int nseg, const int* Cseg,
                          const int* Coff, int lstm_hid, int dtype, void* stream);
+int rsis_conv_dgrad_is_weight(int dtype, int Cout, int Ctot, int ks, int stride, int pad, int nseg, const int* Cseg, const int* Coff,
+                              int lstm_hid);
 
 int rsis_conv2d_fwd(const float* const* src, const int* Csrc, int nsrc, int B, int H, int W, const void* Wp, int Cout,
                     int ks, int stride, int pad, const float* bias, const float* addend, float* out, int Ho, int Wo,
@@ -51,6 +53,13 @@
 int rsis_conv2d_wgrad_batch(const rsis_wgrad_job* jobs, int njobs, void* stream);
 
 int rsis_bias_grad(const float* dy, float* db, int B, int C, int HW, int lstm_hid, void* stream);
+#define RSIS_BIAS_GRAD_MAX_JOBS 8
+typedef struct rsis_bias_grad_job {
+  const float* dy;
+  float* db;
+  int B, C, HW, lstm_hid;
+} rsis_bias_grad_job;
+int rsis_bias_grad_batch(const rsis_bias_grad_job* jobs, int njobs, void* stream);
 
 int rsis_convlstm_fwd(const float* const* src, const int* Csrc, int nsrc, int B, int H, int W, const void* Wp,
                       const float* bias_packed, const float* addend, const float* c_prev, float* h_out, float* c_out,
@@ -176,6 +185,7 @@
 int rsis_conv_out_seq_wgrad(const float* dy, const float* x, float* dW, float* db, int T, int B, int Cin, int H, int W, void* stream);
 
 int rsis_sum_leading(const float* x, float* y, int T, long n, void* stream);
+int rsis_sum_leading_bias(const float* x, float* y, float* db, int T, int B, int C, int HW, int lstm_hid, void* stream);
 
 int rsis_affine_nearest(const float* x, float* y, const float* mat, int mat_rows, int N, int C, int H, int W, void* stream);
 
diff --git a/rsis_amd/_lib.py b/rsis_amd/_lib.py
--- a/rsis_amd/_lib.py
+++ b/rsis_amd/_lib.py
@@ -9,6 +9,12 @@
 _vp, _i, _l, _f = ctypes.c_void_p, ctypes.c_int, ctypes.c_long, ctypes.c_float
 _ip = ctypes.POINTER(ctypes.c_int)
 _vpp = ctypes.POINTER(ctypes.c_void_p)
+
+
+class BiasGradJob(ctypes.Structure):
+    _fields_ = [("dy", ctypes.c_void_p), ("db", ctypes.c_void_p), ("B", ctypes.c_int), ("C", ctypes.c_int), ("HW", ctypes.c_int),
+                ("lstm_hid", ctypes.c_int)]
+
 
 class PackJob(ctypes.Structure):
     _fields_ = [("W", ctypes.c_void_p), ("out", ctypes.c_void_p), ("dgrad", ctypes.c_int), ("dtype", ctypes.c_int), ("Cout", ctypes.c_int),
@@ -75,6 +81,7 @@
     "rsis_conv_packed_bytes_dgrad": (_l, [_i, _i, _i, _i, _i, _i]),
     "rsis_conv_pack_fwd": (_i, [_vp, _vp, _i, _i, _i, _i, _i, _i, _ip, _ip, _i, _i, _vp]),
     "rsis_conv_pack_dgrad": (_i, [_vp, _vp, _i, _i, _i, _i, _i, _i, _ip, _ip, _i, _i, _vp]),
+    "rsis_conv_dgrad_is_weight": (_i, [_i, _i, _i, _i, _i, _i, _i, _ip, _ip, _i]),
     "rsis_conv_pack_job_fill": (_i, [ctypes.POINTER(PackJob)]),
     "rsis_conv_pack_batch": (_i, [_vp, _i, _i, _vp]),
     "rsis_conv2d_fwd": (_i, [_vpp, _ip, _i, _i, _i, _i, _vp, _i, _i, _i, _i, _vp, _vp, _vp, _i, _i, _i, _i, _vp]),
@@ -95,6 +102,8 @@
     "rsis_conv_out_seq_wgrad": (_i, [_vp, _vp, _vp, _vp, _i, _i, _i, _i, _i, _vp]),
     "rsis_sum_leading": (_i, [_vp, _vp, _i, _l, _vp]),
     "rsis_bias_grad": (_i, [_vp, _vp, _i, _i, _i, _i, _vp]),
+    "rsis_bias_grad_batch": (_i, [ctypes.POINTER(BiasGradJob), _i, _vp]),
+    "rsis_sum_leading_bias": (_i, [_vp, _vp, _vp, _i, _i, _i, _i, _i, _vp]),
     "rsis_convlstm_fwd": (_i, [_vpp, _ip, _i, _i, _i, _i, _vp, _vp, _vp, _vp, _vp, _vp, _vp, _i, _i, _i, _i, _i, _vp]),
     "rsis_convlstm_fwd_batch": (_i, [ctypes.POINTER(LstmJob), _i, _vp]),
     "rsis_convlstm_bwd_gates": (_i, [_vp, _vp, _vp, _vp, _vp, _vp, _vp, _vp, _vp, _i, _i, _i, _vp]),
diff --git a/rsis_amd/csrc/api.hip b/rsis_amd/csrc/api.hip
--- a/rsis_amd/csrc/api.hip
+++ b/rsis_amd/csrc/api.hip
@@ -158,6 +158,15 @@
 int rsis_conv_pack_dgrad(const float* W, void* Wd, int Cout, int Ctot, int ks, int stride, int pad, int nseg, const int* Cseg,
                          const int* Coff, int lstm_hid, int dtype, void* stream) {
   return pack_one(true, W, Wd, Cout, Ctot, ks, stride, pad, nseg, Cseg, Coff, lstm_hid, dtype, stream);
+}
+
+int rsis_conv_dgrad_is_weight(int dtype, int Cout, int Ctot, int ks, int stride, int pad, int nseg, const int* Cseg, const int* Coff,
+                              int lstm_hid) {
+  if (pack_args_check(Cout, Ctot, ks, nseg, Cseg, Coff, lstm_hid)) return 0;
+  const PackPlan p = pack_plan(true, dtype, Cout, Ctot, ks, stride, pad, nseg, Cseg, Coff, lstm_hid);
+  return p.status == RSIS_OK && p.mode == PACK_IGEMM_DGRAD && ks == 1 && nseg == 1 && Cseg[0] == Ctot && (!Coff || Coff[0] == 0) &&
+                 lstm_hid == 0 && p.ldw == Ctot && p.krows == Cout
+             ? 1 : 0;
 }
 
 int rsis_conv_pack_job_fill(rsis_pack_job* j) {
@@ -455,6 +464,24 @@
 int rsis_bias_grad(const float* dy, float* db, int B, int C, int HW, int lstm_hid, void* stream) {
   if (!dy || !db) return RSIS_ERR_ARG;
   return rsis_l_channel_sum(dy, db, B, C, HW, lstm_hid, (hipStream_t)stream);
+}
+static bool bias_grad_ok(const float* dy, const float* db, int B, int C, int HW, int lstm_hid) {
+  return dy && db && B >= 1 && C >= 1 && HW >= 1 && lstm_hid >= 0 && (lstm_hid == 0 || C == 4 * lstm_hid);
+}
+int rsis_bias_grad_batch(const rsis_bias_grad_job* jobs, int njobs, void* stream) {
+  if (!jobs || njobs < 1) return RSIS_ERR_ARG;
+  for (int j = 0; j < njobs; ++j)
+    if (!bias_grad_ok(jobs[j].dy, jobs[j].db, jobs[j].B, jobs[j].C, jobs[j].HW, jobs[j].lstm_hid)) return RSIS_ERR_ARG;
+  for (int j0 = 0; j0 < njobs; j0 += RSIS_BIAS_GRAD_MAX_JOBS) {
+    const int m = njobs - j0 < RSIS_BIAS_GRAD_MAX_JOBS ? njobs - j0 : RSIS_BIAS_GRAD_MAX_JOBS;
+    const int rc = rsis_l_channel_sum_group(jobs + j0, m, (hipStream_t)stream);
+    if (rc != RSIS_OK) return rc;
+  }
+  return RSIS_OK;
+}
+int rsis_sum_leading_bias(const float* x, float* y, float* db, int T, int B, int C, int HW, int lstm_hid, void* stream) {
+  if (!x || !y || T < 1 || !bias_grad_ok(y, db, B, C, HW, lstm_hid)) return RSIS_ERR_ARG;
+  return rsis_l_sum_leading_bias(x, y, db, T, B, C, HW, lstm_hid, (hipStream_t)stream);
 }
 
 static int lstm_fill(ConvArgs& a, int& route, const float* const* src, const int* Csrc, int nsrc, int B, int H, int W, const void* Wp,
diff --git a/rsis_amd/csrc/launchers.h b/rsis_amd/csrc/launchers.h
--- a/rsis_amd/csrc/launchers.h
+++ b/rsis_amd/csrc/launchers.h
@@ -55,6 +55,8 @@
 int rsis_l_maxpool_bwd(const float* dy, const unsigned char* arg, float* dx, long BC, int H, int W, int Ho, int Wo, int accumulate, hipStream_t st);
 int rsis_l_sum_leading(const float* x, float* y, int T, long n, hipStream_t st);
 int rsis_l_channel_sum(const float* dy, float* db, int B, int C, int HW, int hid, hipStream_t st);
+int rsis_l_sum_leading_bias(const float* x, float* y, float* db, int T, int B, int C, int HW, int hid, hipStream_t st);
+int rsis_l_channel_sum_group(const rsis_bias_grad_job* jobs, int n, hipStream_t st);
 int rsis_l_adam(float* p, const float* g, float* m, float* v, long n, float lr, float b1, float b2, float eps, float wd, int step, float gscale, const int* step_dev,
                 hipStream_t st);
 int rsis_l_assign(const float* scores, long long* perm, int B, int G, int T, hipStream_t st);
diff --git a/rsis_amd/csrc/pointwise.hip b/rsis_amd/csrc/pointwise.hip
--- a/rsis_amd/csrc/pointwise.hip
+++ b/rsis_amd/csrc/pointwise.hip
@@ -588,7 +588,8 @@
   for (int i = 0; i < NT / 64; ++i) { a += sa[i]; b += sb[i]; }
 }
 
-template <int NT, int VPT>
+constexpr bool BN_RES_EARLY_256 = false, BN_RES_EARLY_512 = true, BN_RES_EARLY_1024 = true;
+template <int NT, int VPT, bool RES_EARLY>
 __global__ __launch_bounds__(NT) void bn_fwd_fused_kernel(const float* __restrict__ x, const float* __restrict__ res,
                                                           float* __restrict__ y, unsigned char* __restrict__ mask,
                                                           const float* __restrict__ gamma,
@@ -598,14 +599,31 @@
                                                           float momentum, int relu) {
   const int c = blockIdx.x;
   const int ng = (int)(N / 4), hwg = HW / 4;
-  f32x4 v[VPT];
+  f32x4 v[VPT], rv[RES_EARLY ? VPT : 1];
   double s = 0.0, ss = 0.0;
 #pragma unroll
   for (int i = 0; i < VPT; ++i) {
-    const int g = threadIdx.x + i * NT;
-    if (g < ng) {
-      const int b = g / hwg, sp = (g - b * hwg) * 4;
-      v[i] = *reinterpret_cast<const f32x4*>(x + ((size_t)b * C + c) * HW + sp);
+    const int g = min((int)threadIdx.x + i * NT, ng - 1);
+    const int b = g / hwg, sp = (g - b * hwg) * 4;
+    v[i] = *reinterpret_cast<const f32x4*>(x + ((size_t)b * C + c) * HW + sp);
+  }
+  if constexpr (RES_EARLY) {
+    if (res) {
+#pragma unroll
+      for (int i = 0; i < VPT; ++i) {
+        const int g = min((int)threadIdx.x + i * NT, ng - 1);
+        const int b = g / hwg, sp = (g - b * hwg) * 4;
+        rv[i] = *reinterpret_cast<const f32x4*>(res + ((size_t)b * C + c) * HW + sp);
+      }
+    } else {
+#pragma unroll
+      for (int i = 0; i < VPT; ++i) rv[i] = f32x4{0.f, 0.f, 0.f, 0.f};
+    }
+  }
+#pragma unroll
+  for (int i = 0; i < VPT; ++i) {
+    if ((int)threadIdx.x + i * NT < ng) {
+#pragma clang fp contract(off)
       s += (v[i][0] + v[i][1]) + (v[i][2] + v[i][3]);
       ss += (v[i][0] * v[i][0] + v[i][1] * v[i][1]) + (v[i][2] * v[i][2] + v[i][3] * v[i][3]);
     }
@@ -629,7 +647,8 @@
       const int b = g / hwg, sp = (g - b * hwg) * 4;
       const size_t idx = ((size_t)b * C + c) * HW + sp;
       f32x4 r = {0.f, 0.f, 0.f, 0.f};
-      if (res) r = *reinterpret_cast<const f32x4*>(res + idx);
+      if constexpr (RES_EARLY) r = rv[i];
+      else if (res) r = *reinterpret_cast<const f32x4*>(res + idx);
       f32x4 o;
 #pragma unroll
       for (int k = 0; k < 4; ++k) { const float t = v[i][k] * sc + sh + r[k]; o[k] = relu ? fmaxf(t, 0.f) : t; }
@@ -674,22 +693,34 @@
       }
     }
   } else {
+    f32x4 yv[VPT];
 #pragma unroll
     for (int i = 0; i < VPT; ++i) {
-      const int gi = threadIdx.x + i * NT;
-      if (gi < ng) {
+      const int gi = min((int)threadIdx.x + i * NT, ng - 1);
+      const int b = gi / hwg, sp = (gi - b * hwg) * 4;
+      const size_t idx = ((size_t)b * C + c) * HW + sp;
+      g[i] = *reinterpret_cast<const f32x4*>(dy + idx);
+      xh[i] = *reinterpret_cast<const f32x4*>(x + idx);
+    }
+    if (relu) {
+#pragma unroll
+      for (int i = 0; i < VPT; ++i) {
+        const int gi = min((int)threadIdx.x + i * NT, ng - 1);
         const int b = gi / hwg, sp = (gi - b * hwg) * 4;
-        const size_t idx = ((size_t)b * C + c) * HW + sp;
-        g[i] = *reinterpret_cast<const f32x4*>(dy + idx);
-        const f32x4 xv = *reinterpret_cast<const f32x4*>(x + idx);
-        if (relu) {
-          const f32x4 yv = *reinterpret_cast<const f32x4*>(y + idx);
-#pragma unroll
-          for (int k = 0; k < 4; ++k) if (!(yv[k] > 0.f)) g[i][k] = 0.f;
-        }
+        yv[i] = *reinterpret_cast<const f32x4*>(y + ((size_t)b * C + c) * HW + sp);
+      }
+    } else {
+#pragma unroll
+      for (int i = 0; i < VPT; ++i) yv[i] = f32x4{1.f, 1.f, 1.f, 1.f};
+    }
+#pragma unroll
+    for (int i = 0; i < VPT; ++i) {
+      if ((int)threadIdx.x + i * NT < ng) {
+#pragma unroll
+        for (int k = 0; k < 4; ++k) if (!(yv[i][k] > 0.f)) g[i][k] = 0.f;
         float p1 = 0.f, p2 = 0.f;
 #pragma unroll
-        for (int k = 0; k < 4; ++k) { xh[i][k] = (xv[k] - m) * r; p1 += g[i][k]; p2 += g[i][k] * xh[i][k]; }
+        for (int k = 0; k < 4; ++k) { xh[i][k] = (xh[i][k] - m) * r; p1 += g[i][k]; p2 += g[i][k] * xh[i][k]; }
         s1 += p1; s2 += p2;
       }
     }
@@ -832,24 +863,7 @@
   }
 }
 
-__global__ __launch_bounds__(256) void channel_sum_kernel(const float* __restrict__ dy, float* __restrict__ db, int C, int HW,
-                                                          long N, int hid) {
-  const int c = blockIdx.x;
-  double s = 0.0;
-  if ((HW & 3) == 0) {
-    const long ng = N / 4;
-    const int hwg = HW / 4;
-    for (long g = blockIdx.y * 256L + threadIdx.x; g < ng; g += gridDim.y * 256L) {
-      const long b = g / hwg; const int sp = (int)(g - b * hwg) * 4;
-      const f32x4 v = *reinterpret_cast<const f32x4*>(dy + (b * C + c) * HW + sp);
-      s += ((double)v[0] + (double)v[1]) + ((double)v[2] + (double)v[3]);
-    }
-  } else {
-    for (long e = blockIdx.y * 256L + threadIdx.x; e < N; e += gridDim.y * 256L) {
-      const long b = e / HW; const int sp = (int)(e - b * HW);
-      s += dy[(b * C + c) * HW + sp];
-    }
-  }
+__device__ __forceinline__ void channel_sum_finish(double s, float* __restrict__ db, int c, int hid) {
   for (int o = 32; o > 0; o >>= 1) s += __shfl_down(s, o, 64);
   __shared__ double sa[4];
   if ((threadIdx.x & 63) == 0) sa[threadIdx.x >> 6] = s;
@@ -858,6 +872,38 @@
     const int row = hid > 0 ? (c & 3) * hid + (c >> 2) : c;
     atomicAdd(db + row, (float)(sa[0] + sa[1] + sa[2] + sa[3]));
   }
+}
+__device__ __forceinline__ void channel_sum_body(const float* __restrict__ dy, float* __restrict__ db, int C, int HW, long N, int hid,
+                                                 int c, int split, int nsplit) {
+  double s = 0.0;
+  if ((HW & 3) == 0) {
+    const long ng = N / 4;
+    const int hwg = HW / 4;
+    for (long g = split * 256L + threadIdx.x; g < ng; g += nsplit * 256L) {
+      const long b = g / hwg; const int sp = (int)(g - b * hwg) * 4;
+      const f32x4 v = *reinterpret_cast<const f32x4*>(dy + (b * C + c) * HW + sp);
+      s += ((double)v[0] + (double)v[1]) + ((double)v[2] + (double)v[3]);
+    }
+  } else {
+    for (long e = split * 256L + threadIdx.x; e < N; e += nsplit * 256L) {
+      const long b = e / HW; const int sp = (int)(e - b * HW);
+      s += dy[(b * C + c) * HW + sp];
+    }
+  }
+  channel_sum_finish(s, db, c, hid);
+}
+__global__ __launch_bounds__(256) void channel_sum_kernel(const float* __restrict__ dy, float* __restrict__ db, int C, int HW,
+                                                          long N, int hid) {
+  channel_sum_body(dy, db, C, HW, N, hid, blockIdx.x, blockIdx.y, gridDim.y);
+}
+struct ChannelSumJob { const float* dy; float* db; long N; int C, HW, hid, nsplit, begin; };
+struct ChannelSumGroup { ChannelSumJob job[RSIS_BIAS_GRAD_MAX_JOBS]; int n; };
+__global__ __launch_bounds__(256) void channel_sum_group_kernel(const ChannelSumGroup g) {
+  int j = 0;
+  while (j + 1 < g.n && (int)blockIdx.x >= g.job[j + 1].begin) ++j;
+  const ChannelSumJob& a = g.job[j];
+  const int l = blockIdx.x - a.begin;
+  channel_sum_body(a.dy, a.db, a.C, a.HW, a.N, a.hid, l % a.C, l / a.C, a.nsplit);
 }
 
 __global__ void adam_kernel(float* __restrict__ p, const float* __restrict__ g, float* __restrict__ m, float* __restrict__ v,
@@ -1197,13 +1243,13 @@
   if (mask && (!relu || (HW & 3))) return RSIS_ERR_UNSUPPORTED;
   if (train && bn_fused_ok(C, HW, N)) {
     if (N / 4 <= 256 * 8 && C <= 512)
-      hipLaunchKernelGGL((bn_fwd_fused_kernel<512, 4>), dim3(C), dim3(512), 0, st, x, res, y, mask, gamma, beta, run_mean, run_var,
+      hipLaunchKernelGGL((bn_fwd_fused_kernel<512, 4, BN_RES_EARLY_512>), dim3(C), dim3(512), 0, st, x, res, y, mask, gamma, beta, run_mean, run_var,
                          save_mean, save_rstd, C, HW, N, eps, momentum, relu);
     else if (N / 4 <= 256 * 8)
-      hipLaunchKernelGGL((bn_fwd_fused_kernel<256, 8>), dim3(C), dim3(256), 0, st, x, res, y, mask, gamma, beta, run_mean, run_var,
+      hipLaunchKernelGGL((bn_fwd_fused_kernel<256, 8, BN_RES_EARLY_256>), dim3(C), dim3(256), 0, st, x, res, y, mask, gamma, beta, run_mean, run_var,
                          save_mean, save_rstd, C, HW, N, eps, momentum, relu);
     else
-      hipLaunchKernelGGL((bn_fwd_fused_kernel<1024, 8>), dim3(C), dim3(1024), 0, st, x, res, y, mask, gamma, beta, run_mean, run_var,
+      hipLaunchKernelGGL((bn_fwd_fused_kernel<1024, 8, BN_RES_EARLY_1024>), dim3(C), dim3(1024), 0, st, x, res, y, mask, gamma, beta, run_mean, run_var,
                          save_mean, save_rstd, C, HW, N, eps, momentum, relu);
     return rsis_check_launch();
   }
@@ -1308,6 +1354,37 @@
   return rsis_check_launch();
 }
 
+__global__ __launch_bounds__(256) void sum_leading_bias_kernel(const float* __restrict__ x, float* __restrict__ y, float* __restrict__ db,
+                                                               int T, long n4, int C, int HW, long N, int hid) {
+  const int c = blockIdx.x;
+  const long ng = N / 4;
+  const int hwg = HW / 4;
+  double s = 0.0;
+  for (long g = blockIdx.y * 256L + threadIdx.x; g < ng; g += gridDim.y * 256L) {
+    const long b = g / hwg; const int sp = (int)(g - b * hwg) * 4;
+    const size_t o = (size_t)(((b * C + c) * HW + sp) >> 2);
+    const f32x4* p = reinterpret_cast<const f32x4*>(x) + o;
+    f32x4 acc = p[0];
+    for (int t = 1; t < T; ++t) { const f32x4 v = p[(size_t)t * n4]; acc[0] += v[0]; acc[1] += v[1]; acc[2] += v[2]; acc[3] += v[3]; }
+    reinterpret_cast<f32x4*>(y)[o] = acc;
+    s += ((double)acc[0] + (double)acc[1]) + ((double)acc[2] + (double)acc[3]);
+  }
+  channel_sum_finish(s, db, c, hid);
+}
+int rsis_l_sum_leading_bias(const float* x, float* y, float* db, int T, int B, int C, int HW, int hid, hipStream_t st) {
+  const long n = (long)B * C * HW;
+  const bool fused = (HW & 3) == 0 && ((((size_t)x | (size_t)y) & 15) == 0) && !rsis_deterministic();
+  if (!fused) {
+    const int rc = rsis_l_sum_leading(x, y, T, n, st);
+    return rc != RSIS_OK ? rc : rsis_l_channel_sum(y, db, B, C, HW, hid, st);
+  }
+  const long N = (long)B * HW;
+  int S = chan_splits(C, N);
+  if (S > 512) S = 512;
+  hipLaunchKernelGGL(sum_leading_bias_kernel, dim3(C, S), dim3(256), 0, st, x, y, db, T, n / 4, C, HW, N, hid);
+  return rsis_check_launch();
+}
+
 int rsis_l_channel_sum(const float* dy, float* db, int B, int C, int HW, int hid, hipStream_t st) {
   const long N = (long)B * HW;
   int S = chan_splits(C, N);
@@ -1315,6 +1392,24 @@
   hipLaunchKernelGGL(channel_sum_kernel, dim3(C, S), dim3(256), 0, st, dy, db, C, HW, N, hid);
   return rsis_check_launch();
 }
+int rsis_l_channel_sum_group(const rsis_bias_grad_job* jobs, int n, hipStream_t st) {
+  if (n < 1 || n > RSIS_BIAS_GRAD_MAX_JOBS) return RSIS_ERR_ARG;
+  ChannelSumGroup g;
+  g.n = n;
+  long total = 0;
+  for (int j = 0; j < n; ++j) {
+    ChannelSumJob& a = g.job[j];
+    a.dy = jobs[j].dy; a.db = jobs[j].db; a.C = jobs[j].C; a.HW = jobs[j].HW; a.hid = jobs[j].lstm_hid;
+    a.N = (long)jobs[j].B * a.HW;
+    a.nsplit = chan_splits(a.C, a.N);
+    if (a.nsplit > 512) a.nsplit = 512;
+    a.begin = (int)total;
+    total += (long)a.C * a.nsplit;
+    if (total >= (1L << 31)) return RSIS_ERR_UNSUPPORTED;
+  }
+  hipLaunchKernelGGL(channel_sum_group_kernel, dim3((unsigned)total), dim3(256), 0, st, g);
+  return rsis_check_launch();
+}
 int rsis_l_adam(float* p, const float* g, float* m, float* v, long n, float lr, float b1, float b2, float eps, float wd,
                 int step, float gscale, const int* step_dev, hipStream_t st) {
   hipLaunchKernelGGL(adam_kernel, dim3(ew_grid(n)), dim3(256), 0, st, p, g, m, v, n, lr, b1, b2, eps, wd, step, gscale, step_dev);
diff --git a/rsis_amd/decoder_seq.py b/rsis_amd/decoder_seq.py
--- a/rsis_amd/decoder_seq.py
+++ b/rsis_amd/decoder_seq.py
@@ -295,6 +295,10 @@
     def sum_t(self, DA, dG):
         check(self.L.rsis_sum_leading(ptr(DA), ptr(dG), self.T, dG.numel(), stream()), "rsis_sum_leading")
 
+    def sum_t_bias(self, DA, dG, db, lv):
+        check(self.L.rsis_sum_leading_bias(ptr(DA), ptr(dG), ptr(db), self.T, self.B, 4 * lv.hid, lv.H * lv.W, lv.hid, stream()),
+              "rsis_sum_leading_bias")
+
     def skip_dgrad(self, jobs):
         for dy, wd, cin, dtype, (dx,) in jobs:
             B, Cout, H, W = dy.shape
@@ -375,6 +379,8 @@
     def dgrad(self, jobs):
         if jobs:
             ops.blk_conv3x3_batch([ops.blk_conv_job([dy], wd, sum(x.shape[1] for x in dxs) * 8, cpack=cin, dsts=dxs) for dy, wd, cin, _dt, dxs in jobs])
+
+    sum_t_bias = None
 
     def sum_t(self, DA, dG):
         check(self.L.rsis_blk_sum_leading(ptr(DA), ptr(dG), self.T, dG.numel() // 8, stream()), "rsis_blk_sum_leading")
@@ -576,14 +582,18 @@
                     dg.append((DA[i][t], wds[i], lv.dyn.cin, dpk[i].dtype, dxs))
             lay.lstm_bwd(lstm)
             lay.dgrad(dg)
-        dG, dskip, dfeats = [None] * n, [None] * n, [None] * n
+        dG, dskip, dfeats, bias_done = [None] * n, [None] * n, [None] * n, [False] * n
         for grp in ([[i] for i in range(n)] if lay.by_level else [range(n)]):
             for i in grp:
                 if T == 1:
                     dG[i] = DA[i][0]
                 else:
                     dG[i] = torch.empty_like(levels[i].G)
-                    lay.sum_t(DA[i], dG[i])
+                    if need_par[2 * i + 1] and lay.sum_t_bias is not None:
+                        lay.sum_t_bias(DA[i], dG[i], target(2 * i + 1)[0], levels[i])
+                        bias_done[i] = True
+                    else:
+                        lay.sum_t(DA[i], dG[i])
                 if need_feat[i]:
                     dskip[i] = torch.empty_like(levels[i].skip)
             lay.skip_dgrad([(dG[i], levels[i].hoist.dgrad(gates_w[i]), levels[i].hoist.cin, levels[i].hoist.dtype, [dskip[i]]) for i in grp
@@ -594,7 +604,7 @@
                 hid, H, W = lv.hid, lv.H, lv.W
                 if need_feat[i]:
                     dfeats[i] = dskip[i] if _is_blk(feats[i]) else lay.to_nchw(dskip[i])
-                if need_par[kb]:
+                if need_par[kb] and not bias_done[i]:
                     lay.bias_grad(dG[i], target(kb)[0], lv)
                 if need_par[kw]:
                     dW, direct = target(kw)
diff --git a/rsis_amd/ops.py b/rsis_amd/ops.py
--- a/rsis_amd/ops.py
+++ b/rsis_amd/ops.py
@@ -127,6 +127,7 @@
         self.lstm_hid = int(lstm_hid)
         self._key_f = None
         self._key_d = None
+        self._ident = None
         self.training_call = False
         self._twin = None
         self.wp = None
@@ -181,7 +182,17 @@
             _PACKS.add(self)
         return self.wp
 
+    def dgrad_is_weight(self, w):
+        shape = tuple(w.shape)
+        if self._ident is None or self._ident[0] != shape:
+            nseg, segs, offs = self._seg_args()
+            self._ident = (shape, bool(lib().rsis_conv_dgrad_is_weight(self.dtype, shape[0], shape[1], self.ks, self.stride, self.pad, nseg,
+                                                                       segs, offs, self.lstm_hid)))
+        return self._ident[1] and w.is_contiguous() and w.dtype == torch.float32 and w.data_ptr() % 16 == 0
+
     def dgrad(self, w):
+        if self.dgrad_is_weight(w):
+            return w.detach()
         key = self._key(w)
         if self._key_d != key:
             L = lib()
@@ -270,6 +281,7 @@
 
 
 def flush_wgrads():
+    flush_bias_grads()
     n = len(_WGRAD_QUEUE)
     if n == 0:
         return
@@ -280,6 +292,30 @@
         check(lib().rsis_conv2d_wgrad_batch(jobs, n, stream()), "rsis_conv2d_wgrad_batch")
     finally:
         del _WGRAD_QUEUE[:]
+
+
+_BIAS_QUEUE = []
+
+
+def bias_grad_launch(L, dy, db, direct):
+    B, C, H, W = dy.shape
+    if direct and WGRAD_DEFER[0]:
+        _BIAS_QUEUE.append(((dy.data_ptr(), db.data_ptr(), B, C, H * W, 0), (dy, db)))
+        return
+    check(L.rsis_bias_grad(ptr(dy), ptr(db), B, C, H * W, 0, stream()), "rsis_bias_grad")
+
+
+def flush_bias_grads():
+    n = len(_BIAS_QUEUE)
+    if n == 0:
+        return
+    jobs = (_lib.BiasGradJob * n)()
+    for j, (f, _keep) in zip(jobs, _BIAS_QUEUE):
+        j.dy, j.db, j.B, j.C, j.HW, j.lstm_hid = f
+    try:
+        check(lib().rsis_bias_grad_batch(jobs, n, stream()), "rsis_bias_grad_batch")
+    finally:
+        del _BIAS_QUEUE[:]
 
 
 def _wgrad_all(L, dy, srcs, w_shape, ks, stride, pad, lstm_hid, out=None, dtype=DTYPE_F32):
@@ -382,8 +418,7 @@
         if want_b:
             tgt = _direct_target(ctx.bparam)
             db = tgt if tgt is not None else torch.zeros(weight.shape[0], dtype=torch.float32, device=dy.device)
-            check(L.rsis_bias_grad(ptr(dy), ptr(db), dy.shape[0], dy.shape[1], dy.shape[2] * dy.shape[3], 0, stream()),
-                  "rsis_bias_grad")
+            bias_grad_launch(L, dy, db, tgt is not None)
             grads[nsrc + 1] = None if tgt is not None else db
         return (None, None, None, None, None) + tuple(grads)
 
diff --git a/rsis_amd/train.py b/rsis_amd/train.py
--- a/rsis_amd/train.py
+++ b/rsis_amd/train.py
@@ -196,6 +196,7 @@
             ops.DIRECT_GRAD[0] = prev
             ops.WGRAD_DEFER[0] = prev_defer
             del ops._WGRAD_QUEUE[:]
+            del ops._BIAS_QUEUE[:]
             if staged:
                 encoder.split_backward, reducer.hooks_enabled = restore
         if staged:
```

After: 977.2 (median of 6 runs). No clear change (+0.5%).
